# duyhominhnguyen/conan-fgw

Hardware: AMD Instinct MI355X
Metric: molecules/s (K=5 conformers) (higher is better)
Workload: dtype f32

## Files before the change

### conan-fgw_amd/_lib.py

```python
from __future__ import annotations

import ctypes
import os
import subprocess

import torch

_HERE = os.path.dirname(os.path.abspath(__file__))
_SO = os.path.join(_HERE, "libconan_fgw_hip.so")
_LIB = None
ABI_VERSION = 6

c_int, c_float, c_void_p, c_ll = ctypes.c_int, ctypes.c_float, ctypes.c_void_p, ctypes.c_longlong


class FgwParams(ctypes.Structure):
    _fields_ = [("alpha", c_float), ("epsilon", c_float), ("max_iter", c_int), ("tol", c_float), ("inner_tol", c_float),
                ("num_iter_max", c_int), ("stop_thr", c_float), ("fixed_structure", c_int), ("fixed_features", c_int),
                ("warmstart", c_int), ("loss_fun", c_int), ("cs_small_int", c_int)]


class BatchLayout(ctypes.Structure):
    _fields_ = [(n, c_int) for n in ("B", "K", "num_graphs", "num_atoms", "num_bond_edges", "max_nodes", "x_dim", "ea_dim")] + \
               [(n, c_ll) for n in ("off_atom_off", "off_bond_off", "off_z", "off_pos", "off_x", "off_bsrc", "off_bdst", "off_battr", "off_y", "bytes")]


class WgradJob(ctypes.Structure):
    _fields_ = [("ws", c_void_p), ("dW", c_void_p), ("dbias", c_void_p), ("M", c_int), ("K", c_int), ("N", c_int), ("slices", c_int)]


class WgradSlabJob(ctypes.Structure):
    _fields_ = [("g", c_void_p), ("x", c_void_p), ("m_dev", c_void_p), ("ws", c_void_p), ("M", c_int), ("K", c_int), ("N", c_int), ("slices", c_int)]


_P = c_void_p
SIGNATURES = {
    "conan_abi_version": (c_int, []),
    "conan_collate_layout": (c_int, [c_int, c_int, _P, _P, c_int, c_int, ctypes.POINTER(BatchLayout)]),
    "conan_collate_pack": (c_int, [ctypes.POINTER(BatchLayout), _P, _P, _P, _P, _P, _P, _P, _P, _P]),
    "conan_collate_unpack": (c_int, [_P, ctypes.POINTER(BatchLayout), _P, _P, _P, _P, _P, _P, _P, _P, _P, _P, _P]),
    "conan_graph_ptr_from_batch": (c_int, [_P, c_int, c_int, _P, _P]),
    "conan_radius_graph_csr": (c_int, [_P, _P, c_int, c_int, c_float, c_int, c_int, _P, _P, _P, _P, _P, _P]),
    "conan_csr_transpose": (c_int, [_P, c_int, c_int, _P, _P, _P, _P, _P, _P]),
    "conan_edge_pairs": (c_int, [_P, _P, _P, _P, _P, c_int, _P, _P, _P, _P, _P, _P, _P, _P]),
    "conan_radius_graph_build_ws": (c_ll, [c_int, c_int, c_int, c_int]),
    "conan_radius_graph_build": (c_int, [_P, _P, c_int, c_int, c_float, c_int, c_int] + [_P] * 12 + [_P]),
    "conan_edge_index_i64": (c_int, [_P, _P, c_int, _P, _P]),
    "conan_embedding_fwd": (c_int, [_P, _P, c_int, c_int, c_int, _P, _P]),
    "conan_onehot_rows": (c_int, [_P, c_int, c_int, c_int, _P, _P]),
    "conan_embedding_bwd_ws": (c_ll, [c_int, c_int, c_int]),
    "conan_embedding_bwd": (c_int, [_P, _P, c_int, c_int, c_int, c_int, _P, _P, _P]),
    "conan_linear_fwd": (c_int, [_P, _P, _P, _P, c_int, c_int, c_int, c_int, c_int, _P, _P, _P]),
    "conan_linear_multi_fwd": (c_int, [_P, _P, _P, c_int, c_int, c_int, c_int, c_int, _P, _P, _P, _P]),
    "conan_linear_sum_fwd": (c_int, [_P, _P, _P, c_int, c_int, _P, _P, c_int, c_int, _P, _P, _P]),
    "conan_ssp_bwd": (c_int, [_P, _P, c_int, c_int, _P, _P, _P]),
    "conan_linear_wgrad_ws": (c_ll, [c_int, c_int, c_int]),
    "conan_linear_wgrad": (c_int, [_P, _P, c_int, c_int, c_int, _P, _P, _P, _P, _P]),
    "conan_bond_graph_csr": (c_int, [_P, c_int, c_int, _P, _P, _P, _P, _P, _P, _P, _P]),
    "conan_gat_edge_vec": (c_int, [_P, _P, c_int, c_int, _P, _P]),
    "conan_gat_edge_vec_bwd": (c_int, [_P, _P, _P, c_int, c_int, _P, _P, _P]),
    "conan_gat_node_alpha": (c_int, [_P, _P, _P, c_int, c_int, _P, _P, _P]),
    "conan_gat_aggregate_fwd": (c_int, [_P, _P, _P, _P, _P, _P, _P, c_int, _P, _P, c_float, c_int, c_int, _P, _P, _P, _P]),
    "conan_gat_bwd_ws": (c_ll, [c_int, c_int, c_int, c_int]),
    "conan_gat_aggregate_bwd": (c_int, [_P] * 15 + [c_int, _P, c_float, c_int, c_int, c_int, _P, _P, _P, _P]),
    "conan_linear_act_fwd": (c_int, [_P, _P, _P, c_int, c_int, c_int, c_int, _P, _P, _P, _P]),
    "conan_unary_fwd": (c_int, [_P, c_ll, c_int, _P, _P]),
    "conan_unary_bwd": (c_int, [_P, _P, c_ll, c_int, _P, _P]),
    "conan_zero_tail": (c_int, [_P, _P, c_int, c_int, _P]),
    "conan_rbf_wgrad": (c_int, [_P, _P, c_int, _P, c_int, c_float, c_int, _P, _P, _P, _P, _P]),
    "conan_wgrad_batchable": (c_int, [c_int, c_int]),
    "conan_linear_wgrad_scaled": (c_int, [_P, _P, c_int, c_int, c_int, _P, _P, _P, _P, _P, _P]),
    "conan_linear_wgrad_slabs": (c_int, [_P, _P, c_int, c_int, c_int, _P, _P, _P]),
    "conan_rbf_wgrad_slabs": (c_int, [_P, _P, c_int, _P, c_int, c_float, c_int, _P, _P, _P]),
    "conan_wgrad_reduce_batch": (c_int, [ctypes.POINTER(WgradJob), c_int, _P]),
    "conan_linear_wgrad_slabs_batch": (c_int, [ctypes.POINTER(WgradSlabJob), c_int, _P]),
    "conan_filter_bwd_supported": (c_int, [c_int, c_int]),
    "conan_filter_bwd_slices": (c_int, [c_int]),
    "conan_filter_bwd_ws": (c_ll, [c_int, c_int, c_int]),
    "conan_filter_bwd": (c_int, [_P, _P, _P, c_int, _P, c_int, c_float, _P, c_int, _P, _P, _P, _P, _P, _P]),
    "conan_filter_bwd2_supported": (c_int, [c_int, c_int]),
    "conan_filter_bwd2_slices": (c_int, [c_int]),
    "conan_filter_bwd2_ws": (c_ll, [c_int, c_int, c_int]),
    "conan_filter_bwd2": (c_int, [_P, _P, _P, c_int, _P, c_int, c_float, _P, c_int, _P, _P, _P, _P, _P, _P, _P, _P]),
    "conan_rbf_fwd": (c_int, [_P, _P, c_int, _P, c_int, c_float, _P, _P]),
    "conan_cutoff_scale": (c_int, [_P, _P, c_int, c_int, c_float, _P, _P, _P]),
# ... 63 lines not shown
    "conan_fgw_densify": (c_int, [_P, _P, _P, _P, c_int, c_int, c_int, c_float, c_float, c_float, _P, _P, _P, _P]),
    "conan_fgw_densify_bwd": (c_int, [_P, _P, _P, _P, c_int, c_int, c_int, c_float, c_float, c_float, _P, _P]),
    "conan_fgw_workspace_bytes": (c_ll, [c_int] * 7),
    "conan_fgw_barycenter_fwd": (c_int, [_P, _P, _P, _P, _P, _P, _P, c_int, c_int, c_int, c_int, ctypes.POINTER(FgwParams), c_int, c_int,
                                         _P, _P, _P, _P, _P, _P, _P, _P]),
    "conan_fgw_barycenter_fwd_ragged": (c_int, [_P, _P, _P, _P, _P, _P, _P, _P, _P, _P, c_int, c_int, c_int, c_int, ctypes.POINTER(FgwParams),
                                                c_int, c_int, _P, _P, _P, _P, _P, _P, _P, _P]),
    "conan_fgw_pair_workspace_bytes": (c_ll, [c_int, c_int, c_int, c_int]),
    "conan_fgw_pair_fwd": (c_int, [_P, _P, _P, _P, _P, _P, c_int, c_int, ctypes.POINTER(FgwParams), c_int, c_int, _P, _P, _P, _P, _P, _P]),
    "conan_fgw_pair_dist": (c_int, [_P, _P, _P, _P, _P, _P, c_int, c_int, c_float, c_int, _P, _P]),
    "conan_fgw_pair_dist_bwd": (c_int, [_P, _P, _P, _P, _P, _P, c_int, c_int, c_float, c_int, _P, _P, _P, _P, _P, _P]),
    "conan_fgw_acc_lds_resident": (c_int, [c_int]),
    "conan_fgw_acc_pair_workspace_bytes": (c_ll, [c_int, c_int]),
    "conan_fgw_acc_pair_fwd": (c_int, [_P] * 6 + [c_int, c_int, ctypes.c_double, ctypes.c_double, c_int, ctypes.c_double] + [_P] * 5),
    "conan_fgw_mixup_workspace_bytes": (c_ll, [c_int, c_int, c_int, c_int]),
    "conan_fgw_mixup_barycenter_fwd": (c_int, [_P] * 7 + [c_int, c_int, c_int, c_int, ctypes.POINTER(FgwParams), ctypes.c_double, c_int, ctypes.c_double] + [_P] * 8),
    "conan_sinkhorn_workspace_bytes": (c_ll, [c_int, c_int, c_int]),
    "conan_sinkhorn_lds_resident": (c_int, [c_int, c_int]),
    "conan_sinkhorn_fwd": (c_int, [_P] * 7 + [c_int, c_int, c_int, c_ll, c_float, c_int, c_int, c_float] + [_P] * 8),
    "conan_sinkhorn_bwd_workspace_bytes": (c_ll, [c_int, c_int, c_int, c_int]),
    "conan_sinkhorn_bwd_lds_resident": (c_int, [c_int, c_int]),
    "conan_sinkhorn_bwd": (c_int, [_P] * 7 + [c_int, c_int, c_int, c_ll, c_float, c_int, c_int] + [_P] * 9),
    "conan_sinkhorn_ext_workspace_bytes": (c_ll, [c_int, c_int, c_int]),
    "conan_sinkhorn_ext_lds_resident": (c_int, [c_int, c_int]),
    "conan_sinkhorn_ext_nerr": (c_int, [c_int, c_int, c_int]),
    "conan_sinkhorn_ext_fwd": (c_int, [_P] * 7 + [c_int, c_int, c_int, c_ll, ctypes.c_double, c_int, c_int, ctypes.c_double, ctypes.c_double, c_int,
                                       ctypes.c_double, c_int] + [_P] * 11),
    "conan_fgw_barycenter_bwd": (c_int, [_P, _P, _P, _P, c_int, c_int, c_int, c_int, _P, _P]),
    "conan_fgw_barycenter_bwd_full_workspace_bytes": (c_ll, [c_int, c_int, c_int, c_int]),
    "conan_fgw_barycenter_bwd_full": (c_int, [_P, _P, _P, _P, _P, _P, _P, _P, _P, c_int, c_int, c_int, c_int, c_int, c_int, c_int,
                                              _P, _P, _P, _P, _P, _P, _P, _P]),
    "conan_fgw_readout_fwd": (c_int, [_P, c_int, c_int, c_int, c_int, c_int, _P, _P]),
    "conan_fgw_readout_bwd": (c_int, [_P, _P, c_int, c_int, c_int, c_int, c_int, _P, _P]),
}

_D = ctypes.c_double
EXT_SIGNATURES = {
    "conan_fgw_acc_pair_bwd_lds_resident": (c_int, [c_int]),
    "conan_fgw_acc_pair_bwd_workspace_bytes": (c_ll, [c_int, c_int, c_int]),
    "conan_fgw_acc_pair_bwd": (c_int, [_P] * 6 + [c_int, c_int, _D, _D, c_int] + [_P] * 12),
}

EXT_TABLES = {
    "conan_fgw_hip_pair_grad.h": {
        "conan_fgw_pair_bwd_lds_resident": (c_int, [c_int]),
        "conan_fgw_pair_bwd_workspace_bytes": (c_ll, [c_int, c_int, c_int, c_int]),
        "conan_fgw_pair_bwd": (c_int, [_P] * 6 + [c_int, c_int, _D, _D, c_int, c_int, _D, c_int, c_int] + [_P] * 13),
    },
    "conan_fgw_hip_bregman_grad.h": {
        "conan_fgw_bregman_bwd_lds_resident": (c_int, [c_int]),
        "conan_fgw_bregman_bwd_workspace_bytes": (c_ll, [c_int, c_int, c_int]),
        "conan_fgw_bregman_bwd": (c_int, [_P] * 6 + [c_int, c_int, _D, _D, c_int, c_int, c_int] + [_P] * 13),
    },
    "conan_fgw_hip_mixup_grad.h": {
        "conan_fgw_mixup_barycenter_fwd_record": (c_int, [_P] * 7 + [c_int, c_int, c_int, c_int, ctypes.POINTER(FgwParams), _D, c_int, _D] + [_P] * 9),
        "conan_fgw_mixup_barycenter_bwd_lds_resident": (c_int, [c_int]),
        "conan_fgw_mixup_barycenter_bwd_workspace_bytes": (c_ll, [c_int] * 5),
        "conan_fgw_mixup_barycenter_bwd": (c_int, [_P] * 6 + [c_int, c_int, c_int, c_int, ctypes.POINTER(FgwParams), _D, c_int, _D] + [_P] * 15),
    },
}

_ERR = {-1: "bad argument", -2: "HIP launch failure", -3: "unsupported configuration"}


def library_path() -> str:
    return _SO


def build(force: bool = False) -> str:
    args = ["make", "-C", os.path.join(_HERE, "csrc"), "-s", "-j8"]
    if force:
        args.append("-B")
    subprocess.check_call(args)
    return _SO


def lib():
    global _LIB
    if _LIB is None:
        if not os.path.exists(_SO):
            raise RuntimeError(
                f"{_SO} is missing: the HIP extension is not built. Run `python -c 'import __graft_entry__ as g; g.build()'` "
                "(or make -C conan-fgw_amd/csrc). There is no CPU fallback for this path.")
        L = ctypes.CDLL(_SO)
        for table in (SIGNATURES, EXT_SIGNATURES, *EXT_TABLES.values()):
            for name, (res, args) in table.items():
                fn = getattr(L, name)
                fn.restype, fn.argtypes = res, args
        if L.conan_abi_version() != ABI_VERSION:
            raise RuntimeError(f"libconan_fgw_hip.so: ABI version {L.conan_abi_version()} != {ABI_VERSION} expected by _lib.py (stale build: "
                               "make -C conan-fgw_amd/csrc)")
        _LIB = L
    return _LIB


def stream_ptr() -> int:
    return _raw_stream(_cur_device())


try:
    _raw_stream = torch._C._cuda_getCurrentRawStream
    _cur_device = torch._C._cuda_getDevice
except AttributeError:
    def _raw_stream(_dev):
        return torch.cuda.current_stream().cuda_stream

# ... 31 lines not shown
```

### conan-fgw_amd/csrc/fp_planes.h

```cpp
#pragma once
#include "common.h"

namespace {

typedef float f32x16 __attribute__((ext_vector_type(16)));
typedef __bf16 bf16x8 __attribute__((ext_vector_type(8)));
typedef __bf16 bf16x4 __attribute__((ext_vector_type(4)));
typedef _Float16 f16x8 __attribute__((ext_vector_type(8)));
typedef _Float16 f16x4 __attribute__((ext_vector_type(4)));

__device__ __forceinline__ void split3(const float *v, bf16x8 &p1, bf16x8 &p2, bf16x8 &p3) {
#pragma unroll
    for (int j = 0; j < 8; ++j) {
        const __bf16 h1 = (__bf16)v[j];
        const float r1 = v[j] - (float)h1;
        const __bf16 h2 = (__bf16)r1;
        const float r2 = r1 - (float)h2;
        p1[j] = h1; p2[j] = h2; p3[j] = (__bf16)r2;
    }
}
__device__ __forceinline__ void split2h(const float *v, f16x8 &p1, f16x8 &p2) {
#pragma unroll
    for (int j = 0; j < 8; ++j) {
        const _Float16 h1 = (_Float16)v[j];
// ... 70 lines not shown
    float4 v[TRANS ? PERW * 4 : PER];
    static __device__ __forceinline__ bool block(int u, int &n, int &k) {
        const int tid = threadIdx.x, lane = tid & 63, wave = tid >> 6;
        if (!TRANS) {
            const int q = tid + u * NT;
            n = (4 * q) / KD; k = 4 * q - n * KD;
            return q < V4;
        }
        const int n4l = (lane & 3) | ((lane >> 4) << 2), k4l = (lane >> 2) & 3;
        const int pt = wave + u * (NT / 64);
        k = (pt / (NO / 64)) * 16 + 4 * k4l; n = (pt % (NO / 64)) * 64 + 4 * n4l;
        return pt < PATCHES;
    }
    __device__ __forceinline__ void fetch(const float *w, int ldw = TRANS ? NO : KD) {
#pragma unroll
        for (int u = 0; u < (TRANS ? PERW : PER); ++u) {
            int n, k;
            const bool ok = block(u, n, k);
#pragma unroll
            for (int j = 0; j < (TRANS ? 4 : 1); ++j) {
                const float *p = TRANS ? w + (size_t)(k + j) * ldw + n : w + (size_t)(n * KD + k) + (size_t)n * (ldw - KD);
                v[(TRANS ? 4 : 1) * u + j] = ok ? *reinterpret_cast<const float4 *>(p) : make_float4(0.f, 0.f, 0.f, 0.f);
            }
        }
    }
    __device__ __forceinline__ float absmax() const {
        float m = 0.f;
#pragma unroll
        for (int u = 0; u < (TRANS ? PERW * 4 : PER); ++u) m = absmax4(m, v[u]);
        return m;
    }
    template <class St>
    __device__ __forceinline__ void each4(St st) const {
#pragma unroll
        for (int u = 0; u < (TRANS ? PERW : PER); ++u) {
            int n, k;
            if (!block(u, n, k)) continue;
#pragma unroll
            for (int e = 0; e < (TRANS ? 4 : 1); ++e) {
                float v4[4];
                if (TRANS) transpose4_row(&v[4 * u], e, v4);
                else { v4[0] = v[u].x; v4[1] = v[u].y; v4[2] = v[u].z; v4[3] = v[u].w; }
                st(n + e, k, v4);
            }
        }
    }
    template <class P>
    __device__ __forceinline__ void park(void *planes, float sc, P kperm) const {
        each4([&](int n, int k, const float *v4) { store4_planes(planes, NO, KD + 8, n, kperm(k), v4, sc); });
    }
    __device__ __forceinline__ void park(void *planes, float sc) const { park(planes, sc, [](int k) { return k; }); }
};

template <int S>
__device__ __forceinline__ void row_load(const float *__restrict__ src, int row, int pitch, int h, float4 (&xa)[S], float4 (&xb)[S]) {
    const float *r = src + (size_t)row * pitch + 8 * h;
#pragma unroll
    for (int s = 0; s < S; ++s) {
        xa[s] = *reinterpret_cast<const float4 *>(r + 16 * s);
        xb[s] = *reinterpret_cast<const float4 *>(r + 16 * s + 4);
    }
}
template <int S>
__device__ __forceinline__ float row_absmax(const float4 (&xa)[S], const float4 (&xb)[S]) {
    float am = 0.f;
#pragma unroll
    for (int s = 0; s < S; ++s) { am = absmax4(am, xa[s]); am = absmax4(am, xb[s]); }
    return fmaxf(am, __shfl_xor(am, 32));
}
__device__ __forceinline__ void row_split(const float4 &a, const float4 &b, float sc, f16x8 &q1, f16x8 &q2) {
    const float xv[8] = {a.x, a.y, a.z, a.w, b.x, b.y, b.z, b.w};
    split2h(xv, sc, q1, q2);
}
template <int N, int WS, int NB>
__device__ __forceinline__ void planes_kstep(const void *planes, int colp, int l31, const f16x8 &q1, const f16x8 &q2, f32x16 (&acc)[NB]) {
    const _Float16 *WH = reinterpret_cast<const _Float16 *>(planes);
#pragma unroll
    for (int nb = 0; nb < NB; ++nb) {
        const int row = 32 * nb + l31;
        const f16x8 p1 = *reinterpret_cast<const f16x8 *>(&WH[(0 * N + row) * WS + colp]);
        const f16x8 p2 = *reinterpret_cast<const f16x8 *>(&WH[(1 * N + row) * WS + colp]);
        acc[nb] = __builtin_amdgcn_mfma_f32_32x32x16_f16(p2, q1, acc[nb], 0, 0, 0);
        acc[nb] = __builtin_amdgcn_mfma_f32_32x32x16_f16(p1, q2, acc[nb], 0, 0, 0);
        acc[nb] = __builtin_amdgcn_mfma_f32_32x32x16_f16(p1, q1, acc[nb], 0, 0, 0);
    }
}

}
```

### conan-fgw_amd/csrc/gemm.hip

```cpp
#include "fp_planes.h"

namespace {

constexpr int BM = 64;
constexpr int BK = 32;
constexpr int XP = BK + 1;

template <int NB>
__global__ void __launch_bounds__(256) k_linear(const float *__restrict__ x, const float *__restrict__ w,
                                                const float *__restrict__ bias, const float *__restrict__ residual,
                                                int M, int K, int N, int w_kn, int act, float *__restrict__ y,
                                                const int *__restrict__ m_dev) {
    constexpr int BN = 64 * NB;
    if (m_dev) M = min(M, *m_dev);
    if ((int)blockIdx.x * BM >= M) return;
    constexpr int WP = BN + 1;
    __shared__ float xs[BM * XP];
    __shared__ float ws[BK * WP];
    const int tid = threadIdx.x, lane = tid & 63, wave = tid >> 6;
    const int wm = wave >> 1, wn = wave & 1;
    const int row0 = blockIdx.x * BM, col0 = blockIdx.y * BN;
    f32x16 acc[NB];
#pragma unroll
    for (int b = 0; b < NB; ++b)
#pragma unroll
        for (int r = 0; r < 16; ++r) acc[b][r] = 0.f;

    for (int k0 = 0; k0 < K; k0 += BK) {
        for (int t = tid; t < BM * BK; t += 256) {
            int r = t / BK, k = t % BK;
            int gr = row0 + r, gk = k0 + k;
            xs[r * XP + k] = (gr < M && gk < K) ? x[(size_t)gr * K + gk] : 0.f;
        }
        if (w_kn) {
            for (int t = tid; t < BK * BN; t += 256) {
                int k = t / BN, n = t % BN;
                int gk = k0 + k, gn = col0 + n;
                ws[k * WP + n] = (gk < K && gn < N) ? w[(size_t)gk * N + gn] : 0.f;
            }
        } else {
            for (int t = tid; t < BK * BN; t += 256) {
                int n = t / BK, k = t % BK;
                int gk = k0 + k, gn = col0 + n;
                ws[k * WP + n] = (gk < K && gn < N) ? w[(size_t)gn * K + gk] : 0.f;
            }
        }
        __syncthreads();
        const int arow = wm * 32 + (lane & 31), kh = lane >> 5;
#pragma unroll
        for (int kk = 0; kk < BK; kk += 2) {
            float a = xs[arow * XP + kk + kh];
#pragma unroll
            for (int b = 0; b < NB; ++b) {
// ... 641 lines not shown
__global__ void __launch_bounds__(256) k_wgrad_reduce4_batch(WgradJobs J) {
    __shared__ float4 part[8][32];
    const int job = blockIdx.y;
    const int NK4 = J.NK4[job], N4 = J.N4[job], slices = J.slices[job];
    float4 *bout = J.bout[job];
    const int g = threadIdx.x >> 5, c = threadIdx.x & 31;
    const int idx = blockIdx.x * 32 + c;
    if ((int)blockIdx.x * 32 >= NK4 + (bout ? N4 : 0)) return;
    const bool is_w = idx < NK4, is_b = !is_w && bout && idx - NK4 < N4;
    const float4 *src = is_w ? J.slabs[job] + idx : J.bias_slabs[job] + (idx - NK4);
    const int stride = is_w ? NK4 : N4;
    float4 a0 = make_float4(0.f, 0.f, 0.f, 0.f), a1 = a0, a2 = a0, a3 = a0;
    if (is_w || is_b) {
        int s = g;
        for (; s + 56 < slices; s += 64) {
            float4 v[8];
#pragma unroll
            for (int u = 0; u < 8; ++u) v[u] = src[(size_t)(s + 8 * u) * stride];
#pragma unroll
            for (int u = 0; u < 8; u += 4) {
                a0.x += v[u].x; a0.y += v[u].y; a0.z += v[u].z; a0.w += v[u].w;
                a1.x += v[u + 1].x; a1.y += v[u + 1].y; a1.z += v[u + 1].z; a1.w += v[u + 1].w;
                a2.x += v[u + 2].x; a2.y += v[u + 2].y; a2.z += v[u + 2].z; a2.w += v[u + 2].w;
                a3.x += v[u + 3].x; a3.y += v[u + 3].y; a3.z += v[u + 3].z; a3.w += v[u + 3].w;
            }
        }
        for (; s < slices; s += 8) { const float4 v0 = src[(size_t)s * stride]; a0.x += v0.x; a0.y += v0.y; a0.z += v0.z; a0.w += v0.w; }
    }
    a0.x += a2.x; a0.y += a2.y; a0.z += a2.z; a0.w += a2.w;
    a1.x += a3.x; a1.y += a3.y; a1.z += a3.z; a1.w += a3.w;
    part[g][c] = make_float4(a0.x + a1.x, a0.y + a1.y, a0.z + a1.z, a0.w + a1.w);
    __syncthreads();
    if (g == 0 && (is_w || is_b)) {
        float4 r = part[0][c];
#pragma unroll
        for (int q = 1; q < 8; ++q) { const float4 v = part[q][c]; r.x += v.x; r.y += v.y; r.z += v.z; r.w += v.w; }
        if (is_w) J.out[job][idx] = r; else bout[idx - NK4] = r;
    }
}

constexpr int WG_GROUPS = 16;

static int wgrad_slices(int M, int K) {
    int s = (M + 127) / 128;
    if (s < 1) s = 1;
    const int cap = K > 64 ? 512 : WG_SLICES_MAX;
    if (s > cap) s = cap;
    return s;
}

}

int conan_linear_t_try(const float *x, const float *w, const float *bias, const float *residual, int M, int K, int N, int w_kn,
                       int act, float *y, const int *m_dev, hipStream_t s, int *rc, float *pre_out);
int conan_linear_t_multi(const float *x, const float *const *w, const float *const *bias, int M, int K, int N, int njobs, int act, float *const *y,
                         float *const *pre, const int *m_dev, hipStream_t s, int *rc);
int conan_linear_t_sum(const float *const *x, const int *ldx, const float *const *w, int nsrc, int w_kn, int ldw, const float *bias,
                       const float *residual, int M, int N, float *y, const int *m_dev, hipStream_t s, int *rc);

extern "C" {

int conan_linear_fwd(const float *x, const float *w, const float *bias, const float *residual, int M, int K, int N,
                     int w_kn, int act, const int *m_dev, float *y, void *stream) {
    if (!x || !w || !y || M < 0 || K <= 0 || N <= 0 || act < 0 || act > 3 || (act == 2 && !residual)) return CONAN_E_BADARG;
    if (M == 0) return CONAN_OK;
    hipStream_t s = as_stream(stream);
    {
        int rc = CONAN_OK;
        if (conan_linear_t_try(x, w, bias, residual, M, K, N, w_kn, act, y, m_dev, s, &rc, nullptr)) return rc;
    }
    if (K <= 128 && N <= 128 && (K % BK) == 0) {
        const int Kp = (K + BK - 1) / BK * BK;
        const int tiles = (M + RM - 1) / RM;
        const int grid = tiles < 512 ? tiles : 512;
        if (N > 64) {
            const size_t lds = ((size_t)Kp * 129 + 2 * RM * XP) * 4;
            (void)hipFuncSetAttribute(reinterpret_cast<const void *>(&k_linear_res<2>), hipFuncAttributeMaxDynamicSharedMemorySize, (int)lds);
            k_linear_res<2><<<grid, 256, lds, s>>>(x, w, bias, residual, M, K, N, w_kn, act, y, m_dev);
        } else {
            const size_t lds = ((size_t)Kp * 65 + 2 * RM * XP) * 4;
            (void)hipFuncSetAttribute(reinterpret_cast<const void *>(&k_linear_res<1>), hipFuncAttributeMaxDynamicSharedMemorySize, (int)lds);
            k_linear_res<1><<<grid, 256, lds, s>>>(x, w, bias, residual, M, K, N, w_kn, act, y, m_dev);
        }
        CONAN_LAUNCH_CHECK();
        return CONAN_OK;
    }
    if (N > 64) {
        dim3 grid((M + BM - 1) / BM, (N + 127) / 128);
        k_linear<2><<<grid, 256, 0, s>>>(x, w, bias, residual, M, K, N, w_kn, act, y, m_dev);
    } else {
        dim3 grid((M + BM - 1) / BM, (N + 63) / 64);
        k_linear<1><<<grid, 256, 0, s>>>(x, w, bias, residual, M, K, N, w_kn, act, y, m_dev);
    }
    CONAN_LAUNCH_CHECK();
    return CONAN_OK;
}

int conan_linear_act_fwd(const float *x, const float *w, const float *bias, int M, int K, int N, int act, const int *m_dev, float *y,
                         float *pre, void *stream) {
    if (!x || !w || !y || !pre || M < 0 || K <= 0 || N <= 0 || (act != 1 && act != 3)) return CONAN_E_BADARG;
    if (M == 0) return CONAN_OK;
    int rc = CONAN_OK;
    if (conan_linear_t_try(x, w, bias, nullptr, M, K, N, 0, act, y, m_dev, as_stream(stream), &rc, pre)) return rc;
    return CONAN_E_UNSUPPORTED;
}

int conan_linear_multi_fwd(const float *x, const float *const *w, const float *const *bias, int M, int K, int N, int num_layers, int act,
                           const int *m_dev, float *const *y, float *const *pre, void *stream) {
    if (!x || !w || !y || M < 0 || K <= 0 || N <= 0 || num_layers < 1 || (act != 0 && act != 1 && act != 3)) return CONAN_E_BADARG;
    for (int q = 0; q < num_layers; ++q)
        if (!w[q] || !y[q]) return CONAN_E_BADARG;
    if (M == 0) return CONAN_OK;
    int rc = CONAN_OK;
    if (conan_linear_t_multi(x, w, bias, M, K, N, num_layers, act, y, pre, m_dev, as_stream(stream), &rc)) return rc;
    for (int q = 0; q < num_layers; ++q) {
        if (!conan_linear_t_try(x, w[q], bias ? bias[q] : nullptr, nullptr, M, K, N, 0, act, y[q], m_dev, as_stream(stream), &rc, pre ? pre[q] : nullptr))
            return CONAN_E_UNSUPPORTED;
        if (rc != CONAN_OK) return rc;
    }
    return CONAN_OK;
}

int conan_linear_sum_fwd(const float *const *x, const int *ldx, const float *const *w, int num_inputs, int w_kn, const float *bias,
                         const float *residual, int M, int N, const int *m_dev, float *y, void *stream) {
    if (!x || !ldx || !w || !y || M < 0 || N <= 0 || num_inputs < 1) return CONAN_E_BADARG;
    for (int c = 0; c < num_inputs; ++c)
        if (!x[c] || !w[c] || ldx[c] < 128 || (ldx[c] & 3)) return CONAN_E_BADARG;
    if (M == 0) return CONAN_OK;
    int rc = CONAN_OK;
    if (conan_linear_t_sum(x, ldx, w, num_inputs, w_kn, w_kn ? N : 128, bias, residual, M, N, y, m_dev, as_stream(stream), &rc)) return rc;
    return CONAN_E_UNSUPPORTED;
}

int conan_ssp_bwd(const float *dy, const float *y, int rows, int width, const int *m_dev, float *g, void *stream) {
    const long long count = (long long)rows * width;
    if (rows < 0 || width <= 0 || (count && (!dy || !y || !g))) return CONAN_E_BADARG;
    if (!count) return CONAN_OK;
    int blocks = (int)((count + 255) / 256);
    if (blocks > 4096) blocks = 4096;
    k_ssp_bwd<<<blocks, 256, 0, as_stream(stream)>>>(dy, y, count, width, m_dev, g);
    CONAN_LAUNCH_CHECK();
    return CONAN_OK;
}

long long conan_linear_wgrad_ws(int M, int K, int N) {
    return (long long)(wgrad_slices(M, K) + WG_GROUPS) * ((long long)N * K + N);
}

static int wgrad_launch(const float *g, const float *x, int M, int K, int N, const int *m_dev, float *dW, float *dbias, float *ws,
                        hipStream_t s, const float *dist, const float *offset, float coeff, const float *gmax = nullptr) {
    const bool rbf = dist != nullptr;
    const int slices = wgrad_slices(M, K);
    float *slabs = ws, *bias_slabs = ws + (size_t)slices * N * K;
    {
        const int KT = K > 64 ? 128 : 64;
        dim3 grid(slices, (N + 127) / 128, (K + KT - 1) / KT);
        int tn_remap = 0;
// ... 170 lines not shown
```

### conan-fgw_amd/csrc/gemm_t.hip

```cpp
#include "fp_planes.h"

namespace {

constexpr int LT_THREADS = 512;
#ifndef CONAN_LINEAR_MAX_WGS
#define CONAN_LINEAR_MAX_WGS 256
#endif

constexpr int LT_NPL = 2;
constexpr int LT_OP = 68;

struct LtJobs {
    const float *w[4], *bias[4];
    float *y[4], *pre[4];
};

template <int K, int N, int ACT, int NT>
__global__ void __launch_bounds__(NT) k_linear_t16(const float *__restrict__ x, const float *__restrict__ w,
                                                           const float *__restrict__ bias, const float *__restrict__ residual,
                                                           int M, int w_kn, float *y,
                                                           const int *__restrict__ m_dev, int ldx, int ldw, int ldy,
                                                           const float *accum, float *pre_out, int nc, const LtJobs J) {
    constexpr int act = ACT;
    constexpr int NB = N / 32;
    constexpr int S = K / 16;
    constexpr int WS = K + 8;
    extern __shared__ __attribute__((aligned(16))) float lds[];
    __bf16 *WB = reinterpret_cast<__bf16 *>(lds);
    float *BL = lds + (LT_NPL * N * WS) / 2;
    float *OT = BL + N + (threadIdx.x >> 6) * (32 * LT_OP);
    __shared__ float wred[NT / 64];
    float wun = 1.0f;
    if (m_dev) M = min(M, *m_dev);
    const int tiles = (M + 31) >> 5;
    const int tid = threadIdx.x, lane = tid & 63, wave = tid >> 6;
    const int chunk = nc > 1 ? (int)blockIdx.x % nc : 0, slot = nc > 1 ? (int)blockIdx.x / nc : (int)blockIdx.x;
    const int nslots = nc > 1 ? (int)gridDim.x / nc : (int)gridDim.x;
    if (nc > 1 && J.w[0]) {
        w = J.w[chunk]; bias = J.bias[chunk]; y = J.y[chunk]; pre_out = J.pre[chunk];
    } else if (nc > 1) {
        const int n0 = chunk * N;
        w += w_kn ? (size_t)n0 : (size_t)n0 * ldw;
        if (bias) bias += n0;
        if (residual) residual += n0;
        if (accum) accum += n0;
        if (pre_out) pre_out += n0;
        y += n0;
    }
    if (slot * (NT / 64) >= tiles) return;
    const int l31 = lane & 31, h = lane >> 5;
    const int wave_stride = nslots * (NT / 64);
    float4 xa[S], xb[S];
    auto load_x = [&](int t) { row_load<S>(x, min((t << 5) + l31, M - 1), ldx, h, xa, xb); };
    if (slot * (NT / 64) + wave < tiles) load_x(slot * (NT / 64) + wave);
    auto stage = [&](auto &st) {
        st.fetch(w, ldw);
        float wsc;
        pow2_scale(block_absmax<NT>(st.absmax(), wred), wsc, wun);
        st.park(WB, wsc);
    };
    if (!w_kn) { WeightPlanes<N, K, NT, false> st; stage(st); } else { WeightPlanes<N, K, NT, true> st; stage(st); }
    for (int t = tid; t < N; t += NT) BL[t] = bias ? bias[t] : 0.f;
    __syncthreads();

    for (int tile = slot * (NT / 64) + wave; tile < tiles; tile += wave_stride) {
        const int m = (tile << 5) + l31;
        const bool valid = m < M;
        f32x16 acc[NB];
#pragma unroll
        for (int nb = 0; nb < NB; ++nb)
#pragma unroll
            for (int r = 0; r < 16; ++r) acc[nb][r] = 0.f;
        float xsc, xu;
        pow2_scale(row_absmax<S>(xa, xb), xsc, xu);
        const float xun = xu * wun;
        f16x8 q1[S], q2[S];
#pragma unroll
        for (int s = 0; s < S; ++s) row_split(xa[s], xb[s], xsc, q1[s], q2[s]);
        if (tile + wave_stride < tiles) load_x(tile + wave_stride);
#pragma unroll
        for (int s = 0; s < S; ++s) {
            planes_kstep<N, WS>(WB, 16 * s + 8 * h, l31, q1[s], q2[s], acc);
            __builtin_amdgcn_sched_barrier(0);
        }
        const int mc = valid ? m : M - 1;
        const float *rr = residual ? residual + (size_t)mc * ldy + 4 * h : nullptr;
        const float *ar = accum ? accum + (size_t)mc * ldy + 4 * h : nullptr;
        float4 rv[NB][4];
        if (rr) {
#pragma unroll
            for (int nb = 0; nb < NB; ++nb)
#pragma unroll
                for (int q = 0; q < 4; ++q) rv[nb][q] = *reinterpret_cast<const float4 *>(rr + 32 * nb + 8 * q);
        }
#pragma unroll
        for (int nb = 0; nb < NB; ++nb) {
#pragma unroll
            for (int q = 0; q < 4; ++q) {
                const float4 bb = *reinterpret_cast<const float4 *>(&BL[32 * nb + 8 * q + 4 * h]);
                float v[4] = {fmaf(acc[nb][4 * q], xun, bb.x), fmaf(acc[nb][4 * q + 1], xun, bb.y), fmaf(acc[nb][4 * q + 2], xun, bb.z),
                              fmaf(acc[nb][4 * q + 3], xun, bb.w)};
                if (ar) {
                    const float4 av = *reinterpret_cast<const float4 *>(ar + 32 * nb + 8 * q);
                    v[0] += av.x; v[1] += av.y; v[2] += av.z; v[3] += av.w;
                }
                if (pre_out && valid) *reinterpret_cast<float4 *>(pre_out + (size_t)m * ldy + 4 * h + 32 * nb + 8 * q) = make_float4(v[0], v[1], v[2], v[3]);
                const float r4[4] = {rr ? rv[nb][q].x : 0.f, rr ? rv[nb][q].y : 0.f, rr ? rv[nb][q].z : 0.f, rr ? rv[nb][q].w : 0.f};
#pragma unroll
                for (int u = 0; u < 4; ++u) {
                    if (act == 1) v[u] = ssp_f(v[u]);
                    else if (act == 3) v[u] = v[u] * __builtin_amdgcn_rcpf(1.0f + __expf(-v[u]));
                    if (act == 2) v[u] *= 1.0f - 0.5f * __expf(-r4[u]);
                    else if (rr) v[u] += r4[u];
                }
                *reinterpret_cast<float4 *>(&OT[l31 * LT_OP + 32 * (nb & 1) + 8 * q + 4 * h]) = make_float4(v[0], v[1], v[2], v[3]);
            }
            if (nb & 1) {
                const int rbase = tile << 5;
                wave_lds_fence();
#pragma unroll
                for (int i = 0; i < 8; ++i) {
                    const int r = 4 * i + (lane >> 4), c = 4 * (lane & 15);
                    const float4 o = *reinterpret_cast<const float4 *>(&OT[r * LT_OP + c]);
                    if (rbase + r < M) *reinterpret_cast<float4 *>(y + (size_t)(rbase + r) * ldy + 32 * (nb - 1) + c) = o;
                }
                wave_lds_fence();
            }
        }
    }
}

template <int K, int N>
int launch_t(const float *x, const float *w, const float *bias, const float *residual, int M, int w_kn, int act, float *y,
             const int *m_dev, hipStream_t s, int ldx = K, int ldw = 0, int ldy = N, const float *accum = nullptr, float *pre_out = nullptr,
             int nc = 1, const LtJobs *jobs = nullptr) {
    if (ldw == 0) ldw = w_kn ? N : K;
    LtJobs J{};
    if (jobs) J = *jobs;
    const size_t lds_w = ((size_t)(LT_NPL * N * (K + 8)) / 2 + N) * 4;
    const int tiles16 = (M + 31) / 32;
    const bool narrow = tiles16 < 8 * 256;
    const size_t lds16 = lds_w + (size_t)(narrow ? 4 : 8) * 32 * LT_OP * 4;
    const int per = narrow ? 4 : 8;
    int grid16 = (tiles16 + per - 1) / per;
    if (grid16 > CONAN_LINEAR_MAX_WGS / nc) grid16 = CONAN_LINEAR_MAX_WGS / nc;
    grid16 *= nc;
#define LAUNCH16(A)                                                                                                              \
    do {                                                                                                                         \
        if (narrow) {                                                                                                            \
            (void)hipFuncSetAttribute(reinterpret_cast<const void *>(&k_linear_t16<K, N, A, 256>),                               \
                                      hipFuncAttributeMaxDynamicSharedMemorySize, (int)lds16);                                   \
            k_linear_t16<K, N, A, 256><<<grid16, 256, lds16, s>>>(x, w, bias, residual, M, w_kn, y, m_dev, ldx, ldw, ldy, accum, pre_out, nc, J); \
        } else {                                                                                                                 \
            (void)hipFuncSetAttribute(reinterpret_cast<const void *>(&k_linear_t16<K, N, A, LT_THREADS>),                        \
                                      hipFuncAttributeMaxDynamicSharedMemorySize, (int)lds16);                                   \
            k_linear_t16<K, N, A, LT_THREADS><<<grid16, LT_THREADS, lds16, s>>>(x, w, bias, residual, M, w_kn, y, m_dev, ldx, ldw, ldy, accum, \
                                                                                pre_out, nc, J);                                 \
        }                                                                                                                        \
    } while (0)
    switch (act) {
        case 0: LAUNCH16(0); break;
        case 1: LAUNCH16(1); break;
        case 2: LAUNCH16(2); break;
        default: LAUNCH16(3); break;
    }
#undef LAUNCH16
    return hipGetLastError() == hipSuccess ? CONAN_OK : CONAN_E_LAUNCH;
}


struct LtSrcs {
    const float *x[3], *w[3];
    int ldx[3];
};
__device__ __forceinline__ float pow2i(int e) { return e < -126 ? 0.f : __uint_as_float((unsigned)(min(e, 127) + 127) << 23); }
constexpr int LT_NOEXP = -100000;
__device__ __forceinline__ int pow2_exp(float amax) {
    const int e = (int)((__float_as_uint(amax) >> 23) & 0xffu);
    return (e >= 9 && e <= 254) ? e - 135 : LT_NOEXP;
}
template <int K, int N, int NT>
__device__ __forceinline__ int lt_stage_planes(const float *__restrict__ w, int w_kn, int ldw, _Float16 *WB, float *wred) {
    int ew;
    auto stage = [&](auto &st) {
        st.fetch(w, ldw);
        ew = pow2_exp(block_absmax<NT>(st.absmax(), wred));
        st.park(WB, ew == LT_NOEXP ? 1.0f : pow2i(-ew));
    };
    if (!w_kn) { WeightPlanes<N, K, NT, false> st; stage(st); } else { WeightPlanes<N, K, NT, true> st; stage(st); }
    __syncthreads();
    return ew == LT_NOEXP ? 0 : ew;
}

constexpr int LS_OP = 36;
__device__ __forceinline__ void ls_store64(float *OT, const float4 (&vv)[2][4], float *yb, int ldy, int rbase, int M, int lane) {
    const int l31 = lane & 31, h = lane >> 5;
#pragma unroll
    for (int half = 0; half < 2; ++half) {
        if ((l31 >> 4) == half) {
#pragma unroll
            for (int nb = 0; nb < 2; ++nb)
#pragma unroll
                for (int q = 0; q < 4; ++q) *reinterpret_cast<float4 *>(&OT[(l31 & 15) * LT_OP + 32 * nb + 8 * q + 4 * h]) = vv[nb][q];
        }
        wave_lds_fence();
#pragma unroll
        for (int i = 0; i < 4; ++i) {
            const int rw = 4 * i + (lane >> 4), cc = 4 * (lane & 15);
            const float4 o = *reinterpret_cast<const float4 *>(&OT[rw * LT_OP + cc]);
            const int r = rbase + 16 * half + rw;
// ... 190 lines not shown
}

template <int KC, int NC>
static int chunk_launch(const float *x, const float *w, const float *bias, const float *residual, int M, int K, int N, int w_kn, int act,
                        float *y, const int *m_dev, hipStream_t s, float *pre_out) {
    if (K == KC && N / NC > 1 && N / NC <= 4)
        return launch_t<KC, NC>(x, w, bias, residual, M, w_kn, act, y, m_dev, s, K, w_kn ? N : K, N, nullptr, pre_out, N / NC);
    for (int n0 = 0; n0 < N; n0 += NC)
        for (int k0 = 0; k0 < K; k0 += KC) {
            const bool first = k0 == 0, last = k0 + KC >= K;
            const float *wc = w_kn ? w + (size_t)k0 * N + n0 : w + (size_t)n0 * K + k0;
            const int rc = launch_t<KC, NC>(x + k0, wc, (first && bias) ? bias + n0 : nullptr, (last && residual) ? residual + n0 : nullptr, M, w_kn,
                                            last ? act : 0, y + n0, m_dev, s, K, w_kn ? N : K, N, first ? nullptr : y + n0,
                                            (last && pre_out) ? pre_out + n0 : nullptr);
            if (rc != CONAN_OK) return rc;
        }
    return CONAN_OK;
}

#ifndef CONAN_LINEAR_FAN
#define CONAN_LINEAR_FAN 1
#endif
#ifndef CONAN_LINEAR_FAN_MIN_ROWS
#define CONAN_LINEAR_FAN_MIN_ROWS 65536
#endif
int conan_linear_t_multi(const float *x, const float *const *w, const float *const *bias, int M, int K, int N, int njobs, int act, float *const *y,
                         float *const *pre, const int *m_dev, hipStream_t s, int *rc) {
    if (K != 128 || N != 128 || njobs < 2 || njobs > 4 || M < 1) return 0;
    LtJobs J{};
    for (int q = 0; q < njobs; ++q) { J.w[q] = w[q]; J.bias[q] = bias ? bias[q] : nullptr; J.y[q] = y[q]; J.pre[q] = pre ? pre[q] : nullptr; }
    if (CONAN_LINEAR_FAN && act == 0 && !pre && njobs <= 3 && M >= CONAN_LINEAR_FAN_MIN_ROWS) {
        *rc = njobs == 2 ? launch_fan<2>(x, J, M, m_dev, s) : launch_fan<3>(x, J, M, m_dev, s);
        return 1;
    }
    *rc = launch_t<128, 128>(x, w[0], nullptr, nullptr, M, 0, act, y[0], m_dev, s, 128, 0, 128, nullptr, nullptr, njobs, &J);
    return 1;
}

int conan_linear_t_sum(const float *const *x, const int *ldx, const float *const *w, int nsrc, int w_kn, int ldw, const float *bias,
                       const float *residual, int M, int N, float *y, const int *m_dev, hipStream_t s, int *rc) {
    if (N != 128 || nsrc < 2 || nsrc > 3 || M < 1) return 0;
    LtSrcs Sx{};
    for (int c = 0; c < nsrc; ++c) { Sx.x[c] = x[c]; Sx.w[c] = w[c]; Sx.ldx[c] = ldx[c]; }
    *rc = nsrc == 2 ? launch_sum<2>(Sx, bias, residual, M, w_kn, y, m_dev, ldw, N, s) : launch_sum<3>(Sx, bias, residual, M, w_kn, y, m_dev, ldw, N, s);
    return 1;
}

#ifndef CONAN_LINEAR_NO_KSUM
#define CONAN_LINEAR_KSUM 1
#else
#define CONAN_LINEAR_KSUM 0
#endif
int conan_linear_t_try(const float *x, const float *w, const float *bias, const float *residual, int M, int K, int N, int w_kn,
                       int act, float *y, const int *m_dev, hipStream_t s, int *rc, float *pre_out) {
    if (M < 1) return 0;
    if (CONAN_LINEAR_KSUM && N == 128 && (K == 256 || K == 384) && act == 0 && !pre_out) {
        const float *xs[3], *wc[3];
        int ldx[3];
        for (int c = 0; c < K / 128; ++c) { xs[c] = x + 128 * c; ldx[c] = K; wc[c] = w_kn ? w + (size_t)128 * c * N : w + 128 * c; }
        if (conan_linear_t_sum(xs, ldx, wc, K / 128, w_kn, w_kn ? N : K, bias, residual, M, N, y, m_dev, s, rc)) return 1;
    }
    if (K == 128 && N == 128) { *rc = launch_t<128, 128>(x, w, bias, residual, M, w_kn, act, y, m_dev, s, 128, 0, 128, nullptr, pre_out); return 1; }
    if (K == 128 && N == 64) { *rc = launch_t<128, 64>(x, w, bias, residual, M, w_kn, act, y, m_dev, s, 128, 0, 64, nullptr, pre_out); return 1; }
    if (K == 64 && N == 64) { *rc = launch_t<64, 64>(x, w, bias, residual, M, w_kn, act, y, m_dev, s, 64, 0, 64, nullptr, pre_out); return 1; }
    if (K == 64 && N == 128) { *rc = launch_t<64, 128>(x, w, bias, residual, M, w_kn, act, y, m_dev, s, 64, 0, 128, nullptr, pre_out); return 1; }
    if (K == 32 && N == 128 && !w_kn) { *rc = launch_t<32, 128>(x, w, bias, residual, M, w_kn, act, y, m_dev, s, 32, 0, 128, nullptr, pre_out); return 1; }
    if ((K % 64) || (N % 64) || K > 1024 || N > 1024) return 0;
    const bool k128 = (K % 128) == 0, n128 = (N % 128) == 0;
    if (k128 && n128) *rc = chunk_launch<128, 128>(x, w, bias, residual, M, K, N, w_kn, act, y, m_dev, s, pre_out);
    else if (k128) *rc = chunk_launch<128, 64>(x, w, bias, residual, M, K, N, w_kn, act, y, m_dev, s, pre_out);
    else if (n128) *rc = chunk_launch<64, 128>(x, w, bias, residual, M, K, N, w_kn, act, y, m_dev, s, pre_out);
    else *rc = chunk_launch<64, 64>(x, w, bias, residual, M, K, N, w_kn, act, y, m_dev, s, pre_out);
    return 1;
}
```

### conan-fgw_amd/csrc/mlp2.hip

```cpp
#include "fp_planes.h"

namespace {

constexpr int M2_THREADS = 256, M2_WAVES = 4;
constexpr int M2_NPL = 2;

__device__ __forceinline__ int m2_perm4(int k) {
    const int a = (k & 15) >> 2;
    return (k & ~15) + 8 * (a & 1) + 4 * (a >> 1);
}
template <int NO, int KD, bool TRANS> using M2Planes = WeightPlanes<NO, KD, M2_THREADS, TRANS>;

template <int KA, int NA, int NB, int MODE, int SUM = 0>
__device__ __forceinline__ void m2_rows(const float4 (&xa)[KA / 16], const float4 (&xb)[KA / 16], const float4 (&av)[MODE == 1 ? NA / 32 : 1][4],
                                        const float *__restrict__ residual, const __bf16 *WB, const __bf16 *WB2, const float *BL, float unA, float unB,
                                        int m, int mr, bool valid, int h, int l31, float *__restrict__ mid_out, float *__restrict__ y,
                                        float4 (&keep)[SUM ? NB / 32 : 1][4]) {
    constexpr int SA = KA / 16, SB = NA / 16, MBA = NA / 32, MBB = NB / 32;
    constexpr int WSA = KA + 8, WSB = NA + 8;
    f32x16 acc1[MBA];
#pragma unroll
    for (int nb = 0; nb < MBA; ++nb)
#pragma unroll
        for (int r = 0; r < 16; ++r) acc1[nb][r] = 0.f;
    float xsc, xu;
    pow2_scale(row_absmax<SA>(xa, xb), xsc, xu);
    const float un1 = xu * unA;
#pragma unroll
    for (int s = 0; s < SA; ++s) {
        f16x8 q1, q2;
        row_split(xa[s], xb[s], xsc, q1, q2);
        planes_kstep<NA, WSA>(WB, 16 * s + 8 * h, l31, q1, q2, acc1);
        __builtin_amdgcn_sched_barrier(0);
    }
#pragma unroll
    for (int nb = 0; nb < MBA; ++nb)
#pragma unroll
        for (int r = 0; r < 16; ++r) acc1[nb][r] *= un1;
#pragma unroll
    for (int nb = 0; nb < MBA; ++nb)
#pragma unroll
        for (int q = 0; q < 4; ++q) {
            float v[4];
            if (MODE == 1) {
                const float a4[4] = {av[nb][q].x, av[nb][q].y, av[nb][q].z, av[nb][q].w};
#pragma unroll
                for (int u = 0; u < 4; ++u) v[u] = acc1[nb][4 * q + u] * (1.0f - 0.5f * __expf(-a4[u]));
            } else if (MODE == 3) {
#pragma unroll
                for (int u = 0; u < 4; ++u) v[u] = acc1[nb][4 * q + u];
            } else {
                const float4 bb = *reinterpret_cast<const float4 *>(&BL[32 * nb + 8 * q + 4 * h]);
                const float p4[4] = {acc1[nb][4 * q + 0] + bb.x, acc1[nb][4 * q + 1] + bb.y, acc1[nb][4 * q + 2] + bb.z, acc1[nb][4 * q + 3] + bb.w};
#pragma unroll
                for (int u = 0; u < 4; ++u) v[u] = MODE == 0 ? ssp_f(p4[u]) : p4[u];
            }
#pragma unroll
            for (int u = 0; u < 4; ++u) acc1[nb][4 * q + u] = v[u];
            if (mid_out && valid)
                *reinterpret_cast<float4 *>(mid_out + (size_t)m * NA + 32 * nb + 8 * q + 4 * h) = make_float4(v[0], v[1], v[2], v[3]);
        }
    float4 rv[MODE == 0 ? MBB : 1][4];
    if (MODE == 0 && residual) {
        const float *rr = residual + (size_t)mr * NB + 4 * h;
// ... 15 lines not shown
        for (int r = 0; r < 16; ++r) am = fmaxf(am, fabsf(acc1[nb][r]));
    am = fmaxf(am, __shfl_xor(am, 32));
    float msc, mu;
    pow2_scale(am, msc, mu);
    const float un2 = mu * unB;
#pragma unroll
    for (int ms = 0; ms < SB; ++ms) {
        const int mb = ms >> 1, sgrp = ms & 1;
        float hv[8];
#pragma unroll
        for (int j = 0; j < 8; ++j) hv[j] = acc1[mb][8 * sgrp + j];
        f16x8 q1, q2;
        split2h(hv, msc, q1, q2);
        planes_kstep<NB, WSB>(WB2, 32 * mb + 16 * sgrp + 8 * h, l31, q1, q2, acc2);
        __builtin_amdgcn_sched_barrier(0);
    }
    if (!valid) return;
#pragma unroll
    for (int nb = 0; nb < MBB; ++nb)
#pragma unroll
        for (int q = 0; q < 4; ++q) {
            const float4 bb = *reinterpret_cast<const float4 *>(&BL[NA + 32 * nb + 8 * q + 4 * h]);
            float4 o = make_float4(fmaf(acc2[nb][4 * q], un2, bb.x), fmaf(acc2[nb][4 * q + 1], un2, bb.y), fmaf(acc2[nb][4 * q + 2], un2, bb.z),
                                   fmaf(acc2[nb][4 * q + 3], un2, bb.w));
            if (MODE == 0 && residual) { o.x += rv[nb][q].x; o.y += rv[nb][q].y; o.z += rv[nb][q].z; o.w += rv[nb][q].w; }
            if (MODE == 2) { o.x = ssp_f(o.x); o.y = ssp_f(o.y); o.z = ssp_f(o.z); o.w = ssp_f(o.w); }
            if (SUM == 1) { keep[nb][q] = o; continue; }
            if (SUM == 2) { o.x += keep[nb][q].x; o.y += keep[nb][q].y; o.z += keep[nb][q].z; o.w += keep[nb][q].w; }
            *reinterpret_cast<float4 *>(y + (size_t)m * NB + 32 * nb + 8 * q + 4 * h) = o;
        }
}

template <int KA>
__device__ __forceinline__ void m2_ssp_bwd_row(float4 (&xa)[KA / 16], float4 (&xb)[KA / 16], const float4 (&ya)[KA / 16], const float4 (&yb)[KA / 16],
                                               float *__restrict__ in_out, int m, int h, bool valid) {
#pragma unroll
    for (int s = 0; s < KA / 16; ++s) {
        xa[s].x *= 1.0f - 0.5f * __expf(-ya[s].x); xa[s].y *= 1.0f - 0.5f * __expf(-ya[s].y);
        xa[s].z *= 1.0f - 0.5f * __expf(-ya[s].z); xa[s].w *= 1.0f - 0.5f * __expf(-ya[s].w);
        xb[s].x *= 1.0f - 0.5f * __expf(-yb[s].x); xb[s].y *= 1.0f - 0.5f * __expf(-yb[s].y);
        xb[s].z *= 1.0f - 0.5f * __expf(-yb[s].z); xb[s].w *= 1.0f - 0.5f * __expf(-yb[s].w);
        if (in_out && valid) {
            float *gr = in_out + (size_t)m * KA + 8 * h + 16 * s;
            *reinterpret_cast<float4 *>(gr) = xa[s];
            *reinterpret_cast<float4 *>(gr + 4) = xb[s];
        }
    }
}

template <int KA, int NA, int NB, int MODE>
__global__ void __launch_bounds__(M2_THREADS) k_mlp2(const float *__restrict__ x, const float *__restrict__ wA, const float *__restrict__ bA,
                                                     const float *__restrict__ wB, const float *__restrict__ bB, const float *__restrict__ aux,
                                                     const float *__restrict__ residual, int M, float *__restrict__ mid_out, float *__restrict__ y,
                                                     float *__restrict__ in_out) {
    constexpr bool BWD = (MODE & 1) != 0;
    constexpr int SA = KA / 16, MBA = NA / 32;
    constexpr int WORDS_A = (M2_NPL * NA * (KA + 8)) / 2, WORDS_B = (M2_NPL * NB * (NA + 8)) / 2;
    constexpr int WORDS = WORDS_A + WORDS_B;
    extern __shared__ __attribute__((aligned(16))) float lds[];
    __bf16 *WB = reinterpret_cast<__bf16 *>(lds);
    __bf16 *WB2 = reinterpret_cast<__bf16 *>(lds + WORDS_A);
    float *BL = lds + WORDS;
    __shared__ float wred[2 * M2_WAVES];
    float unA = 1.0f, unB = 1.0f;
    const int tid = threadIdx.x, lane = tid & 63, wave = tid >> 6;
    const int l31 = lane & 31, h = lane >> 5;
    const int tile = blockIdx.x * M2_WAVES + wave;
    const int m = (tile << 5) + l31;
    const bool valid = m < M;
    const int mr = valid ? m : M - 1;

    float4 xa[SA], xb[SA];
    row_load<SA>(x, mr, KA, h, xa, xb);
    float4 av[MODE == 1 ? MBA : 1][4];
    if (MODE == 1) {
        const float *ar = aux + (size_t)mr * NA + 4 * h;
#pragma unroll
        for (int nb = 0; nb < MBA; ++nb)
#pragma unroll
            for (int q = 0; q < 4; ++q) av[nb][q] = *reinterpret_cast<const float4 *>(ar + 32 * nb + 8 * q);
    }
    float4 ya[SA], yb[SA];
    if (MODE == 3) row_load<SA>(aux, mr, KA, h, ya, yb);
    M2Planes<NA, KA, BWD> stA;
    M2Planes<NB, NA, BWD> stB;
    stA.fetch(wA);
    stB.fetch(wB);
    const float ma = wave_max(stA.absmax()), mb = wave_max(stB.absmax());
    if (lane == 0) { wred[wave] = ma; wred[M2_WAVES + wave] = mb; }
    __syncthreads();
    float a = wred[0], b = wred[M2_WAVES];
#pragma unroll
    for (int w = 1; w < M2_WAVES; ++w) { a = fmaxf(a, wred[w]); b = fmaxf(b, wred[M2_WAVES + w]); }
    float scA, scB;
    pow2_scale(a, scA, unA);
    pow2_scale(b, scB, unB);
    stA.park(WB, scA);
    stB.park(WB2, scB, [](int k) { return m2_perm4(k); });
    for (int t = tid; t < NA + NB; t += M2_THREADS) BL[t] = BWD ? 0.f : (t < NA ? bA[t] : bB[t - NA]);
    if (MODE == 3) m2_ssp_bwd_row<KA>(xa, xb, ya, yb, in_out, m, h, valid);
    __syncthreads();

    float4 none[1][4];
    m2_rows<KA, NA, NB, MODE>(xa, xb, av, residual, WB, WB2, BL, unA, unB, m, mr, valid, h, l31, mid_out, y, none);
}

struct M2Head {
    const float *x, *wA, *bA, *wB, *bB, *aux;
    float *mid_out, *y, *in_out;
};
template <int KA, int NA, int NB, int MODE, bool SPLIT>
__global__ void __launch_bounds__(M2_THREADS) k_mlp2_dual(const M2Head ha, const M2Head hb, const int *__restrict__ m_dev, int M) {
    static_assert(MODE == 2 || (MODE == 3 && !SPLIT), "heads: lin1 -> lin2 -> act and its backward");
    constexpr bool BWD = MODE == 3;
    constexpr int NH = SPLIT ? 1 : 2, NX = BWD ? NH : 1;
    constexpr int SA = KA / 16;
    constexpr int WORDS_A = (M2_NPL * NA * (KA + 8)) / 2, WORDS_B = (M2_NPL * NB * (NA + 8)) / 2;
    constexpr int WORDS = WORDS_A + WORDS_B;
    extern __shared__ __attribute__((aligned(16))) float lds[];
    __shared__ float wred[NH * 2 * M2_WAVES];
    if (m_dev) M = min(M, *m_dev);
    if ((int)blockIdx.x * (32 * M2_WAVES) >= M) return;
    const M2Head hd[2] = {SPLIT && blockIdx.y ? hb : ha, hb};
    const int tid = threadIdx.x, lane = tid & 63, wave = tid >> 6;
    const int l31 = lane & 31, h = lane >> 5;
    const int m = ((blockIdx.x * M2_WAVES + wave) << 5) + l31;
    const bool valid = m < M;
    const int mr = valid ? m : M - 1;

    float4 xa[NX][SA], xb[NX][SA], ya[NX][SA], yb[NX][SA];
#pragma unroll
    for (int i = 0; i < NX; ++i) {
        row_load<SA>(hd[i].x, mr, KA, h, xa[i], xb[i]);
        if (BWD) row_load<SA>(hd[i].aux, mr, KA, h, ya[i], yb[i]);
    }
    M2Planes<NA, KA, BWD> stA[NH];
    M2Planes<NB, NA, BWD> stB[NH];
#pragma unroll
    for (int i = 0; i < NH; ++i) {
        stA[i].fetch(hd[i].wA);
        stB[i].fetch(hd[i].wB);
    }
#pragma unroll
    for (int i = 0; i < NH; ++i) {
        const float ma = wave_max(stA[i].absmax()), mb = wave_max(stB[i].absmax());
        if (lane == 0) { wred[(2 * i) * M2_WAVES + wave] = ma; wred[(2 * i + 1) * M2_WAVES + wave] = mb; }
    }
    __syncthreads();
    float unA[NH], unB[NH];
#pragma unroll
    for (int i = 0; i < NH; ++i) {
        float a = wred[(2 * i) * M2_WAVES], b = wred[(2 * i + 1) * M2_WAVES];
#pragma unroll
        for (int w = 1; w < M2_WAVES; ++w) { a = fmaxf(a, wred[(2 * i) * M2_WAVES + w]); b = fmaxf(b, wred[(2 * i + 1) * M2_WAVES + w]); }
        float scA, scB;
        pow2_scale(a, scA, unA[i]);
        pow2_scale(b, scB, unB[i]);
        stA[i].park(lds + i * WORDS, scA);
        stB[i].park(lds + i * WORDS + WORDS_A, scB, [](int k) { return m2_perm4(k); });
        float *BL = lds + NH * WORDS + i * (NA + NB);
        for (int t = tid; t < NA + NB; t += M2_THREADS) BL[t] = BWD ? 0.f : (t < NA ? hd[i].bA[t] : hd[i].bB[t - NA]);
        if (BWD) m2_ssp_bwd_row<KA>(xa[i], xb[i], ya[i], yb[i], hd[i].in_out, m, h, valid);
    }
    __syncthreads();

    float4 av[1][4];
    float4 keep[BWD ? NB / 32 : 1][4];
#pragma unroll
    for (int i = 0; i < NH; ++i) {
        const __bf16 *WB = reinterpret_cast<const __bf16 *>(lds + i * WORDS), *WB2 = reinterpret_cast<const __bf16 *>(lds + i * WORDS + WORDS_A);
        const float *BL = lds + NH * WORDS + i * (NA + NB);
        if constexpr (!BWD) {
            float4 none[1][4];
            m2_rows<KA, NA, NB, MODE>(xa[0], xb[0], av, nullptr, WB, WB2, BL, unA[i], unB[i], m, mr, valid, h, l31, hd[i].mid_out, hd[i].y, none);
        } else if (i == 0) {
            m2_rows<KA, NA, NB, MODE, 1>(xa[i], xb[i], av, nullptr, WB, WB2, BL, unA[i], unB[i], m, mr, valid, h, l31, hd[i].mid_out, nullptr, keep);
        } else {
            m2_rows<KA, NA, NB, MODE, 2>(xa[i], xb[i], av, nullptr, WB, WB2, BL, unA[i], unB[i], m, mr, valid, h, l31, hd[i].mid_out, hd[i].y, keep);
        }
    }
}

template <int KA, int NA, int NB, int MODE>
int m2_launch(const float *x, const float *wA, const float *bA, const float *wB, const float *bB, const float *aux, const float *residual, int M,
              float *mid_out, float *y, float *in_out, hipStream_t s) {
    constexpr int WA = (M2_NPL * NA * (KA + 8)) / 2, WBw = (M2_NPL * NB * (NA + 8)) / 2;
    const size_t lds = ((size_t)(WA + WBw) + NA + NB) * 4;
    (void)hipFuncSetAttribute(reinterpret_cast<const void *>(&k_mlp2<KA, NA, NB, MODE>), hipFuncAttributeMaxDynamicSharedMemorySize, (int)lds);
    const int tiles = (M + 31) / 32;
    k_mlp2<KA, NA, NB, MODE><<<(tiles + M2_WAVES - 1) / M2_WAVES, M2_THREADS, lds, s>>>(x, wA, bA, wB, bB, aux, residual, M, mid_out, y, in_out);
    return hipGetLastError() == hipSuccess ? CONAN_OK : CONAN_E_LAUNCH;
}

template <int KA, int NA, int NB, int MODE, bool SPLIT>
int m2_launch_dual(const M2Head &ha, const M2Head &hb, const int *m_dev, int M, hipStream_t s) {
    constexpr int WA = (M2_NPL * NA * (KA + 8)) / 2, WBw = (M2_NPL * NB * (NA + 8)) / 2;
    const size_t lds = (SPLIT ? 1 : 2) * ((size_t)(WA + WBw) + NA + NB) * 4;
    (void)hipFuncSetAttribute(reinterpret_cast<const void *>(&k_mlp2_dual<KA, NA, NB, MODE, SPLIT>), hipFuncAttributeMaxDynamicSharedMemorySize, (int)lds);
    const int tiles = (M + 31) / 32;
    k_mlp2_dual<KA, NA, NB, MODE, SPLIT><<<dim3((tiles + M2_WAVES - 1) / M2_WAVES, SPLIT ? 2 : 1), M2_THREADS, lds, s>>>(ha, hb, m_dev, M);
    return hipGetLastError() == hipSuccess ? CONAN_OK : CONAN_E_LAUNCH;
}

}

extern "C" {

int conan_mlp2_supported(int M, int K, int N1, int N2) { return (K == 128 && N1 == 128 && N2 == 128 && M >= 1 && M <= 65536) ? 1 : 0; }

int conan_mlp2_fwd(const float *x, const float *w1, const float *b1, const float *w2, const float *b2, const float *residual, int M, int K, int N1,
                   int N2, float *mid_out, float *y, void *stream) {
    if (!x || !w1 || !b1 || !w2 || !b2 || !y || M < 0) return CONAN_E_BADARG;
    if (M == 0) return CONAN_OK;
    if (!conan_mlp2_supported(M, K, N1, N2)) return CONAN_E_UNSUPPORTED;
    return m2_launch<128, 128, 128, 0>(x, w1, b1, w2, b2, nullptr, residual, M, mid_out, y, nullptr, as_stream(stream));
}

int conan_mlp2_bwd(const float *dy, const float *w2, const float *w1, const float *mid, int M, int K, int N1, int N2, float *dmid_out, float *dx,
                   void *stream) {
    if (!dy || !w1 || !w2 || !mid || !dx || M < 0) return CONAN_E_BADARG;
    if (M == 0) return CONAN_OK;
    if (!conan_mlp2_supported(M, K, N1, N2)) return CONAN_E_UNSUPPORTED;
    return m2_launch<128, 128, 128, 1>(dy, w2, nullptr, w1, nullptr, mid, nullptr, M, dmid_out, dx, nullptr, as_stream(stream));
}

int conan_mlp2_outact_supported(int M, int K, int N1, int N2) { return (K == 128 && N1 == 64 && N2 == 64 && M >= 1 && M <= 65536) ? 1 : 0; }

int conan_mlp2_outact_fwd(const float *x, const float *w1, const float *b1, const float *w2, const float *b2, int M, int K, int N1, int N2,
                          float *mid_out, float *y, void *stream) {
    if (!x || !w1 || !b1 || !w2 || !b2 || !y || M < 0) return CONAN_E_BADARG;
    if (M == 0) return CONAN_OK;
    if (!conan_mlp2_outact_supported(M, K, N1, N2)) return CONAN_E_UNSUPPORTED;
    return m2_launch<128, 64, 64, 2>(x, w1, b1, w2, b2, nullptr, nullptr, M, mid_out, y, nullptr, as_stream(stream));
}

int conan_mlp2_outact_bwd(const float *dy, const float *y, const float *w2, const float *w1, int M, int K, int N1, int N2, float *g_out,
                          float *dmid_out, float *dx, void *stream) {
    if (!dy || !y || !w1 || !w2 || !dx || M < 0) return CONAN_E_BADARG;
    if (M == 0) return CONAN_OK;
    if (!conan_mlp2_outact_supported(M, K, N1, N2)) return CONAN_E_UNSUPPORTED;
    return m2_launch<64, 64, 128, 3>(dy, w2, nullptr, w1, nullptr, y, nullptr, M, dmid_out, dx, g_out, as_stream(stream));
}

int conan_mlp2_outact_dual_fwd(const float *x, const float *w1a, const float *b1a, const float *w2a, const float *b2a, const float *w1b, const float *b1b,
                               const float *w2b, const float *b2b, int M, int K, int N1, int N2, const int *m_dev, int form, float *mid_a, float *y_a,
                               float *mid_b, float *y_b, void *stream) {
    if (!x || !w1a || !b1a || !w2a || !b2a || !w1b || !b1b || !w2b || !b2b || !y_a || !y_b || M < 0 || (form != 0 && form != 1)) return CONAN_E_BADARG;
    if (M == 0) return CONAN_OK;
    if (!conan_mlp2_outact_supported(M, K, N1, N2)) return CONAN_E_UNSUPPORTED;
    const M2Head ha = {x, w1a, b1a, w2a, b2a, nullptr, mid_a, y_a, nullptr}, hb = {x, w1b, b1b, w2b, b2b, nullptr, mid_b, y_b, nullptr};
    return form == 0 ? m2_launch_dual<128, 64, 64, 2, true>(ha, hb, m_dev, M, as_stream(stream))
                     : m2_launch_dual<128, 64, 64, 2, false>(ha, hb, m_dev, M, as_stream(stream));
}

int conan_mlp2_outact_dual_bwd(const float *dy_a, const float *y_a, const float *w2a, const float *w1a, const float *dy_b, const float *y_b,
                               const float *w2b, const float *w1b, int M, int K, int N1, int N2, const int *m_dev, float *g_a, float *dmid_a, float *g_b,
                               float *dmid_b, float *dx, void *stream) {
    if (!dy_a || !y_a || !w1a || !w2a || !dy_b || !y_b || !w1b || !w2b || !dx || M < 0) return CONAN_E_BADARG;
    if (M == 0) return CONAN_OK;
    if (!conan_mlp2_outact_supported(M, K, N1, N2)) return CONAN_E_UNSUPPORTED;
    const M2Head ha = {dy_a, w2a, nullptr, w1a, nullptr, y_a, dmid_a, nullptr, g_a}, hb = {dy_b, w2b, nullptr, w1b, nullptr, y_b, dmid_b, dx, g_b};
    return m2_launch_dual<64, 64, 128, 3, false>(ha, hb, m_dev, M, as_stream(stream));
}

}
```

### conan-fgw_amd/gat.py

```python
from __future__ import annotations

import math
from typing import Optional

import torch
from torch import Tensor, nn

from . import ops
from ._lib import call, lib, ptr, stream_ptr

f32 = torch.float32
i32 = torch.int32


class BondGraph:

    def __init__(self, edge_index: Tensor, num_nodes: int):
        if not edge_index.is_cuda:
            raise RuntimeError("conan_fgw_amd has no CPU path: edge_index must live on the GPU")
        dev = edge_index.device
        ei = edge_index.to(torch.int64).contiguous()
        self.num_nodes, self.num_edges = int(num_nodes), int(ei.shape[1])
        n, E = self.num_nodes, max(self.num_edges, 1)
        ws = torch.empty(2 * (n + 1), dtype=i32, device=dev)
# ... 33 lines not shown
        g = ctx.graph
        dout = dout.contiguous()
        n, C = h.shape
        D = w_e.shape[1]
        dev = h.device
        ws = torch.empty(int(lib().conan_gat_bwd_ws(n, g.num_edges, C, D)), dtype=f32, device=dev)
        dh = torch.empty_like(h)
        dpar = torch.empty(3 * C + D, dtype=f32, device=dev)
        call("conan_gat_aggregate_bwd", ptr(h), ptr(dout), ptr(alpha), ptr(alpha_self), ptr(al_s), ptr(al_d), ptr(a_s), ptr(a_d), ptr(g.rowptr),
             ptr(g.col), ptr(g.eid), ptr(g.t_rowptr), ptr(g.t_pos), ptr(g.t_tgt), ptr(ea), D, ptr(v), ctx.slope, n, g.num_edges, C, ptr(ws), ptr(dh),
             ptr(dpar), stream_ptr())
        dw_e, datt_e = torch.empty_like(w_e), torch.empty(C, dtype=f32, device=dev)
        call("conan_gat_edge_vec_bwd", ptr(w_e), ptr(a_e), ptr(dpar[3 * C:]), C, D, ptr(dw_e), ptr(datt_e), stream_ptr())
        s_src, s_dst, s_edge = ctx.shapes
        return (dh, dpar[:C].view(s_src), dpar[C:2 * C].view(s_dst), dw_e, datt_e.view(s_edge),
                dpar[2 * C:3 * C] if ctx.needs_input_grad[5] else None, None, None, None)


def _glorot(t: Tensor):
    a = math.sqrt(6.0 / (t.size(-2) + t.size(-1)))
    with torch.no_grad():
        t.uniform_(-a, a)


class GATConv(nn.Module):

    def __init__(self, in_channels: int, out_channels: int, edge_dim: int = 3, negative_slope: float = 0.2):
        super().__init__()
        self.in_channels, self.out_channels, self.edge_dim, self.negative_slope = in_channels, out_channels, edge_dim, negative_slope
        self.heads = 1
        self.lin_src = nn.Linear(in_channels, out_channels, bias=False)
        self.lin_dst = self.lin_src
        self.att_src = nn.Parameter(torch.empty(1, 1, out_channels))
        self.att_dst = nn.Parameter(torch.empty(1, 1, out_channels))
        self.lin_edge = nn.Linear(edge_dim, out_channels, bias=False)
        self.att_edge = nn.Parameter(torch.empty(1, 1, out_channels))
        self.bias = nn.Parameter(torch.zeros(out_channels))
        for t in (self.lin_src.weight, self.lin_edge.weight, self.att_src, self.att_dst, self.att_edge):
            _glorot(t)

    def forward(self, x: Tensor, graph: BondGraph, edge_attr: Tensor) -> Tensor:
        h = ops.linear(x, self.lin_src.weight, None)
        return _GATAggregateFn.apply(h, self.att_src, self.att_dst, self.lin_edge.weight, self.att_edge, self.bias, graph, edge_attr,
                                     self.negative_slope)


class GATBased(nn.Module):

    def __init__(self, out_channels: int = 64, edge_dim: int = 3, in_channels: int = 9):
        super().__init__()
        self.gat_conv1 = GATConv(in_channels, out_channels, edge_dim)
        self.gat_conv2 = GATConv(out_channels, out_channels, edge_dim)

    def forward(self, x: Tensor, edge_index: Tensor, edge_attr: Tensor, batch: Tensor, num_graphs: Optional[int] = None) -> Tensor:
        if not x.is_cuda:
            raise RuntimeError("conan_fgw_amd has no CPU path: inputs must live on the GPU")
        x = x.float().contiguous()
        edge_attr = edge_attr.float()
        graph = BondGraph(edge_index, x.shape[0])
        h = self.gat_conv1(x, graph, edge_attr)
        h = self.gat_conv2(h, graph, edge_attr)
        if num_graphs is None:
            num_graphs = ops.batch_hints(batch)[0]
        if num_graphs is None:
            num_graphs = int(batch.max().item()) + 1
        gp = ops.graph_ptr_from_batch(batch, num_graphs)
        return ops.segment_sum(h, gp, num_graphs)
```

### conan-fgw_amd/head.py

```python
from __future__ import annotations

import torch
from torch import Tensor
from torch.nn import Linear

from . import ops


class EquivModelsHolder:

    @staticmethod
    def get_model(name: str, device, **kwargs):
        if name == "schnet":
            from .schnet import SchNetNoSum
            if "cutoff" in kwargs:
                return SchNetNoSum(device, hidden_channels=kwargs.get("feat_dim"), use_covalent=False, cutoff=kwargs.get("cutoff"),
                                   num_gaussians=10, num_filters=256, num_interactions=3)
            return SchNetNoSum(device, hidden_channels=kwargs.get("feat_dim"), use_covalent=False, num_interactions=3)
        if name == "gat":
            from .gat import GATBased
            return GATBased(out_channels=kwargs.get("feat_dim") // 2)
        if name == "visnet":
            from .visnet import ViSNet
            return ViSNet(device, hidden_channels=kwargs.get("feat_dim"))
        raise ValueError(f"get_model({name!r}): not a backbone of the MI355X hot path (schnet, visnet, gat); DimeNet / ESAN / "
                         "schnet_covalent variants are not reachable from train_val.py and are not built here")


def get_model(name: str, device, **kwargs):
    return EquivModelsHolder.get_model(name, device, **kwargs)


GAT_ON_SIDE_STREAM = True


class EmbeddingsWithGATAggregationBaryCenter(torch.nn.Module):

    def __init__(self, num_conformers: int, device=None, model_name: str = "schnet", agg_weight: float = 0.2,
                 max_iter: int = 100, epsilon: float = 0.1, gat_in_channels: int = 9):
        super().__init__()
        from .gat import GATBased
        self.num_conformers = num_conformers
        device = torch.device("cuda", torch.cuda.current_device()) if device is None else torch.device(device)
        self.node_embeddings_model = EquivModelsHolder.get_model(model_name, device, feat_dim=128)
        out_channels = self.node_embeddings_model.hidden_channels // 2
        self.gat_embeddings_model = (EquivModelsHolder.get_model("gat", device, feat_dim=128) if gat_in_channels == 9
                                     else GATBased(out_channels=128 // 2, in_channels=gat_in_channels))
        self.transformation_matrix_3d = Linear(out_channels, out_channels)
        self.transformation_matrix_bary = Linear(out_channels, out_channels)
        self.transformation_matrix_cov = Linear(out_channels, out_channels)
        self.molecular_regression_lin = Linear(out_channels, 1)
        self.numItermax, self.epsilon, self.agg_weight = max_iter, epsilon, agg_weight

    def _side_stream(self, device) -> "torch.cuda.Stream":
        s = getattr(self, "_gat_stream", None)
        if s is None or s.device != device:
            s = torch.cuda.Stream(device=device)
            object.__setattr__(self, "_gat_stream", s)
        return s

    def forward_dummy(self, batch, conformers_index, node_index):
        return None

    def create_aggregation_index(self, num_graphs, device=None) -> Tensor:
        if not isinstance(num_graphs, int):
            batch = num_graphs
            num_graphs = len(batch.smiles) if hasattr(batch, "smiles") else int(batch.num_graphs)
            if device is None:
                device = batch.z.device
        return self._aggregation_index(num_graphs, device)

    def _aggregation_index(self, num_graphs: int, device) -> Tensor:
        return torch.arange(num_graphs // self.num_conformers, device=device).repeat_interleave(self.num_conformers)

    def forward(self, batch, conformers_index: Tensor, node_index: Tensor, num_graphs: int = None, max_nodes: int = None) -> Tensor:
        K = self.num_conformers
        main = torch.cuda.current_stream()
        side = self._side_stream(main.device) if GAT_ON_SIDE_STREAM else main
        side.wait_stream(main)
        with torch.cuda.stream(side):
            x_cov = self.gat_embeddings_model(batch.x, batch.edge_index, batch.edge_attr, batch.batch,
                                              **({"num_graphs": num_graphs} if num_graphs is not None else {}))
            x_cov = ops.linear(x_cov, self.transformation_matrix_cov.weight, self.transformation_matrix_cov.bias)
        nm = self.node_embeddings_model
        if (ops.HEAD_SUMS_FUSED and isinstance(self.molecular_regression_lin, Linear) and hasattr(nm, "forward_w_barycenter_parts")
                and ops.stage2_head_sums_supported(nm.hidden_channels // 2, K, nm.READOUT_MODE)):
            h_3d, gptr, Y = nm.forward_w_barycenter_parts(batch.z, batch.pos, K, node_index,
                                                          **({"num_graphs": num_graphs, "max_nodes": max_nodes} if num_graphs is not None else {}))
            if conformers_index is not None and conformers_index.numel() != gptr.numel() - 1:
                raise ValueError("conformers_index must have one entry per conformer graph")
            main.wait_stream(side)
            x_cov.record_stream(main)
            return ops.stage2_head_sums(Y, h_3d, gptr, x_cov, self.transformation_matrix_3d, self.transformation_matrix_bary,
                                        self.molecular_regression_lin, self.agg_weight, K)
        x_3d, x_bary = self.node_embeddings_model.forward_w_barycenter(
            z=batch.z, pos=batch.pos, num_conformers=K, batch=node_index, max_iter=self.numItermax, epsilon=self.epsilon,
            **({"num_graphs": num_graphs, "max_nodes": max_nodes} if num_graphs is not None else {}))
        G, d = x_3d.shape
        if conformers_index is not None and conformers_index.numel() != G:
            raise ValueError("conformers_index must have one entry per conformer graph")
        main.wait_stream(side)
        x_cov.record_stream(main)
        if isinstance(self.molecular_regression_lin, Linear) and ops.stage2_head_supported(d):
            return ops.stage2_head(x_3d, x_cov, x_bary, self.transformation_matrix_3d, self.transformation_matrix_bary,
                                   self.molecular_regression_lin, self.agg_weight, K)
        x_bary = ops.linear(x_bary, self.transformation_matrix_bary.weight, self.transformation_matrix_bary.bias)
        x_3d = ops.linear(x_3d, self.transformation_matrix_3d.weight, self.transformation_matrix_3d.bias)
        x = x_3d + x_cov + self.agg_weight * x_bary
        x = x.view(G // K, K, d).mean(dim=1)
        return ops.linear(x.contiguous(), self.molecular_regression_lin.weight, self.molecular_regression_lin.bias)


class EmbeddingsWithGATAggregation(EmbeddingsWithGATAggregationBaryCenter):

    def forward(self, batch, conformers_index: Tensor, node_index: Tensor, num_graphs: int = None, max_nodes: int = None) -> Tensor:
        K = self.num_conformers
        x_3d = self.node_embeddings_model(batch.z, batch.pos, node_index)
        x_3d = ops.linear(x_3d, self.transformation_matrix_3d.weight, self.transformation_matrix_3d.bias)
        x_cov = self.gat_embeddings_model(batch.x, batch.edge_index, batch.edge_attr, batch.batch,
                                          **({"num_graphs": num_graphs} if num_graphs is not None else {}))
        x_cov = ops.linear(x_cov, self.transformation_matrix_cov.weight, self.transformation_matrix_cov.bias)
        x = x_3d + x_cov
        G, d = x.shape
        if conformers_index is not None and conformers_index.numel() != G:
            raise ValueError("conformers_index must have one entry per conformer graph")
        x = x.view(G // K, K, d).mean(dim=1)
        return ops.linear(x.contiguous(), self.molecular_regression_lin.weight, self.molecular_regression_lin.bias)


class _SelfAttentionParams(torch.nn.Module):

    def __init__(self, dim: int):
        super().__init__()
        self.query, self.key, self.value = Linear(dim, dim), Linear(dim, dim), Linear(dim, dim)


class EmbeddingsWithGATAggregationClassificationBaryCenter(EmbeddingsWithGATAggregationBaryCenter):

    def __init__(self, num_conformers: int, device=None, agg_weight: float = 0.2, gat_in_channels: int = 9, model_name: str = "schnet",
                 feat_dim: int = 512):
        torch.nn.Module.__init__(self)
        from .gat import GATBased
        self.num_conformers = num_conformers
        device = torch.device("cuda", torch.cuda.current_device()) if device is None else torch.device(device)
        self.node_embeddings_model = EquivModelsHolder.get_model(model_name, device, feat_dim=feat_dim, cutoff=10.0)
        out_channels = self.node_embeddings_model.hidden_channels // 2
        self.gat_embeddings_model = (EquivModelsHolder.get_model("gat", device, feat_dim=feat_dim) if gat_in_channels == 9
                                     else GATBased(out_channels=feat_dim // 2, in_channels=gat_in_channels))
        self.transformation_matrix_3d = Linear(out_channels, out_channels)
        self.transformation_matrix_cov = Linear(out_channels, out_channels)
        self.transformation_matrix_bary = Linear(out_channels, out_channels)
        self.molecular_regression_lin = torch.nn.Sequential(
            Linear(out_channels, out_channels), torch.nn.ReLU(), Linear(out_channels, out_channels // 2), torch.nn.ReLU(),
            Linear(out_channels // 2, 1))
        self.self_attention = _SelfAttentionParams(out_channels)
        self.numItermax, self.epsilon, self.agg_weight = 100, 0.1, agg_weight

    def forward(self, batch, conformers_index: Tensor, node_index: Tensor, num_graphs: int = None, max_nodes: int = None) -> Tensor:
        K = self.num_conformers
        main = torch.cuda.current_stream()
        side = self._side_stream(main.device)
        side.wait_stream(main)
        with torch.cuda.stream(side):
            x_cov = self.gat_embeddings_model(batch.x, batch.edge_index, batch.edge_attr, batch.batch,
                                              **({"num_graphs": num_graphs} if num_graphs is not None else {}))
            x_cov = ops.linear(x_cov, self.transformation_matrix_cov.weight, self.transformation_matrix_cov.bias)
        x_3d, x_bary = self.node_embeddings_model.forward_w_barycenter(
            z=batch.z, pos=batch.pos, num_conformers=K, batch=node_index,
            **({"num_graphs": num_graphs, "max_nodes": max_nodes} if num_graphs is not None else {}))
        x_3d = ops.linear(x_3d, self.transformation_matrix_3d.weight, self.transformation_matrix_3d.bias)
        x_bary = ops.linear(x_bary, self.transformation_matrix_bary.weight, self.transformation_matrix_bary.bias)
        main.wait_stream(side)
        x_cov.record_stream(main)
        x = x_3d + x_cov + self.agg_weight * x_bary
        G, d = x.shape
        if conformers_index is not None and conformers_index.numel() != G:
            raise ValueError("conformers_index must have one entry per conformer graph")
        x = x.view(G // K, K, d).mean(dim=1).contiguous()
        mlp = self.molecular_regression_lin
        x = ops.relu(ops.linear(x, mlp[0].weight, mlp[0].bias))
        x = ops.relu(ops.linear(x, mlp[2].weight, mlp[2].bias))
        x = ops.linear(x, mlp[4].weight, mlp[4].bias)
        return ops.sigmoid(x)


class EmbeddingsWithGATAggregationClassification(EmbeddingsWithGATAggregationClassificationBaryCenter):

    def forward(self, batch, conformers_index: Tensor, node_index: Tensor, num_graphs: int = None, max_nodes: int = None) -> Tensor:
        K = self.num_conformers
        hint = {"num_graphs": num_graphs} if num_graphs is not None else {}
        x_3d = self.node_embeddings_model(batch.z, batch.pos, node_index, **hint)
        x_3d = ops.linear(x_3d, self.transformation_matrix_3d.weight, self.transformation_matrix_3d.bias)
        x_cov = self.gat_embeddings_model(batch.x, batch.edge_index, batch.edge_attr, batch.batch, **hint)
        x_cov = ops.linear(x_cov, self.transformation_matrix_cov.weight, self.transformation_matrix_cov.bias)
        x = x_3d + x_cov
        G, d = x.shape
        if conformers_index is not None and conformers_index.numel() != G:
            raise ValueError("conformers_index must have one entry per conformer graph")
        x = x.view(G // K, K, d).mean(dim=1).contiguous()
        value = self.self_attention.value
        x = ops.linear(x, value.weight, value.bias)
        mlp = self.molecular_regression_lin
        x = ops.relu(ops.linear(x, mlp[0].weight, mlp[0].bias))
        x = ops.relu(ops.linear(x, mlp[2].weight, mlp[2].bias))
        x = ops.linear(x, mlp[4].weight, mlp[4].bias)
        return ops.sigmoid(x)


class EmbeddingsWithGAT(torch.nn.Module):

    def __init__(self, num_conformers: int, device=None, model_name: str = "schnet", gat_in_channels: int = 9):
        super().__init__()
        from .gat import GATBased
        self.num_conformers = num_conformers
        device = torch.device("cuda", torch.cuda.current_device()) if device is None else torch.device(device)
        self.node_embeddings_model = EquivModelsHolder.get_model(model_name, device, feat_dim=128)
        out_channels = self.node_embeddings_model.hidden_channels // 2
        self.gat_embeddings_model = (EquivModelsHolder.get_model("gat", device, feat_dim=128) if gat_in_channels == 9
                                     else GATBased(out_channels=128 // 2, in_channels=gat_in_channels))
        self.molecular_regression_lin = Linear(out_channels, 1)

    def forward_dummy(self, batch, conformers_index, node_index):
        return None

    create_aggregation_index = EmbeddingsWithGATAggregationBaryCenter.create_aggregation_index
    _aggregation_index = EmbeddingsWithGATAggregationBaryCenter._aggregation_index

    def forward(self, batch, conformers_index: Tensor = None, node_index: Tensor = None, num_graphs: int = None, max_nodes: int = None) -> Tensor:
        x_cov = self.gat_embeddings_model(batch.x, batch.edge_index, batch.edge_attr, batch.batch,
                                          **({"num_graphs": num_graphs} if num_graphs is not None else {}))
        return ops.linear(x_cov, self.molecular_regression_lin.weight, self.molecular_regression_lin.bias)


def classification_loss(predicted: Tensor, expected: Tensor, class_weights: Tensor = None) -> Tensor:
    return ops.bce_loss(predicted, expected, weight=class_weights)
```

### conan-fgw_amd/ops.py

```python
from __future__ import annotations

import ctypes
import math
from typing import Optional

import torch
from torch import Tensor

from . import wgrad
from ._lib import FgwParams, call, lib, ptr, stream_ptr

f32, i32, i64 = torch.float32, torch.int32, torch.int64


def _c(t: Tensor) -> Tensor:
    return t if t.is_contiguous() else t.contiguous()


FUSED_GRAPH_BUILD = True


class RadiusGraph:

    def __init__(self, pos: Tensor, graph_ptr: Tensor, num_graphs: int, cutoff: float, max_num_neighbors: int, loop: bool = False,
                 pairs: bool = False, transpose: bool = False):
        pos = _c(pos)
        if pos.dtype != f32:
            raise RuntimeError("pos must be float32")
        n = pos.shape[0]
        dev = pos.device
        self.num_atoms, self.num_graphs, self.graph_ptr = n, num_graphs, graph_ptr
        self.cutoff, self.cap, self.loop = float(cutoff), int(max_num_neighbors), bool(loop)
        self.max_edges = ME = max(1, n * (self.cap if self.loop else self.cap + 1))
        self.rowptr = torch.empty(n + 1, dtype=i32, device=dev)
        self.col = torch.empty(ME, dtype=i32, device=dev)
        self.tgt = torch.empty(ME, dtype=i32, device=dev)
        self.dist = torch.empty(ME, dtype=f32, device=dev)
        self._deg = torch.empty(n + 1, dtype=i32, device=dev)
        self._t_rowptr = self._t_eid = None
        self.pid = None
        if FUSED_GRAPH_BUILD:
            ws = torch.empty(max(1, lib().conan_radius_graph_build_ws(n, num_graphs, self.cap, int(self.loop))), dtype=i32, device=dev)
            if pairs:
                self.pid = torch.empty(ME, dtype=i32, device=dev)
                self.pair_e0 = torch.empty(ME, dtype=i32, device=dev)
                self.pair_e1 = torch.empty(ME, dtype=i32, device=dev)
                self.pair_dist = torch.empty(ME, dtype=f32, device=dev)
                self.num_pairs_dev = torch.empty(1, dtype=i32, device=dev)
            if transpose:
                self._t_rowptr = torch.empty(n + 1, dtype=i32, device=dev)
                self._t_eid = torch.empty(ME, dtype=i32, device=dev)
            call("conan_radius_graph_build", ptr(pos) if n else None, ptr(graph_ptr, i32), n, num_graphs, self.cutoff, self.cap, int(self.loop), ptr(ws),
                 ptr(self.rowptr), ptr(self.col), ptr(self.tgt), ptr(self.dist),
                 ptr(self.pid), ptr(self.pair_e0 if pairs else None), ptr(self.pair_e1 if pairs else None), ptr(self.pair_dist if pairs else None),
                 ptr(self.num_pairs_dev if pairs else None), ptr(self._t_rowptr), ptr(self._t_eid), stream_ptr())
# ... 41 lines not shown

    def edge_weight(self) -> Tensor:
        return self.dist[: self.num_edges]


def empty_rows(rows: int, width: int, device, m_dev: Optional[Tensor]) -> Tensor:
    t = torch.empty(rows, width, dtype=f32, device=device)
    if m_dev is not None:
        call("conan_zero_tail", ptr(t), ptr(m_dev), rows, width, stream_ptr())
    return t


POISON_UNREAD_TAILS = False


def unread_rows(rows: int, width: int, device) -> Tensor:
    t = torch.empty(rows, width, dtype=f32, device=device)
    if POISON_UNREAD_TAILS:
        t.fill_(float("nan"))
    return t


def batch_hints(batch: Optional[Tensor]):
    h = getattr(batch, "_conan_hints", None) if batch is not None else None
    return h if h is not None else (None, None)


def graph_ptr_from_batch(batch: Tensor, num_graphs: int) -> Tensor:
    batch = _c(batch)
    out = torch.empty(num_graphs + 1, dtype=i32, device=batch.device)
    call("conan_graph_ptr_from_batch", ptr(batch, i64), batch.shape[0], num_graphs, ptr(out), stream_ptr())
    return out


deferred_weight_gradients, flush_weight_gradients = wgrad.deferred, wgrad.flush


gmax_stats = {"tracked": 0, "used": 0}


def _tag_gmax(t: Tensor, gmax: Tensor):
    t._conan_gmax = (gmax, t._version)
    gmax_stats["tracked"] += 1


def _take_gmax(t: Tensor, g: Tensor):
    tag = getattr(t, "_conan_gmax", None)
    if tag is None or tag[1] != t._version or g.data_ptr() != t.data_ptr():
        return None
    gmax_stats["used"] += 1
    return tag[0]


class _LinearFn(torch.autograd.Function):
    @staticmethod
    def forward(ctx, x, w, b, residual, act, m_dev, grad_tail_unread=False):
        x, w = _c(x), _c(w)
        M, K = x.shape
        N = w.shape[0]
        y = torch.empty(M, N, dtype=f32, device=x.device)
        call("conan_linear_fwd", ptr(x, f32), ptr(w, f32), ptr(b), ptr(_c(residual)) if residual is not None else None,
             M, K, N, 0, act, ptr(m_dev), ptr(y), stream_ptr())
        ctx.act, ctx.m_dev, ctx.has_b, ctx.has_res, ctx.grad_tail_unread = act, m_dev, b is not None, residual is not None, grad_tail_unread
        ctx.save_for_backward(x, w, y if act else None)
        return y

    @staticmethod
    def backward(ctx, dy):
        x, w, y = ctx.saved_tensors
        dy = _c(dy)
        M, K = x.shape
        N = w.shape[0]
        md = ctx.m_dev
        if ctx.act:
            if ctx.has_res:
                raise RuntimeError("act + residual backward is not defined for this op")
            g = torch.empty_like(dy)
            call("conan_ssp_bwd", ptr(dy), ptr(y), M, N, ptr(md), ptr(g), stream_ptr())
        else:
            g = dy
        dx = dw = db = None
        if ctx.needs_input_grad[0]:
            if ctx.grad_tail_unread:
                dx = unread_rows(x.shape[0], x.shape[1], x.device)
            else:
                dx = empty_rows(x.shape[0], x.shape[1], x.device, md)
            call("conan_linear_fwd", ptr(g), ptr(w), None, None, M, N, K, 1, 0, ptr(md), ptr(dx), stream_ptr())
        if ctx.needs_input_grad[1] or (ctx.has_b and ctx.needs_input_grad[2]):
            dw, db = wgrad.plain(g, x, M, K, N, md, w, ctx.has_b)
        return dx, dw, db, (dy if ctx.has_res else None), None, None, None


class _LinearTapFn(torch.autograd.Function):

    @staticmethod
    def forward(ctx, x, w):
        x, w = _c(x), _c(w)
        M, K = x.shape
        N = w.shape[0]
        y = torch.empty(M, N, dtype=f32, device=x.device)
        call("conan_linear_fwd", ptr(x, f32), ptr(w, f32), None, None, M, K, N, 0, 0, None, ptr(y), stream_ptr())
        ctx.save_for_backward(x, w)
        return y, x.view_as(x)

    @staticmethod
    def backward(ctx, dy, dtap):
        x, w = ctx.saved_tensors
        M, K = x.shape
        N = w.shape[0]
        dx = dw = None
        if dy is None:
            return dtap, None
        dy = _c(dy)
        if ctx.needs_input_grad[0]:
            dx = torch.empty(M, K, dtype=f32, device=x.device)
            call("conan_linear_fwd", ptr(dy), ptr(w), None, ptr(_c(dtap)) if dtap is not None else None, M, N, K, 1, 0, None, ptr(dx), stream_ptr())
        elif dtap is not None:
            dx = dtap
        if ctx.needs_input_grad[1]:
            dw, _ = wgrad.plain(dy, x, M, K, N, None, w, False)
        return dx, dw


def linear_tap(x: Tensor, weight: Tensor):
    return _LinearTapFn.apply(x, weight)


def linear(x: Tensor, weight: Tensor, bias: Optional[Tensor] = None, act: bool = False, residual: Optional[Tensor] = None,
           m_dev: Optional[Tensor] = None, grad_tail_unread: bool = False) -> Tensor:
    return _LinearFn.apply(x, weight, bias, residual, 1 if act else 0, m_dev, grad_tail_unread)


class _Mlp2Fn(torch.autograd.Function):

    @staticmethod
    def forward(ctx, x, w1, b1, w2, b2, residual):
        x, w1, w2 = _c(x), _c(w1), _c(w2)
        M, K = x.shape
        N1, N2 = w1.shape[0], w2.shape[0]
        need = any(ctx.needs_input_grad[:5])
        mid = torch.empty(M, N1, dtype=f32, device=x.device) if need else None
        y = torch.empty(M, N2, dtype=f32, device=x.device)
        call("conan_mlp2_fwd", ptr(x, f32), ptr(w1, f32), ptr(_c(b1), f32), ptr(w2, f32), ptr(_c(b2), f32),
             ptr(_c(residual)) if residual is not None else None, M, K, N1, N2, ptr(mid), ptr(y), stream_ptr())
        ctx.has_res = residual is not None
        ctx.save_for_backward(x, w1, w2, mid)
        return y

    @staticmethod
    def backward(ctx, dy):
        x, w1, w2, mid = ctx.saved_tensors
        dy = _c(dy)
        M, K = x.shape
        N1, N2 = w1.shape[0], w2.shape[0]
        dmid = torch.empty(M, N1, dtype=f32, device=x.device)
        dx = torch.empty(M, K, dtype=f32, device=x.device)
        call("conan_mlp2_bwd", ptr(dy), ptr(w2), ptr(w1), ptr(mid), M, K, N1, N2, ptr(dmid), ptr(dx), stream_ptr())
        dw2, db2 = wgrad.plain(dy, mid, M, N1, N2, None, w2, True)
        dw1, db1 = wgrad.plain(dmid, x, M, K, N1, None, w1, True)
        return dx, dw1, db1, dw2, db2, (dy if ctx.has_res else None)


def mlp2(x: Tensor, w1: Tensor, b1: Tensor, w2: Tensor, b2: Tensor, residual: Optional[Tensor] = None) -> Tensor:
    if x.is_cuda and b1 is not None and b2 is not None and lib().conan_mlp2_supported(x.shape[0], x.shape[1], w1.shape[0], w2.shape[0]):
        return _Mlp2Fn.apply(x, w1, b1, w2, b2, residual)
    return linear(linear(x, w1, b1, act=True), w2, b2, residual=residual)


class _Mlp2OutActFn(torch.autograd.Function):

    @staticmethod
    def forward(ctx, x, w1, b1, w2, b2):
        x, w1, w2 = _c(x), _c(w1), _c(w2)
        M, K = x.shape
        N1, N2 = w1.shape[0], w2.shape[0]
        need = any(ctx.needs_input_grad)
        mid = torch.empty(M, N1, dtype=f32, device=x.device) if need else None
        y = torch.empty(M, N2, dtype=f32, device=x.device)
        call("conan_mlp2_outact_fwd", ptr(x, f32), ptr(w1, f32), ptr(_c(b1), f32), ptr(w2, f32), ptr(_c(b2), f32), M, K, N1, N2, ptr(mid), ptr(y),
             stream_ptr())
        ctx.save_for_backward(x, w1, w2, mid, y)
        return y

    @staticmethod
    def backward(ctx, dy):
        x, w1, w2, mid, y = ctx.saved_tensors
        dy = _c(dy)
        M, K = x.shape
        N1, N2 = w1.shape[0], w2.shape[0]
        dev = x.device
        g = torch.empty(M, N2, dtype=f32, device=dev)
        dmid = torch.empty(M, N1, dtype=f32, device=dev)
        dx = torch.empty(M, K, dtype=f32, device=dev)
        call("conan_mlp2_outact_bwd", ptr(dy), ptr(y), ptr(w2), ptr(w1), M, K, N1, N2, ptr(g), ptr(dmid), ptr(dx), stream_ptr())
        dw2, db2 = wgrad.plain(g, mid, M, N1, N2, None, w2, True)
        dw1, db1 = wgrad.plain(dmid, x, M, K, N1, None, w1, True)
        return dx, dw1, db1, dw2, db2


def mlp2_outact(x: Tensor, w1: Tensor, b1: Tensor, w2: Tensor, b2: Tensor) -> Tensor:
    if x.is_cuda and b1 is not None and b2 is not None and lib().conan_mlp2_outact_supported(x.shape[0], x.shape[1], w1.shape[0], w2.shape[0]):
        return _Mlp2OutActFn.apply(x, w1, b1, w2, b2)
    return linear(linear(x, w1, b1), w2, b2, act=True)


DUAL_HEAD = True
DUAL_HEAD_FORWARD_FORM = 0


class _Mlp2OutActDualFn(torch.autograd.Function):

    @staticmethod
    def forward(ctx, x, w1a, b1a, w2a, b2a, w1b, b1b, w2b, b2b, m_dev):
        x, w1a, w2a, w1b, w2b = _c(x), _c(w1a), _c(w2a), _c(w1b), _c(w2b)
        M, K = x.shape
        N1, N2 = w1a.shape[0], w2a.shape[0]
        dev = x.device
        need = any(ctx.needs_input_grad)
        mid_a, mid_b = (torch.empty(M, N1, dtype=f32, device=dev) if need else None for _ in range(2))
        y_a, y_b = (torch.empty(M, N2, dtype=f32, device=dev) for _ in range(2))
        call("conan_mlp2_outact_dual_fwd", ptr(x, f32), ptr(w1a, f32), ptr(_c(b1a), f32), ptr(w2a, f32), ptr(_c(b2a), f32), ptr(w1b, f32),
             ptr(_c(b1b), f32), ptr(w2b, f32), ptr(_c(b2b), f32), M, K, N1, N2, ptr(m_dev), DUAL_HEAD_FORWARD_FORM, ptr(mid_a), ptr(y_a), ptr(mid_b),
             ptr(y_b), stream_ptr())
        ctx.m_dev = m_dev
        ctx.save_for_backward(x, w1a, w2a, mid_a, y_a, w1b, w2b, mid_b, y_b)
        return y_a, y_b

    @staticmethod
    def backward(ctx, dy_a, dy_b):
        x, w1a, w2a, mid_a, y_a, w1b, w2b, mid_b, y_b = ctx.saved_tensors
        M, K = x.shape
        N1, N2 = w1a.shape[0], w2a.shape[0]
        dev, md = x.device, ctx.m_dev
        dy_a, dy_b = _c(dy_a), _c(dy_b)
        g_a, g_b = (torch.empty(M, N2, dtype=f32, device=dev) for _ in range(2))
        dmid_a, dmid_b = (torch.empty(M, N1, dtype=f32, device=dev) for _ in range(2))
        dx = empty_rows(M, K, dev, md)
        call("conan_mlp2_outact_dual_bwd", ptr(dy_a), ptr(y_a), ptr(w2a), ptr(w1a), ptr(dy_b), ptr(y_b), ptr(w2b), ptr(w1b), M, K, N1, N2, ptr(md),
             ptr(g_a), ptr(dmid_a), ptr(g_b), ptr(dmid_b), ptr(dx), stream_ptr())
        dw2b, db2b = wgrad.plain(g_b, mid_b, M, N1, N2, md, w2b, True)
        dw1b, db1b = wgrad.plain(dmid_b, x, M, K, N1, md, w1b, True)
        dw2a, db2a = wgrad.plain(g_a, mid_a, M, N1, N2, md, w2a, True)
        dw1a, db1a = wgrad.plain(dmid_a, x, M, K, N1, md, w1a, True)
        return dx, dw1a, db1a, dw2a, db2a, dw1b, db1b, dw2b, db2b, None


def mlp2_outact_dual_supported(M: int, K: int, N1: int, N2: int) -> bool:
    return bool(lib().conan_mlp2_outact_supported(int(M), int(K), int(N1), int(N2)))


def mlp2_outact_dual(x: Tensor, head_a, head_b, m_dev: Optional[Tensor] = None):
    (w1a, b1a, w2a, b2a), (w1b, b1b, w2b, b2b) = head_a, head_b
    if (DUAL_HEAD and x.is_cuda and all(b is not None for b in (b1a, b2a, b1b, b2b)) and w1a.shape == w1b.shape and w2a.shape == w2b.shape
            and mlp2_outact_dual_supported(x.shape[0], x.shape[1], w1a.shape[0], w2a.shape[0])):
        return _Mlp2OutActDualFn.apply(x, w1a, b1a, w2a, b2a, w1b, b1b, w2b, b2b, m_dev)
    if m_dev is not None:
        raise ValueError("mlp2_outact_dual: a device-side row count needs the one-launch form")
    return mlp2_outact(x, w1a, b1a, w2a, b2a), mlp2_outact(x, w1b, b1b, w2b, b2b)


class _Stage2HeadFn(torch.autograd.Function):

    @staticmethod
    def forward(ctx, x3, xc, xb, W3, b3, Wb, bb, wreg, breg, aw, K):
        x3, xc, xb = _c(x3), _c(xc), _c(xb)
        G, D = x3.shape
        if G % K != 0:
            raise ValueError(f"stage2_head: {G} conformer graphs are not a multiple of num_conformers={K}")
        B = G // K
        dev = x3.device
        out = torch.empty(B, 1, dtype=f32, device=dev)
        m3, mb, t = (torch.empty(B, D, dtype=f32, device=dev) for _ in range(3))
        call("conan_stage2_head_fwd", ptr(x3, f32), ptr(xc, f32), ptr(xb, f32), ptr(_c(W3), f32), ptr(_c(b3), f32), ptr(_c(Wb), f32), ptr(_c(bb), f32),
             ptr(_c(wreg), f32), ptr(_c(breg), f32), float(aw), B, K, D, ptr(out), ptr(m3), ptr(mb), ptr(t), stream_ptr())
        ctx.save_for_backward(W3, Wb, wreg, m3, mb, t)
        ctx.dims, ctx.aw = (B, K, D), float(aw)
        return out

    @staticmethod
    def backward(ctx, dout):
        W3, Wb, wreg, m3, mb, t = ctx.saved_tensors
        B, K, D = ctx.dims
        dev = dout.device
        dx3, dxc, dxb = (torch.empty(B * K, D, dtype=f32, device=dev) for _ in range(3))
        dW3, dWb = torch.empty(D, D, dtype=f32, device=dev), torch.empty(D, D, dtype=f32, device=dev)
        db3, dbb = torch.empty(D, dtype=f32, device=dev), torch.empty(D, dtype=f32, device=dev)
        dwreg, dbreg = torch.empty(1, D, dtype=f32, device=dev), torch.empty(1, dtype=f32, device=dev)
        call("conan_stage2_head_bwd", ptr(_c(dout)), ptr(_c(W3)), ptr(_c(Wb)), ptr(_c(wreg)), ptr(m3), ptr(mb), ptr(t), ctx.aw, B, K, D,
             ptr(dx3), ptr(dxc), ptr(dxb), ptr(dW3), ptr(db3), ptr(dWb), ptr(dbb), ptr(dwreg), ptr(dbreg), stream_ptr())
        return dx3, dxc, dxb, dW3, db3, dWb, dbb, dwreg, dbreg, None, None


# ... 1325 lines not shown
```

### conan-fgw_amd/schnet.py

```python
from __future__ import annotations

import math
from typing import Callable, Optional

import torch
from torch import Tensor
from torch.nn import Embedding, Linear, ModuleList, Sequential

from . import ops

OptTensor = Optional[Tensor]


class ShiftedSoftplus(torch.nn.Module):

    def __init__(self):
        super().__init__()
        self.shift = math.log(2.0)

    def forward(self, x: Tensor) -> Tensor:
        return ops.shifted_softplus(x)


class GaussianSmearing(torch.nn.Module):
# ... 112 lines not shown
        if readout not in ("add", "sum"):
            raise NotImplementedError("only the sum readout is used by ConAN")
        self.device = device
        self.hidden_channels = hidden_channels
        self.num_filters = num_filters
        self.num_interactions = num_interactions
        self.num_gaussians = num_gaussians
        self.cutoff = cutoff
        self.use_readout = use_readout
        self.use_covalent = use_covalent
        self.fused_filter = True
        self.mean, self.std, self.scale = mean, std, None
        self.embedding = Embedding(100, hidden_channels, padding_idx=0)
        self.interaction_graph = RadiusInteractionGraph(cutoff, max_num_neighbors)
        self.distance_expansion = GaussianSmearing(0.0, cutoff, num_gaussians)
        self.interactions = ModuleList([InteractionBlock(hidden_channels, num_gaussians, num_filters, cutoff)
                                        for _ in range(num_interactions)])
        self.lin1 = Linear(hidden_channels, hidden_channels // 2)
        self.act = ShiftedSoftplus()
        self.register_buffer("initial_atomref", None)
        self.atomref = None
        torch.nn.init.xavier_uniform_(self.lin1.weight)
        self.lin1.bias.data.fill_(0)
        self.lin1_bary = Linear(hidden_channels, hidden_channels // 2)
        self.lin2_bary = Linear(hidden_channels // 2, hidden_channels // 2)
        self.lin2 = Linear(hidden_channels // 2, hidden_channels // 2)

    def _graphs(self, z: Tensor, pos: Tensor, batch: OptTensor, num_graphs: Optional[int]):
        if not z.is_cuda:
            raise RuntimeError("SchNetNoSum (MI355X) runs on the GPU only: move the inputs to the device; there is no CPU fallback")
        batch = torch.zeros_like(z) if batch is None else batch
        hint_g, hint_n = ops.batch_hints(batch)
        if num_graphs is None:
            num_graphs = hint_g if hint_g is not None else int(batch[-1].item()) + 1
        gptr = ops.graph_ptr_from_batch(batch, num_graphs)
        pairs = self.fused_filter and ops.filter_fused_supported(self.num_gaussians, self.num_filters)
        graph = self.interaction_graph.csr(pos, gptr, num_graphs, pairs=pairs, transpose=torch.is_grad_enabled())
        graph.max_nodes_hint = hint_n if hint_g == num_graphs else None
        return batch, gptr, graph, num_graphs

    def _trunk(self, z: Tensor, graph: ops.RadiusGraph) -> Tensor:
        h = ops.embedding(z, self.embedding.weight, self.embedding.padding_idx)
        if self.fused_filter and ops.filter_fused_supported(self.num_gaussians, self.num_filters):
            rbf = (self.distance_expansion.offset, self.distance_expansion.coeff)
        else:
            rbf = self.distance_expansion(graph)
        for interaction in self.interactions:
            h = interaction(h, graph, rbf)
        return h

    def _head(self, h: Tensor, lin1: Linear, lin2: Linear) -> Tensor:
        return ops.mlp2_outact(h, lin1.weight, lin1.bias, lin2.weight, lin2.bias)

    def forward(self, z: Tensor, pos: Tensor, batch: OptTensor = None, data_batch=None, num_graphs: Optional[int] = None) -> Tensor:
        batch, gptr, graph, G = self._graphs(z, pos, batch, num_graphs)
        h = self._head(self._trunk(z, graph), self.lin1, self.lin2)
        return ops.segment_sum(h, gptr, G) if self.use_readout else h

    def forward_3d_bary(self, z: Tensor, pos: Tensor, batch: OptTensor = None, data_batch=None, num_graphs: Optional[int] = None,
                        _graph=None):
        if _graph is None:
            _, _, graph, _ = self._graphs(z, pos, batch, num_graphs)
        else:
            graph = _graph
        h_shared = self._trunk(z, graph)
        return ops.mlp2_outact_dual(h_shared, *((l1.weight, l1.bias, l2.weight, l2.bias)
                                                for l1, l2 in ((self.lin1, self.lin2), (self.lin1_bary, self.lin2_bary))))

    def _solve_barycenter(self, node_feature: Tensor, edge_index, batch: Tensor, batch_size: int, num_conformers: int,
                          max_nodes: Optional[int] = None):
        K = num_conformers
        G = batch_size * K
        if isinstance(edge_index, ops.RadiusGraph):
            graph = edge_index
        else:
            graph = _graph_from_edge_index(edge_index, batch, G)
        if max_nodes is None:
            max_nodes = getattr(graph, "max_nodes_hint", None)
        if max_nodes is None:
            gp = graph.graph_ptr
            max_nodes = int((gp[1:] - gp[:-1]).max().item())
        Ys, _ = ops.fgw_densify(node_feature, graph, max_nodes, self.FEATURE_SHIFT, adjacency=False)
        N, d = max_nodes, node_feature.shape[1]
        Y, C, T, info, errs = ops.fgw_barycenter_batched(Ys.view(batch_size, K, N, d), None, adjacency=graph)
        self.last_fgw = dict(Y=Y, C=C, T=T, info=info, errs=errs, Ys=Ys)
        return Y, graph

    def _compute_barycenter(self, node_feature: Tensor, edge_index, batch: Tensor, batch_size: int, num_conformers: int,
                            max_nodes: Optional[int] = None, _want_node_out: bool = True):
        Y, graph = self._solve_barycenter(node_feature, edge_index, batch, batch_size, num_conformers, max_nodes)
        F_bary_batch = ops.fgw_readout(Y, num_conformers, self.READOUT_MODE)
        node_out = ops.segment_sum(node_feature, graph.graph_ptr, batch_size * num_conformers) if _want_node_out else None
        return node_out, F_bary_batch

    def forward_w_barycenter_parts(self, z: Tensor, pos: Tensor, num_conformers: int, batch: OptTensor = None, num_graphs: Optional[int] = None,
                                   max_nodes: Optional[int] = None):
        batch, gptr, graph, G = self._graphs(z, pos, batch, num_graphs)
        h_3d, h_bary = self.forward_3d_bary(z, pos, batch, _graph=graph)
        Y, _ = self._solve_barycenter(h_bary, graph, batch, G // num_conformers, num_conformers, max_nodes=max_nodes)
        return h_3d, gptr, Y

    def forward_w_barycenter(self, z: Tensor, pos: Tensor, num_conformers: int, batch: OptTensor = None, data_batch=None,
                             max_iter: int = 100, epsilon: float = 0.1, num_graphs: Optional[int] = None,
                             max_nodes: Optional[int] = None):
        h_3d, gptr, Y = self.forward_w_barycenter_parts(z, pos, num_conformers, batch, num_graphs=num_graphs, max_nodes=max_nodes)
        h_bary = ops.fgw_readout(Y, num_conformers, self.READOUT_MODE)
        h_3d = ops.segment_sum(h_3d, gptr, gptr.numel() - 1)
        return h_3d, h_bary


def _graph_from_edge_index(edge_index: Tensor, batch: Tensor, num_graphs: int) -> ops.RadiusGraph:
    g = object.__new__(ops.RadiusGraph)
    n = batch.shape[0]
    src, tgt = edge_index[0], edge_index[1]
    order = torch.argsort(tgt * n + src)
    src, tgt = src[order], tgt[order]
    deg = torch.bincount(tgt, minlength=n)
    rowptr = torch.zeros(n + 1, dtype=torch.int32, device=batch.device)
    rowptr[1:] = deg.cumsum(0).to(torch.int32)
    g.num_atoms, g.num_graphs = n, num_graphs
    g.graph_ptr = ops.graph_ptr_from_batch(batch, num_graphs)
    g.rowptr, g.col, g.tgt = rowptr, src.to(torch.int32).contiguous(), tgt.to(torch.int32).contiguous()
    g.dist = None
    g.max_edges = max(1, int(src.shape[0]))
    g.num_edges_dev = rowptr[n:]
    g._num_edges = int(src.shape[0])
    g._t_rowptr = g._t_eid = None
    g.pid = None
    g._deg = torch.empty(n + 1, dtype=torch.int32, device=batch.device)
    g.cutoff = g.cap = g.loop = None
    return g
```

### conan-fgw_amd/visnet.py

```python
from __future__ import annotations

import math
from typing import Optional

import torch
from torch import Tensor
from torch.nn import Embedding, LayerNorm, Linear

from . import ops
from . import visnet_ops as vo
from ._lib import call, ptr, stream_ptr

f32 = torch.float32


class ExpNormalSmearing(torch.nn.Module):
    def __init__(self, cutoff: float = 5.0, num_rbf: int = 32):
        super().__init__()
        self.cutoff, self.num_rbf, self.alpha = cutoff, num_rbf, 5.0 / cutoff
        start = torch.exp(torch.tensor(-cutoff))
        self.register_buffer("means", torch.linspace(start, 1, num_rbf))
        self.register_buffer("betas", torch.tensor([(2 / num_rbf * (1 - start)) ** -2] * num_rbf))


# ... 188 lines not shown

class EquivariantScalar(torch.nn.Module):
    def __init__(self, hidden: int, out: int):
        super().__init__()
        self.output_network = torch.nn.ModuleList([GatedEquivariantBlock(hidden, hidden // 2, True), GatedEquivariantBlock(hidden // 2, out, False)])

    def pre_reduce(self, x: Tensor, v: Tensor) -> Tensor:
        for layer in self.output_network:
            x, v = layer(x, v)
        return x


class Atomref(torch.nn.Module):
    def __init__(self, max_z: int = 100):
        super().__init__()
        self.register_buffer("initial_atomref", torch.zeros(max_z, 1))
        self.atomref = Embedding(max_z, 1)
        self.atomref.weight.data.copy_(self.initial_atomref)


class ViSNet(torch.nn.Module):
    FEATURE_SHIFT = 1.0
    READOUT_MODE = 1

    def __init__(self, device, hidden_channels: int, cutoff: float = 5.0):
        super().__init__()
        self.device = device
        self.hidden_channels = hidden_channels
        self.cutoff = cutoff
        self.derivative = False
        self.reduce_op = "sum"
        self.representation_model = ViSNetBlock(hidden_channels=hidden_channels)
        self.output_model = EquivariantScalar(hidden_channels, hidden_channels // 2)
        self.prior_model = Atomref()
        self.output_model_bary = EquivariantScalar(hidden_channels, hidden_channels // 2)
        self.prior_model_bary = Atomref()
        self.register_buffer("mean", torch.tensor(0.0))
        self.register_buffer("std", torch.tensor(1.0))
        from .schnet import RadiusInteractionGraph
        self.interaction_graph = RadiusInteractionGraph(cutoff, max_num_neighbors=32)

    def _prep(self, z: Tensor, batch: Optional[Tensor], num_graphs: Optional[int]):
        if not z.is_cuda:
            raise RuntimeError("ViSNet (MI355X) runs on the GPU only: move the inputs to the device; there is no CPU fallback")
        batch = torch.zeros_like(z) if batch is None else batch
        if num_graphs is None:
            hint_g, _ = ops.batch_hints(batch)
            num_graphs = hint_g if hint_g is not None else int(batch[-1].item()) + 1
        return batch, ops.graph_ptr_from_batch(batch, num_graphs), num_graphs

    def _head(self, xs, vs, z, output_model, prior):
        return vo.prior(output_model.pre_reduce(xs, vs), z, prior.atomref.weight, self.std)

    def forward(self, z: Tensor, pos: Tensor, batch: Tensor, num_graphs: Optional[int] = None) -> Tensor:
        batch, gp, G = self._prep(z, batch, num_graphs)
        xs, vs = self.representation_model(z, pos, gp, G)
        return ops.segment_sum(self._head(xs, vs, z, self.output_model, self.prior_model), gp, G)

    def forward_3d_bary(self, z: Tensor, pos: Tensor, batch: Tensor, num_graphs: Optional[int] = None):
        batch, gp, G = self._prep(z, batch, num_graphs)
        xs, vs = self.representation_model(z, pos, gp, G)
        if NODE_LEVEL_ON_SIDE_STREAM >= 3:
            main = torch.cuda.current_stream()
            side = getattr(self.representation_model, "_node_stream", None) or torch.cuda.Stream(device=main.device)
            object.__setattr__(self.representation_model, "_node_stream", side)
            side.wait_stream(main)
            with torch.cuda.stream(side):
                h = self._head(xs, vs, z, self.output_model, self.prior_model)
            hb = self._head(xs, vs, z, self.output_model_bary, self.prior_model_bary)
            main.wait_stream(side)
            h.record_stream(main)
            return h, hb
        return self._head(xs, vs, z, self.output_model, self.prior_model), self._head(xs, vs, z, self.output_model_bary, self.prior_model_bary)

    def _compute_barycenter(self, node_feature: Tensor, edge_index, batch: Tensor, batch_size: int, num_conformers: int,
                            max_nodes: Optional[int] = None):
        from .schnet import _graph_from_edge_index
        K, G = num_conformers, batch_size * num_conformers
        graph = edge_index if isinstance(edge_index, ops.RadiusGraph) else _graph_from_edge_index(edge_index, batch, G)
        if max_nodes is None:
            hint_g, hint_n = ops.batch_hints(batch)
            max_nodes = hint_n if hint_g == G else None
        if max_nodes is None:
            gp = graph.graph_ptr
            max_nodes = int((gp[1:] - gp[:-1]).max().item())
        Ys, _ = ops.fgw_densify(node_feature, graph, max_nodes, self.FEATURE_SHIFT, adjacency=False)
        N, d = max_nodes, node_feature.shape[1]
        Y, C, T, info, errs = ops.fgw_barycenter_batched(Ys.view(batch_size, K, N, d), None, adjacency=graph)
        self.last_fgw = dict(Y=Y, C=C, T=T, info=info, errs=errs)
        return ops.segment_sum(node_feature, graph.graph_ptr, G), ops.fgw_readout(Y, K, self.READOUT_MODE)

    def forward_w_barycenter(self, z: Tensor, pos: Tensor, num_conformers: int, batch: Optional[Tensor] = None, data_batch=None,
                             max_iter: int = 100, epsilon: float = 0.1, num_graphs: Optional[int] = None, max_nodes: Optional[int] = None):
        batch, gp, G = self._prep(z, batch, num_graphs)
        h_3d, h_bary = self.forward_3d_bary(z, pos, batch, num_graphs=G)
        graph = self.interaction_graph.csr(pos, gp, G)
        _, h_bary = self._compute_barycenter(h_bary, graph, batch, G // num_conformers, num_conformers, max_nodes=max_nodes)
        return ops.segment_sum(h_3d, gp, G), h_bary
```

### conan-fgw_amd/visnet_ops.py

```python
from __future__ import annotations

import torch
from torch import Tensor

from . import ops, wgrad
from ._lib import call, lib, ptr, stream_ptr

f32 = torch.float32
_c = ops._c


SUM_INPUT_GRADIENTS = True


def _new(like: Tensor, *shape):
    return torch.empty(*shape, dtype=f32, device=like.device)


def _tail0_shape(rows: int, width: int, device, m_dev):
    return ops.unread_rows(rows, width, device)


def _tail0(like: Tensor, m_dev):
    return _tail0_shape(like.shape[0], like[0].numel(), like.device, m_dev).view(like.shape)


class _Silu(torch.autograd.Function):
    @staticmethod
    def forward(ctx, x, m_dev):
        x = _c(x)
        y = _tail0(x, m_dev)
        call("conan_silu_fwd", ptr(x, f32), x.shape[0], x.shape[1], ptr(m_dev), ptr(y), stream_ptr())
        ctx.save_for_backward(x)
        ctx.m_dev = m_dev
        return y

    @staticmethod
    def backward(ctx, dy):
        (x,) = ctx.saved_tensors
        dx = _tail0(x, ctx.m_dev)
        call("conan_silu_bwd", ptr(x), ptr(_c(dy)), x.shape[0], x.shape[1], ptr(ctx.m_dev), ptr(dx), stream_ptr())
        return dx, None


def silu(x, m_dev=None):
    return _Silu.apply(x, m_dev)


class _LinearSilu(torch.autograd.Function):

    @staticmethod
    def forward(ctx, x, w, b, m_dev):
        x, w = _c(x), _c(w)
        M, K = x.shape
        N = w.shape[0]
        need = any(ctx.needs_input_grad[:3])
        y = _tail0_shape(M, N, x.device, m_dev)
        if need:
            pre = torch.empty(M, N, dtype=f32, device=x.device)
            call("conan_linear_act_fwd", ptr(x, f32), ptr(w, f32), ptr(b), M, K, N, 3, ptr(m_dev), ptr(y), ptr(pre), stream_ptr())
            ctx.save_for_backward(x, w, pre)
        else:
            call("conan_linear_fwd", ptr(x, f32), ptr(w, f32), ptr(b), None, M, K, N, 0, 3, ptr(m_dev), ptr(y), stream_ptr())
        ctx.m_dev, ctx.has_b = m_dev, b is not None
        return y

    @staticmethod
    def backward(ctx, dy):
        x, w, pre = ctx.saved_tensors
        md = ctx.m_dev
        M, K = x.shape
        N = w.shape[0]
        g = _tail0(pre, md)
        call("conan_silu_bwd", ptr(pre), ptr(_c(dy)), M, N, ptr(md), ptr(g), stream_ptr())
        dx = dw = db = None
        if ctx.needs_input_grad[0]:
            dx = _tail0_shape(M, K, x.device, md)
            call("conan_linear_fwd", ptr(g), ptr(w), None, None, M, N, K, 1, 0, ptr(md), ptr(dx), stream_ptr())
        if ctx.needs_input_grad[1] or (ctx.has_b and ctx.needs_input_grad[2]):
            dw, db = wgrad.plain(g, x, M, K, N, md, w, ctx.has_b)
        return dx, dw, db, None


class _MultiLinear(torch.autograd.Function):

    @staticmethod
    def forward(ctx, x, m_dev, act, tap, *wb):
        x = _c(x)
        M, K = x.shape
        n = len(wb) // 2
        ws, bs = [_c(w) for w in wb[:n]], list(wb[n:])
        need = x.requires_grad or any(w.requires_grad for w in ws)
        ys, pres = [], []
        widths = {w.shape[0] for w in ws}
        if 2 <= n <= 4 and K == 128 and widths == {128} and (all(b is not None for b in bs) or all(b is None for b in bs)):
            import ctypes
            ys = [_tail0_shape(M, 128, x.device, m_dev) for _ in range(n)]
            if act and need:
                pres = [torch.empty(M, 128, dtype=f32, device=x.device) for _ in range(n)]
            arr = lambda ts: (ctypes.c_void_p * n)(*[t.data_ptr() for t in ts])
            call("conan_linear_multi_fwd", ptr(x, f32), arr(ws), arr(bs) if bs[0] is not None else None, M, K, 128, n, 3 if act else 0, ptr(m_dev),
                 arr(ys), arr(pres) if pres else None, stream_ptr())
        else:
            for w, b in zip(ws, bs):
                N = w.shape[0]
                y = _tail0_shape(M, N, x.device, m_dev)
                if act and need:
                    pre = torch.empty(M, N, dtype=f32, device=x.device)
                    call("conan_linear_act_fwd", ptr(x, f32), ptr(w, f32), ptr(b), M, K, N, 3, ptr(m_dev), ptr(y), ptr(pre), stream_ptr())
                    pres.append(pre)
                else:
                    call("conan_linear_fwd", ptr(x, f32), ptr(w, f32), ptr(b), None, M, K, N, 0, 3 if act else 0, ptr(m_dev), ptr(y), stream_ptr())
                ys.append(y)
        ctx.save_for_backward(x, *ws, *pres)
        ctx.n, ctx.act, ctx.m_dev, ctx.has_b, ctx.tap = n, act, m_dev, [b is not None for b in bs], bool(tap)
        return tuple(ys) + ((x.view_as(x),) if tap else ())

    @staticmethod
    def backward(ctx, *dys):
        n, md = ctx.n, ctx.m_dev
        saved = ctx.saved_tensors
        x, ws, pres = saved[0], saved[1:1 + n], saved[1 + n:]
        M, K = x.shape
        seed = _c(dys[n]) if (ctx.tap and dys[n] is not None) else None
        dx = None
        dws, dbs, gs = [None] * n, [None] * n, [None] * n
        for i in range(n):
            if dys[i] is None:
                continue
            N = ws[i].shape[0]
            if ctx.act:
                gs[i] = _tail0(pres[i], md)
                call("conan_silu_bwd", ptr(pres[i]), ptr(_c(dys[i])), M, N, ptr(md), ptr(gs[i]), stream_ptr())
            else:
                gs[i] = _c(dys[i])
        live = [i for i in range(n) if gs[i] is not None]
        one_launch = (SUM_INPUT_GRADIENTS and ctx.needs_input_grad[0] and K == 128 and 2 <= len(live) <= 3
                      and all(ws[i].shape[0] == 128 for i in live))
        if one_launch:
            import ctypes
            m = len(live)
            dx = _tail0_shape(M, K, x.device, md)
            call("conan_linear_sum_fwd", (ctypes.c_void_p * m)(*[gs[i].data_ptr() for i in live]), (ctypes.c_int * m)(*([128] * m)),
                 (ctypes.c_void_p * m)(*[ws[i].data_ptr() for i in live]), m, 1, None, ptr(seed), M, K, ptr(md), ptr(dx), stream_ptr())
            seed = None
        for i in ([] if one_launch else live):
            w, N, g = ws[i], ws[i].shape[0], gs[i]
            if ctx.needs_input_grad[0]:
                if dx is None:
                    dx, res = _tail0_shape(M, K, x.device, md), seed
                    seed = None
                else:
                    res = dx
                if res is None or N <= 128 or (K == 128 and N in (256, 384)):
                    call("conan_linear_fwd", ptr(g), ptr(w), None, ptr(res), M, N, K, 1, 0, ptr(md), ptr(dx), stream_ptr())
                else:
                    tmp = _tail0_shape(M, K, x.device, md)
                    call("conan_linear_fwd", ptr(g), ptr(w), None, None, M, N, K, 1, 0, ptr(md), ptr(tmp), stream_ptr())
                    dx = res + tmp
        if len(live) > 1 and len({ws[i].shape[0] for i in live}) == 1:
            for i, (dw, db) in zip(live, wgrad.shared_x([gs[i] for i in live], x, M, K, ws[live[0]].shape[0], md, [ws[i] for i in live],
                                                               [ctx.has_b[i] for i in live])):
                dws[i], dbs[i] = dw, db
        else:
            for i in live:
                dws[i], dbs[i] = wgrad.plain(gs[i], x, M, K, ws[i].shape[0], md, ws[i], ctx.has_b[i])
        if dx is None and seed is not None:
            dx = seed
        return (dx, None, None, None) + tuple(dws) + tuple(dbs)


def multi_lin(x: Tensor, mods, act_silu: bool = False, m_dev=None, tap: bool = False):
    if all(x.shape[1] % 64 == 0 and m.weight.shape[0] % 64 == 0 for m in mods):
        return _MultiLinear.apply(x, m_dev, act_silu, tap, *[m.weight for m in mods], *[m.bias for m in mods])
    return tuple(lin(x, m, act_silu, m_dev) for m in mods) + ((x,) if tap else ())


def lin(x: Tensor, m: torch.nn.Linear, act_silu: bool = False, m_dev=None, grad_tail_unread: bool = False) -> Tensor:
    if act_silu and x.shape[1] % 64 == 0 and m.weight.shape[0] % 64 == 0:
        return _LinearSilu.apply(x, m.weight, m.bias, m_dev)
    y = ops.linear(x, m.weight, m.bias, m_dev=m_dev, grad_tail_unread=grad_tail_unread and m_dev is not None)
    return silu(y, m_dev) if act_silu else y


class _NeighborScale(torch.autograd.Function):
    @staticmethod
    def forward(ctx, W, graph, cutoff):
        W = _c(W)
        out = torch.empty_like(W)
        call("conan_visnet_neighbor_scale_to", ptr(W), ptr(graph.dist), ptr(graph.col), ptr(graph.tgt), ptr(graph.num_edges_dev),
             graph.max_edges, W.shape[1], float(cutoff), ptr(out), stream_ptr())
        ctx.graph, ctx.cutoff = graph, float(cutoff)
        return out

    @staticmethod
    def backward(ctx, dout):
        g = ctx.graph
        dout = _c(dout)
        d = torch.empty_like(dout)
        call("conan_visnet_neighbor_scale_to", ptr(dout), ptr(g.dist), ptr(g.col), ptr(g.tgt), ptr(g.num_edges_dev), g.max_edges, dout.shape[1],
             ctx.cutoff, ptr(d), stream_ptr())
        return d, None, None


def neighbor_scale(W, graph, cutoff):
    return _NeighborScale.apply(W, graph, cutoff)


class _Concat2(torch.autograd.Function):
    @staticmethod
    def forward(ctx, a, b):
# ... 323 lines not shown
```

Baseline: 116,300.

## Prebuild split-precision weight images once per forward and reuse them across GEMM kernels

Adds a weight-image cache. Each weight matrix is split into f16 planes, pow2-scaled, padded and permuted once per forward pass (scoped by a with_weight_images decorator). The linear and mlp2 kernels then copy that image straight into LDS instead of every block re-reading fp32 weights, running an absmax reduction and splitting them. This removes redundant per-block weight staging and a block-wide sync, at the cost of extra build launches, image memory, and many new API entry points.

```diff
diff --git a/conan-fgw_amd/_lib.py b/conan-fgw_amd/_lib.py
--- a/conan-fgw_amd/_lib.py
+++ b/conan-fgw_amd/_lib.py
@@ -31,6 +31,10 @@
 
 class WgradSlabJob(ctypes.Structure):
     _fields_ = [("g", c_void_p), ("x", c_void_p), ("m_dev", c_void_p), ("ws", c_void_p), ("M", c_int), ("K", c_int), ("N", c_int), ("slices", c_int)]
+
+
+class WeightImageJob(ctypes.Structure):
+    _fields_ = [("w", c_void_p), ("image", c_void_p), ("K", c_int), ("N", c_int), ("form", c_int), ("reserved", c_int)]
 
 
 _P = c_void_p
@@ -200,6 +204,18 @@
         "conan_fgw_bregman_bwd_workspace_bytes": (c_ll, [c_int, c_int, c_int]),
         "conan_fgw_bregman_bwd": (c_int, [_P] * 6 + [c_int, c_int, _D, _D, c_int, c_int, c_int] + [_P] * 13),
     },
+    "conan_fgw_hip_weight_images.h": {
+        "conan_weight_image_bytes": (c_ll, [c_int, c_int]),
+        "conan_weight_images_build": (c_int, [ctypes.POINTER(WeightImageJob), c_int, _P]),
+        "conan_linear_fwd_img": (c_int, [_P, _P, _P, _P, c_int, c_int, c_int, c_int, c_int, _P, _P, _P, _P]),
+        "conan_linear_act_fwd_img": (c_int, [_P, _P, _P, c_int, c_int, c_int, c_int, _P, _P, _P, _P, _P]),
+        "conan_mlp2_fwd_img": (c_int, [_P, _P, _P, _P, _P, _P, c_int, c_int, c_int, c_int, _P, _P, _P, _P, _P]),
+        "conan_mlp2_bwd_img": (c_int, [_P, _P, _P, _P, c_int, c_int, c_int, c_int, _P, _P, _P, _P, _P]),
+        "conan_mlp2_outact_fwd_img": (c_int, [_P, _P, _P, _P, _P, c_int, c_int, c_int, c_int, _P, _P, _P, _P, _P]),
+        "conan_mlp2_outact_bwd_img": (c_int, [_P, _P, _P, _P, c_int, c_int, c_int, c_int, _P, _P, _P, _P, _P, _P]),
+        "conan_mlp2_outact_dual_fwd_img": (c_int, [_P] * 9 + [c_int] * 4 + [_P, c_int, _P, _P, _P, _P, _P, _P]),
+        "conan_mlp2_outact_dual_bwd_img": (c_int, [_P] * 8 + [c_int] * 4 + [_P, _P, _P, _P, _P, _P, _P, _P]),
+    },
     "conan_fgw_hip_mixup_grad.h": {
         "conan_fgw_mixup_barycenter_fwd_record": (c_int, [_P] * 7 + [c_int, c_int, c_int, c_int, ctypes.POINTER(FgwParams), _D, c_int, _D] + [_P] * 9),
         "conan_fgw_mixup_barycenter_bwd_lds_resident": (c_int, [c_int]),
diff --git a/conan-fgw_amd/csrc/fp_planes.h b/conan-fgw_amd/csrc/fp_planes.h
--- a/conan-fgw_amd/csrc/fp_planes.h
+++ b/conan-fgw_amd/csrc/fp_planes.h
@@ -146,6 +146,36 @@
     __device__ __forceinline__ void park(void *planes, float sc) const { park(planes, sc, [](int k) { return k; }); }
 };
 
+__device__ __forceinline__ int m2_perm4(int k) {
+    const int a = (k & 15) >> 2;
+    return (k & ~15) + 8 * (a & 1) + 4 * (a >> 1);
+}
+
+constexpr long long weight_image_plane_bytes(int K, int N) { return 4LL * N * (K + 8); }
+constexpr long long weight_image_bytes(int K, int N) { return (weight_image_plane_bytes(K, N) + 4 + 255) & ~255LL; }
+template <int NO, int KD, int NT>
+struct ImageCopy {
+    static constexpr int V16 = NO * (KD + 8) / 4, PER = (V16 + NT - 1) / NT;
+    uint4 v[PER];
+    __device__ __forceinline__ void fetch(const void *img) {
+        const uint4 *src = reinterpret_cast<const uint4 *>(img);
+#pragma unroll
+        for (int u = 0; u < PER; ++u) {
+            const int q = (int)threadIdx.x + u * NT;
+            v[u] = q < V16 ? src[q] : make_uint4(0u, 0u, 0u, 0u);
+        }
+    }
+    static __device__ __forceinline__ float un(const void *img) { return *reinterpret_cast<const float *>(reinterpret_cast<const uint4 *>(img) + V16); }
+    __device__ __forceinline__ void park(void *planes) const {
+        uint4 *dst = reinterpret_cast<uint4 *>(planes);
+#pragma unroll
+        for (int u = 0; u < PER; ++u) {
+            const int q = (int)threadIdx.x + u * NT;
+            if (q < V16) dst[q] = v[u];
+        }
+    }
+};
+
 template <int S>
 __device__ __forceinline__ void row_load(const float *__restrict__ src, int row, int pitch, int h, float4 (&xa)[S], float4 (&xb)[S]) {
     const float *r = src + (size_t)row * pitch + 8 * h;
diff --git a/conan-fgw_amd/csrc/gemm.hip b/conan-fgw_amd/csrc/gemm.hip
--- a/conan-fgw_amd/csrc/gemm.hip
+++ b/conan-fgw_amd/csrc/gemm.hip
@@ -1,4 +1,5 @@
 #include "fp_planes.h"
+#include "../../include/conan_fgw_hip_weight_images.h"
 
 namespace {
 
@@ -746,7 +747,7 @@
 }
 
 int conan_linear_t_try(const float *x, const float *w, const float *bias, const float *residual, int M, int K, int N, int w_kn,
-                       int act, float *y, const int *m_dev, hipStream_t s, int *rc, float *pre_out);
+                       int act, float *y, const int *m_dev, hipStream_t s, int *rc, float *pre_out, const void *img = nullptr);
 int conan_linear_t_multi(const float *x, const float *const *w, const float *const *bias, int M, int K, int N, int njobs, int act, float *const *y,
                          float *const *pre, const int *m_dev, hipStream_t s, int *rc);
 int conan_linear_t_sum(const float *const *x, const int *ldx, const float *const *w, int nsrc, int w_kn, int ldw, const float *bias,
@@ -754,14 +755,15 @@
 
 extern "C" {
 
-int conan_linear_fwd(const float *x, const float *w, const float *bias, const float *residual, int M, int K, int N,
-                     int w_kn, int act, const int *m_dev, float *y, void *stream) {
+int conan_linear_fwd_img(const float *x, const float *w, const float *bias, const float *residual, int M, int K, int N,
+                         int w_kn, int act, const int *m_dev, float *y, const void *image, void *stream) {
     if (!x || !w || !y || M < 0 || K <= 0 || N <= 0 || act < 0 || act > 3 || (act == 2 && !residual)) return CONAN_E_BADARG;
+    if (image && ((K != 64 && K != 128) || (N != 64 && N != 128))) return CONAN_E_BADARG;
     if (M == 0) return CONAN_OK;
     hipStream_t s = as_stream(stream);
     {
         int rc = CONAN_OK;
-        if (conan_linear_t_try(x, w, bias, residual, M, K, N, w_kn, act, y, m_dev, s, &rc, nullptr)) return rc;
+        if (conan_linear_t_try(x, w, bias, residual, M, K, N, w_kn, act, y, m_dev, s, &rc, nullptr, image)) return rc;
     }
     if (K <= 128 && N <= 128 && (K % BK) == 0) {
         const int Kp = (K + BK - 1) / BK * BK;
@@ -789,14 +791,23 @@
     CONAN_LAUNCH_CHECK();
     return CONAN_OK;
 }
-
+int conan_linear_fwd(const float *x, const float *w, const float *bias, const float *residual, int M, int K, int N,
+                     int w_kn, int act, const int *m_dev, float *y, void *stream) {
+    return conan_linear_fwd_img(x, w, bias, residual, M, K, N, w_kn, act, m_dev, y, nullptr, stream);
+}
+
+int conan_linear_act_fwd_img(const float *x, const float *w, const float *bias, int M, int K, int N, int act, const int *m_dev, float *y,
+                             float *pre, const void *image, void *stream) {
+    if (!x || !w || !y || !pre || M < 0 || K <= 0 || N <= 0 || (act != 1 && act != 3)) return CONAN_E_BADARG;
+    if (image && ((K != 64 && K != 128) || (N != 64 && N != 128))) return CONAN_E_BADARG;
+    if (M == 0) return CONAN_OK;
+    int rc = CONAN_OK;
+    if (conan_linear_t_try(x, w, bias, nullptr, M, K, N, 0, act, y, m_dev, as_stream(stream), &rc, pre, image)) return rc;
+    return CONAN_E_UNSUPPORTED;
+}
 int conan_linear_act_fwd(const float *x, const float *w, const float *bias, int M, int K, int N, int act, const int *m_dev, float *y,
                          float *pre, void *stream) {
-    if (!x || !w || !y || !pre || M < 0 || K <= 0 || N <= 0 || (act != 1 && act != 3)) return CONAN_E_BADARG;
-    if (M == 0) return CONAN_OK;
-    int rc = CONAN_OK;
-    if (conan_linear_t_try(x, w, bias, nullptr, M, K, N, 0, act, y, m_dev, as_stream(stream), &rc, pre)) return rc;
-    return CONAN_E_UNSUPPORTED;
+    return conan_linear_act_fwd_img(x, w, bias, M, K, N, act, m_dev, y, pre, nullptr, stream);
 }
 
 int conan_linear_multi_fwd(const float *x, const float *const *w, const float *const *bias, int M, int K, int N, int num_layers, int act,
diff --git a/conan-fgw_amd/csrc/gemm_t.hip b/conan-fgw_amd/csrc/gemm_t.hip
--- a/conan-fgw_amd/csrc/gemm_t.hip
+++ b/conan-fgw_amd/csrc/gemm_t.hip
@@ -20,7 +20,8 @@
                                                            const float *__restrict__ bias, const float *__restrict__ residual,
                                                            int M, int w_kn, float *y,
                                                            const int *__restrict__ m_dev, int ldx, int ldw, int ldy,
-                                                           const float *accum, float *pre_out, int nc, const LtJobs J) {
+                                                           const float *accum, float *pre_out, int nc, const LtJobs J,
+                                                           const void *__restrict__ img) {
     constexpr int act = ACT;
     constexpr int NB = N / 32;
     constexpr int S = K / 16;
@@ -59,7 +60,12 @@
         pow2_scale(block_absmax<NT>(st.absmax(), wred), wsc, wun);
         st.park(WB, wsc);
     };
-    if (!w_kn) { WeightPlanes<N, K, NT, false> st; stage(st); } else { WeightPlanes<N, K, NT, true> st; stage(st); }
+    if (img) {
+        ImageCopy<N, K, NT> ic;
+        ic.fetch(img);
+        wun = ic.un(img);
+        ic.park(WB);
+    } else if (!w_kn) { WeightPlanes<N, K, NT, false> st; stage(st); } else { WeightPlanes<N, K, NT, true> st; stage(st); }
     for (int t = tid; t < N; t += NT) BL[t] = bias ? bias[t] : 0.f;
     __syncthreads();
 
@@ -133,8 +139,9 @@
 template <int K, int N>
 int launch_t(const float *x, const float *w, const float *bias, const float *residual, int M, int w_kn, int act, float *y,
              const int *m_dev, hipStream_t s, int ldx = K, int ldw = 0, int ldy = N, const float *accum = nullptr, float *pre_out = nullptr,
-             int nc = 1, const LtJobs *jobs = nullptr) {
+             int nc = 1, const LtJobs *jobs = nullptr, const void *img = nullptr) {
     if (ldw == 0) ldw = w_kn ? N : K;
+    if (nc != 1 || ldw != (w_kn ? N : K)) img = nullptr;
     LtJobs J{};
     if (jobs) J = *jobs;
     const size_t lds_w = ((size_t)(LT_NPL * N * (K + 8)) / 2 + N) * 4;
@@ -150,12 +157,12 @@
         if (narrow) {                                                                                                            \
             (void)hipFuncSetAttribute(reinterpret_cast<const void *>(&k_linear_t16<K, N, A, 256>),                               \
                                       hipFuncAttributeMaxDynamicSharedMemorySize, (int)lds16);                                   \
-            k_linear_t16<K, N, A, 256><<<grid16, 256, lds16, s>>>(x, w, bias, residual, M, w_kn, y, m_dev, ldx, ldw, ldy, accum, pre_out, nc, J); \
+            k_linear_t16<K, N, A, 256><<<grid16, 256, lds16, s>>>(x, w, bias, residual, M, w_kn, y, m_dev, ldx, ldw, ldy, accum, pre_out, nc, J, img); \
         } else {                                                                                                                 \
             (void)hipFuncSetAttribute(reinterpret_cast<const void *>(&k_linear_t16<K, N, A, LT_THREADS>),                        \
                                       hipFuncAttributeMaxDynamicSharedMemorySize, (int)lds16);                                   \
             k_linear_t16<K, N, A, LT_THREADS><<<grid16, LT_THREADS, lds16, s>>>(x, w, bias, residual, M, w_kn, y, m_dev, ldx, ldw, ldy, accum, \
-                                                                                pre_out, nc, J);                                 \
+                                                                                pre_out, nc, J, img);                            \
         }                                                                                                                        \
     } while (0)
     switch (act) {
@@ -452,7 +459,7 @@
 #define CONAN_LINEAR_KSUM 0
 #endif
 int conan_linear_t_try(const float *x, const float *w, const float *bias, const float *residual, int M, int K, int N, int w_kn,
-                       int act, float *y, const int *m_dev, hipStream_t s, int *rc, float *pre_out) {
+                       int act, float *y, const int *m_dev, hipStream_t s, int *rc, float *pre_out, const void *img) {
     if (M < 1) return 0;
     if (CONAN_LINEAR_KSUM && N == 128 && (K == 256 || K == 384) && act == 0 && !pre_out) {
         const float *xs[3], *wc[3];
@@ -460,10 +467,10 @@
         for (int c = 0; c < K / 128; ++c) { xs[c] = x + 128 * c; ldx[c] = K; wc[c] = w_kn ? w + (size_t)128 * c * N : w + 128 * c; }
         if (conan_linear_t_sum(xs, ldx, wc, K / 128, w_kn, w_kn ? N : K, bias, residual, M, N, y, m_dev, s, rc)) return 1;
     }
-    if (K == 128 && N == 128) { *rc = launch_t<128, 128>(x, w, bias, residual, M, w_kn, act, y, m_dev, s, 128, 0, 128, nullptr, pre_out); return 1; }
-    if (K == 128 && N == 64) { *rc = launch_t<128, 64>(x, w, bias, residual, M, w_kn, act, y, m_dev, s, 128, 0, 64, nullptr, pre_out); return 1; }
-    if (K == 64 && N == 64) { *rc = launch_t<64, 64>(x, w, bias, residual, M, w_kn, act, y, m_dev, s, 64, 0, 64, nullptr, pre_out); return 1; }
-    if (K == 64 && N == 128) { *rc = launch_t<64, 128>(x, w, bias, residual, M, w_kn, act, y, m_dev, s, 64, 0, 128, nullptr, pre_out); return 1; }
+    if (K == 128 && N == 128) { *rc = launch_t<128, 128>(x, w, bias, residual, M, w_kn, act, y, m_dev, s, 128, 0, 128, nullptr, pre_out, 1, nullptr, img); return 1; }
+    if (K == 128 && N == 64) { *rc = launch_t<128, 64>(x, w, bias, residual, M, w_kn, act, y, m_dev, s, 128, 0, 64, nullptr, pre_out, 1, nullptr, img); return 1; }
+    if (K == 64 && N == 64) { *rc = launch_t<64, 64>(x, w, bias, residual, M, w_kn, act, y, m_dev, s, 64, 0, 64, nullptr, pre_out, 1, nullptr, img); return 1; }
+    if (K == 64 && N == 128) { *rc = launch_t<64, 128>(x, w, bias, residual, M, w_kn, act, y, m_dev, s, 64, 0, 128, nullptr, pre_out, 1, nullptr, img); return 1; }
     if (K == 32 && N == 128 && !w_kn) { *rc = launch_t<32, 128>(x, w, bias, residual, M, w_kn, act, y, m_dev, s, 32, 0, 128, nullptr, pre_out); return 1; }
     if ((K % 64) || (N % 64) || K > 1024 || N > 1024) return 0;
     const bool k128 = (K % 128) == 0, n128 = (N % 128) == 0;
diff --git a/conan-fgw_amd/csrc/mlp2.hip b/conan-fgw_amd/csrc/mlp2.hip
--- a/conan-fgw_amd/csrc/mlp2.hip
+++ b/conan-fgw_amd/csrc/mlp2.hip
@@ -1,15 +1,13 @@
 #include "fp_planes.h"
+#include "../../include/conan_fgw_hip_weight_images.h"
 
 namespace {
 
 constexpr int M2_THREADS = 256, M2_WAVES = 4;
 constexpr int M2_NPL = 2;
 
-__device__ __forceinline__ int m2_perm4(int k) {
-    const int a = (k & 15) >> 2;
-    return (k & ~15) + 8 * (a & 1) + 4 * (a >> 1);
-}
 template <int NO, int KD, bool TRANS> using M2Planes = WeightPlanes<NO, KD, M2_THREADS, TRANS>;
+template <int NO, int KD> using M2Image = ImageCopy<NO, KD, M2_THREADS>;
 
 template <int KA, int NA, int NB, int MODE, int SUM = 0>
 __device__ __forceinline__ void m2_rows(const float4 (&xa)[KA / 16], const float4 (&xb)[KA / 16], const float4 (&av)[MODE == 1 ? NA / 32 : 1][4],
@@ -131,7 +129,7 @@
 __global__ void __launch_bounds__(M2_THREADS) k_mlp2(const float *__restrict__ x, const float *__restrict__ wA, const float *__restrict__ bA,
                                                      const float *__restrict__ wB, const float *__restrict__ bB, const float *__restrict__ aux,
                                                      const float *__restrict__ residual, int M, float *__restrict__ mid_out, float *__restrict__ y,
-                                                     float *__restrict__ in_out) {
+                                                     float *__restrict__ in_out, const void *__restrict__ imgA, const void *__restrict__ imgB) {
     constexpr bool BWD = (MODE & 1) != 0;
     constexpr int SA = KA / 16, MBA = NA / 32;
     constexpr int WORDS_A = (M2_NPL * NA * (KA + 8)) / 2, WORDS_B = (M2_NPL * NB * (NA + 8)) / 2;
@@ -161,21 +159,32 @@
     }
     float4 ya[SA], yb[SA];
     if (MODE == 3) row_load<SA>(aux, mr, KA, h, ya, yb);
-    M2Planes<NA, KA, BWD> stA;
-    M2Planes<NB, NA, BWD> stB;
-    stA.fetch(wA);
-    stB.fetch(wB);
-    const float ma = wave_max(stA.absmax()), mb = wave_max(stB.absmax());
-    if (lane == 0) { wred[wave] = ma; wred[M2_WAVES + wave] = mb; }
-    __syncthreads();
-    float a = wred[0], b = wred[M2_WAVES];
-#pragma unroll
-    for (int w = 1; w < M2_WAVES; ++w) { a = fmaxf(a, wred[w]); b = fmaxf(b, wred[M2_WAVES + w]); }
-    float scA, scB;
-    pow2_scale(a, scA, unA);
-    pow2_scale(b, scB, unB);
-    stA.park(WB, scA);
-    stB.park(WB2, scB, [](int k) { return m2_perm4(k); });
+    if (imgA) {
+        M2Image<NA, KA> icA;
+        M2Image<NB, NA> icB;
+        icA.fetch(imgA);
+        icB.fetch(imgB);
+        unA = icA.un(imgA);
+        unB = icB.un(imgB);
+        icA.park(WB);
+        icB.park(WB2);
+    } else {
+        M2Planes<NA, KA, BWD> stA;
+        M2Planes<NB, NA, BWD> stB;
+        stA.fetch(wA);
+        stB.fetch(wB);
+        const float ma = wave_max(stA.absmax()), mb = wave_max(stB.absmax());
+        if (lane == 0) { wred[wave] = ma; wred[M2_WAVES + wave] = mb; }
+        __syncthreads();
+        float a = wred[0], b = wred[M2_WAVES];
+#pragma unroll
+        for (int w = 1; w < M2_WAVES; ++w) { a = fmaxf(a, wred[w]); b = fmaxf(b, wred[M2_WAVES + w]); }
+        float scA, scB;
+        pow2_scale(a, scA, unA);
+        pow2_scale(b, scB, unB);
+        stA.park(WB, scA);
+        stB.park(WB2, scB, [](int k) { return m2_perm4(k); });
+    }
     for (int t = tid; t < NA + NB; t += M2_THREADS) BL[t] = BWD ? 0.f : (t < NA ? bA[t] : bB[t - NA]);
     if (MODE == 3) m2_ssp_bwd_row<KA>(xa, xb, ya, yb, in_out, m, h, valid);
     __syncthreads();
@@ -187,6 +196,7 @@
 struct M2Head {
     const float *x, *wA, *bA, *wB, *bB, *aux;
     float *mid_out, *y, *in_out;
+    const void *imgA, *imgB;
 };
 template <int KA, int NA, int NB, int MODE, bool SPLIT>
 __global__ void __launch_bounds__(M2_THREADS) k_mlp2_dual(const M2Head ha, const M2Head hb, const int *__restrict__ m_dev, int M) {
@@ -213,30 +223,50 @@
         row_load<SA>(hd[i].x, mr, KA, h, xa[i], xb[i]);
         if (BWD) row_load<SA>(hd[i].aux, mr, KA, h, ya[i], yb[i]);
     }
-    M2Planes<NA, KA, BWD> stA[NH];
-    M2Planes<NB, NA, BWD> stB[NH];
+    float unA[NH], unB[NH];
+    if (ha.imgA) {
+        M2Image<NA, KA> icA[NH];
+        M2Image<NB, NA> icB[NH];
+#pragma unroll
+        for (int i = 0; i < NH; ++i) {
+            icA[i].fetch(hd[i].imgA);
+            icB[i].fetch(hd[i].imgB);
+        }
+#pragma unroll
+        for (int i = 0; i < NH; ++i) {
+            unA[i] = icA[i].un(hd[i].imgA);
+            unB[i] = icB[i].un(hd[i].imgB);
+            icA[i].park(lds + i * WORDS);
+            icB[i].park(lds + i * WORDS + WORDS_A);
+        }
+    } else {
+        M2Planes<NA, KA, BWD> stA[NH];
+        M2Planes<NB, NA, BWD> stB[NH];
+#pragma unroll
+        for (int i = 0; i < NH; ++i) {
+            stA[i].fetch(hd[i].wA);
+            stB[i].fetch(hd[i].wB);
+        }
+#pragma unroll
+        for (int i = 0; i < NH; ++i) {
+            const float ma = wave_max(stA[i].absmax()), mb = wave_max(stB[i].absmax());
+            if (lane == 0) { wred[(2 * i) * M2_WAVES + wave] = ma; wred[(2 * i + 1) * M2_WAVES + wave] = mb; }
+        }
+        __syncthreads();
+#pragma unroll
+        for (int i = 0; i < NH; ++i) {
+            float a = wred[(2 * i) * M2_WAVES], b = wred[(2 * i + 1) * M2_WAVES];
+#pragma unroll
+            for (int w = 1; w < M2_WAVES; ++w) { a = fmaxf(a, wred[(2 * i) * M2_WAVES + w]); b = fmaxf(b, wred[(2 * i + 1) * M2_WAVES + w]); }
+            float scA, scB;
+            pow2_scale(a, scA, unA[i]);
+            pow2_scale(b, scB, unB[i]);
+            stA[i].park(lds + i * WORDS, scA);
+            stB[i].park(lds + i * WORDS + WORDS_A, scB, [](int k) { return m2_perm4(k); });
+        }
+    }
 #pragma unroll
     for (int i = 0; i < NH; ++i) {
-        stA[i].fetch(hd[i].wA);
-        stB[i].fetch(hd[i].wB);
-    }
-#pragma unroll
-    for (int i = 0; i < NH; ++i) {
-        const float ma = wave_max(stA[i].absmax()), mb = wave_max(stB[i].absmax());
-        if (lane == 0) { wred[(2 * i) * M2_WAVES + wave] = ma; wred[(2 * i + 1) * M2_WAVES + wave] = mb; }
-    }
-    __syncthreads();
-    float unA[NH], unB[NH];
-#pragma unroll
-    for (int i = 0; i < NH; ++i) {
-        float a = wred[(2 * i) * M2_WAVES], b = wred[(2 * i + 1) * M2_WAVES];
-#pragma unroll
-        for (int w = 1; w < M2_WAVES; ++w) { a = fmaxf(a, wred[(2 * i) * M2_WAVES + w]); b = fmaxf(b, wred[(2 * i + 1) * M2_WAVES + w]); }
-        float scA, scB;
-        pow2_scale(a, scA, unA[i]);
-        pow2_scale(b, scB, unB[i]);
-        stA[i].park(lds + i * WORDS, scA);
-        stB[i].park(lds + i * WORDS + WORDS_A, scB, [](int k) { return m2_perm4(k); });
         float *BL = lds + NH * WORDS + i * (NA + NB);
         for (int t = tid; t < NA + NB; t += M2_THREADS) BL[t] = BWD ? 0.f : (t < NA ? hd[i].bA[t] : hd[i].bB[t - NA]);
         if (BWD) m2_ssp_bwd_row<KA>(xa[i], xb[i], ya[i], yb[i], hd[i].in_out, m, h, valid);
@@ -262,12 +292,14 @@
 
 template <int KA, int NA, int NB, int MODE>
 int m2_launch(const float *x, const float *wA, const float *bA, const float *wB, const float *bB, const float *aux, const float *residual, int M,
-              float *mid_out, float *y, float *in_out, hipStream_t s) {
+              float *mid_out, float *y, float *in_out, const void *imgA, const void *imgB, hipStream_t s) {
+    if (!imgA || !imgB) imgA = imgB = nullptr;
     constexpr int WA = (M2_NPL * NA * (KA + 8)) / 2, WBw = (M2_NPL * NB * (NA + 8)) / 2;
     const size_t lds = ((size_t)(WA + WBw) + NA + NB) * 4;
     (void)hipFuncSetAttribute(reinterpret_cast<const void *>(&k_mlp2<KA, NA, NB, MODE>), hipFuncAttributeMaxDynamicSharedMemorySize, (int)lds);
     const int tiles = (M + 31) / 32;
-    k_mlp2<KA, NA, NB, MODE><<<(tiles + M2_WAVES - 1) / M2_WAVES, M2_THREADS, lds, s>>>(x, wA, bA, wB, bB, aux, residual, M, mid_out, y, in_out);
+    k_mlp2<KA, NA, NB, MODE><<<(tiles + M2_WAVES - 1) / M2_WAVES, M2_THREADS, lds, s>>>(x, wA, bA, wB, bB, aux, residual, M, mid_out, y, in_out, imgA,
+                                                                                        imgB);
     return hipGetLastError() == hipSuccess ? CONAN_OK : CONAN_E_LAUNCH;
 }
 
@@ -287,59 +319,89 @@
 
 int conan_mlp2_supported(int M, int K, int N1, int N2) { return (K == 128 && N1 == 128 && N2 == 128 && M >= 1 && M <= 65536) ? 1 : 0; }
 
+int conan_mlp2_fwd_img(const float *x, const float *w1, const float *b1, const float *w2, const float *b2, const float *residual, int M, int K, int N1,
+                       int N2, float *mid_out, float *y, const void *img_w1, const void *img_w2, void *stream) {
+    if (!x || !w1 || !b1 || !w2 || !b2 || !y || M < 0) return CONAN_E_BADARG;
+    if (M == 0) return CONAN_OK;
+    if (!conan_mlp2_supported(M, K, N1, N2)) return CONAN_E_UNSUPPORTED;
+    return m2_launch<128, 128, 128, 0>(x, w1, b1, w2, b2, nullptr, residual, M, mid_out, y, nullptr, img_w1, img_w2, as_stream(stream));
+}
 int conan_mlp2_fwd(const float *x, const float *w1, const float *b1, const float *w2, const float *b2, const float *residual, int M, int K, int N1,
                    int N2, float *mid_out, float *y, void *stream) {
-    if (!x || !w1 || !b1 || !w2 || !b2 || !y || M < 0) return CONAN_E_BADARG;
+    return conan_mlp2_fwd_img(x, w1, b1, w2, b2, residual, M, K, N1, N2, mid_out, y, nullptr, nullptr, stream);
+}
+
+int conan_mlp2_bwd_img(const float *dy, const float *w2, const float *w1, const float *mid, int M, int K, int N1, int N2, float *dmid_out, float *dx,
+                       const void *img_w2, const void *img_w1, void *stream) {
+    if (!dy || !w1 || !w2 || !mid || !dx || M < 0) return CONAN_E_BADARG;
     if (M == 0) return CONAN_OK;
     if (!conan_mlp2_supported(M, K, N1, N2)) return CONAN_E_UNSUPPORTED;
-    return m2_launch<128, 128, 128, 0>(x, w1, b1, w2, b2, nullptr, residual, M, mid_out, y, nullptr, as_stream(stream));
-}
-
+    return m2_launch<128, 128, 128, 1>(dy, w2, nullptr, w1, nullptr, mid, nullptr, M, dmid_out, dx, nullptr, img_w2, img_w1, as_stream(stream));
+}
 int conan_mlp2_bwd(const float *dy, const float *w2, const float *w1, const float *mid, int M, int K, int N1, int N2, float *dmid_out, float *dx,
                    void *stream) {
-    if (!dy || !w1 || !w2 || !mid || !dx || M < 0) return CONAN_E_BADARG;
-    if (M == 0) return CONAN_OK;
-    if (!conan_mlp2_supported(M, K, N1, N2)) return CONAN_E_UNSUPPORTED;
-    return m2_launch<128, 128, 128, 1>(dy, w2, nullptr, w1, nullptr, mid, nullptr, M, dmid_out, dx, nullptr, as_stream(stream));
+    return conan_mlp2_bwd_img(dy, w2, w1, mid, M, K, N1, N2, dmid_out, dx, nullptr, nullptr, stream);
 }
 
 int conan_mlp2_outact_supported(int M, int K, int N1, int N2) { return (K == 128 && N1 == 64 && N2 == 64 && M >= 1 && M <= 65536) ? 1 : 0; }
 
+int conan_mlp2_outact_fwd_img(const float *x, const float *w1, const float *b1, const float *w2, const float *b2, int M, int K, int N1, int N2,
+                              float *mid_out, float *y, const void *img_w1, const void *img_w2, void *stream) {
+    if (!x || !w1 || !b1 || !w2 || !b2 || !y || M < 0) return CONAN_E_BADARG;
+    if (M == 0) return CONAN_OK;
+    if (!conan_mlp2_outact_supported(M, K, N1, N2)) return CONAN_E_UNSUPPORTED;
+    return m2_launch<128, 64, 64, 2>(x, w1, b1, w2, b2, nullptr, nullptr, M, mid_out, y, nullptr, img_w1, img_w2, as_stream(stream));
+}
 int conan_mlp2_outact_fwd(const float *x, const float *w1, const float *b1, const float *w2, const float *b2, int M, int K, int N1, int N2,
                           float *mid_out, float *y, void *stream) {
-    if (!x || !w1 || !b1 || !w2 || !b2 || !y || M < 0) return CONAN_E_BADARG;
+    return conan_mlp2_outact_fwd_img(x, w1, b1, w2, b2, M, K, N1, N2, mid_out, y, nullptr, nullptr, stream);
+}
+
+int conan_mlp2_outact_bwd_img(const float *dy, const float *y, const float *w2, const float *w1, int M, int K, int N1, int N2, float *g_out,
+                              float *dmid_out, float *dx, const void *img_w2, const void *img_w1, void *stream) {
+    if (!dy || !y || !w1 || !w2 || !dx || M < 0) return CONAN_E_BADARG;
     if (M == 0) return CONAN_OK;
     if (!conan_mlp2_outact_supported(M, K, N1, N2)) return CONAN_E_UNSUPPORTED;
-    return m2_launch<128, 64, 64, 2>(x, w1, b1, w2, b2, nullptr, nullptr, M, mid_out, y, nullptr, as_stream(stream));
-}
-
+    return m2_launch<64, 64, 128, 3>(dy, w2, nullptr, w1, nullptr, y, nullptr, M, dmid_out, dx, g_out, img_w2, img_w1, as_stream(stream));
+}
 int conan_mlp2_outact_bwd(const float *dy, const float *y, const float *w2, const float *w1, int M, int K, int N1, int N2, float *g_out,
                           float *dmid_out, float *dx, void *stream) {
-    if (!dy || !y || !w1 || !w2 || !dx || M < 0) return CONAN_E_BADARG;
+    return conan_mlp2_outact_bwd_img(dy, y, w2, w1, M, K, N1, N2, g_out, dmid_out, dx, nullptr, nullptr, stream);
+}
+
+int conan_mlp2_outact_dual_fwd_img(const float *x, const float *w1a, const float *b1a, const float *w2a, const float *b2a, const float *w1b,
+                                   const float *b1b, const float *w2b, const float *b2b, int M, int K, int N1, int N2, const int *m_dev, int form,
+                                   float *mid_a, float *y_a, float *mid_b, float *y_b, const void *const *images, void *stream) {
+    if (!x || !w1a || !b1a || !w2a || !b2a || !w1b || !b1b || !w2b || !b2b || !y_a || !y_b || M < 0 || (form != 0 && form != 1)) return CONAN_E_BADARG;
     if (M == 0) return CONAN_OK;
     if (!conan_mlp2_outact_supported(M, K, N1, N2)) return CONAN_E_UNSUPPORTED;
-    return m2_launch<64, 64, 128, 3>(dy, w2, nullptr, w1, nullptr, y, nullptr, M, dmid_out, dx, g_out, as_stream(stream));
-}
-
+    const bool im = images && images[0] && images[1] && images[2] && images[3];
+    const M2Head ha = {x, w1a, b1a, w2a, b2a, nullptr, mid_a, y_a, nullptr, im ? images[0] : nullptr, im ? images[1] : nullptr},
+                 hb = {x, w1b, b1b, w2b, b2b, nullptr, mid_b, y_b, nullptr, im ? images[2] : nullptr, im ? images[3] : nullptr};
+    return form == 0 ? m2_launch_dual<128, 64, 64, 2, true>(ha, hb, m_dev, M, as_stream(stream))
+                     : m2_launch_dual<128, 64, 64, 2, false>(ha, hb, m_dev, M, as_stream(stream));
+}
 int conan_mlp2_outact_dual_fwd(const float *x, const float *w1a, const float *b1a, const float *w2a, const float *b2a, const float *w1b, const float *b1b,
                                const float *w2b, const float *b2b, int M, int K, int N1, int N2, const int *m_dev, int form, float *mid_a, float *y_a,
                                float *mid_b, float *y_b, void *stream) {
-    if (!x || !w1a || !b1a || !w2a || !b2a || !w1b || !b1b || !w2b || !b2b || !y_a || !y_b || M < 0 || (form != 0 && form != 1)) return CONAN_E_BADARG;
+    return conan_mlp2_outact_dual_fwd_img(x, w1a, b1a, w2a, b2a, w1b, b1b, w2b, b2b, M, K, N1, N2, m_dev, form, mid_a, y_a, mid_b, y_b, nullptr, stream);
+}
+
+int conan_mlp2_outact_dual_bwd_img(const float *dy_a, const float *y_a, const float *w2a, const float *w1a, const float *dy_b, const float *y_b,
+                                   const float *w2b, const float *w1b, int M, int K, int N1, int N2, const int *m_dev, float *g_a, float *dmid_a,
+                                   float *g_b, float *dmid_b, float *dx, const void *const *images, void *stream) {
+    if (!dy_a || !y_a || !w1a || !w2a || !dy_b || !y_b || !w1b || !w2b || !dx || M < 0) return CONAN_E_BADARG;
     if (M == 0) return CONAN_OK;
     if (!conan_mlp2_outact_supported(M, K, N1, N2)) return CONAN_E_UNSUPPORTED;
-    const M2Head ha = {x, w1a, b1a, w2a, b2a, nullptr, mid_a, y_a, nullptr}, hb = {x, w1b, b1b, w2b, b2b, nullptr, mid_b, y_b, nullptr};
-    return form == 0 ? m2_launch_dual<128, 64, 64, 2, true>(ha, hb, m_dev, M, as_stream(stream))
-                     : m2_launch_dual<128, 64, 64, 2, false>(ha, hb, m_dev, M, as_stream(stream));
-}
-
+    const bool im = images && images[0] && images[1] && images[2] && images[3];
+    const M2Head ha = {dy_a, w2a, nullptr, w1a, nullptr, y_a, dmid_a, nullptr, g_a, im ? images[0] : nullptr, im ? images[1] : nullptr},
+                 hb = {dy_b, w2b, nullptr, w1b, nullptr, y_b, dmid_b, dx, g_b, im ? images[2] : nullptr, im ? images[3] : nullptr};
+    return m2_launch_dual<64, 64, 128, 3, false>(ha, hb, m_dev, M, as_stream(stream));
+}
 int conan_mlp2_outact_dual_bwd(const float *dy_a, const float *y_a, const float *w2a, const float *w1a, const float *dy_b, const float *y_b,
                                const float *w2b, const float *w1b, int M, int K, int N1, int N2, const int *m_dev, float *g_a, float *dmid_a, float *g_b,
                                float *dmid_b, float *dx, void *stream) {
-    if (!dy_a || !y_a || !w1a || !w2a || !dy_b || !y_b || !w1b || !w2b || !dx || M < 0) return CONAN_E_BADARG;
-    if (M == 0) return CONAN_OK;
-    if (!conan_mlp2_outact_supported(M, K, N1, N2)) return CONAN_E_UNSUPPORTED;
-    const M2Head ha = {dy_a, w2a, nullptr, w1a, nullptr, y_a, dmid_a, nullptr, g_a}, hb = {dy_b, w2b, nullptr, w1b, nullptr, y_b, dmid_b, dx, g_b};
-    return m2_launch_dual<64, 64, 128, 3, false>(ha, hb, m_dev, M, as_stream(stream));
-}
-
-}
+    return conan_mlp2_outact_dual_bwd_img(dy_a, y_a, w2a, w1a, dy_b, y_b, w2b, w1b, M, K, N1, N2, m_dev, g_a, dmid_a, g_b, dmid_b, dx, nullptr, stream);
+}
+
+}
diff --git a/conan-fgw_amd/csrc/weight_images.hip b/conan-fgw_amd/csrc/weight_images.hip
--- /dev/null
+++ b/conan-fgw_amd/csrc/weight_images.hip
@@ -0,0 +1,74 @@
+#include "fp_planes.h"
+#include "../../include/conan_fgw_hip_weight_images.h"
+
+namespace {
+
+constexpr int WI_THREADS = 256, WI_BATCH = 64;
+struct WiJobs {
+    const float *w[WI_BATCH];
+    void *image[WI_BATCH];
+    int code[WI_BATCH];
+};
+
+template <int N, int K, bool TRANS>
+__device__ __forceinline__ void wi_build(const float *__restrict__ w, void *image, bool perm, float *red) {
+    WeightPlanes<N, K, WI_THREADS, TRANS> st;
+    st.fetch(w);
+    float sc, un;
+    pow2_scale(block_absmax<WI_THREADS>(st.absmax(), red), sc, un);
+    if (perm) st.park(image, sc, [](int k) { return m2_perm4(k); });
+    else st.park(image, sc);
+    if (threadIdx.x == 0) *reinterpret_cast<float *>(reinterpret_cast<char *>(image) + weight_image_plane_bytes(K, N)) = un;
+}
+
+__global__ void __launch_bounds__(WI_THREADS) k_weight_images(const WiJobs J) {
+    __shared__ float red[WI_THREADS / 64];
+    const int j = (int)blockIdx.x;
+    const float *w = J.w[j];
+    void *image = J.image[j];
+    const int code = J.code[j];
+    const bool perm = (code & 8) != 0;
+    switch (code & 7) {
+        case 0: wi_build<64, 64, false>(w, image, perm, red); break;
+        case 1: wi_build<64, 128, false>(w, image, perm, red); break;
+        case 2: wi_build<128, 64, false>(w, image, perm, red); break;
+        case 3: wi_build<128, 128, false>(w, image, perm, red); break;
+        case 4: wi_build<64, 64, true>(w, image, perm, red); break;
+        case 5: wi_build<64, 128, true>(w, image, perm, red); break;
+        case 6: wi_build<128, 64, true>(w, image, perm, red); break;
+        default: wi_build<128, 128, true>(w, image, perm, red); break;
+    }
+}
+
+bool wi_dim(int d) { return d == 64 || d == 128; }
+
+}
+
+extern "C" {
+
+long long conan_weight_image_bytes(int K, int N) { return wi_dim(K) && wi_dim(N) ? weight_image_bytes(K, N) : 0; }
+
+int conan_weight_images_build(const conan_weight_image_job *jobs, int num_jobs, void *stream) {
+    if (num_jobs < 0 || (num_jobs && !jobs)) return CONAN_E_BADARG;
+    for (int q = 0; q < num_jobs; ++q) {
+        const conan_weight_image_job &b = jobs[q];
+        if (!b.w || !b.image || !wi_dim(b.K) || !wi_dim(b.N) || b.form < 0 || b.form > 3 || (reinterpret_cast<size_t>(b.w) & 15) ||
+            (reinterpret_cast<size_t>(b.image) & 15))
+            return CONAN_E_BADARG;
+    }
+    hipStream_t s = as_stream(stream);
+    for (int j0 = 0; j0 < num_jobs; j0 += WI_BATCH) {
+        WiJobs J{};
+        const int nb = num_jobs - j0 < WI_BATCH ? num_jobs - j0 : WI_BATCH;
+        for (int q = 0; q < nb; ++q) {
+            const conan_weight_image_job &b = jobs[j0 + q];
+            J.w[q] = b.w; J.image[q] = b.image;
+            J.code[q] = (b.K == 128 ? 1 : 0) | (b.N == 128 ? 2 : 0) | ((b.form & 1) << 2) | ((b.form & 2) << 2);
+        }
+        k_weight_images<<<nb, WI_THREADS, 0, s>>>(J);
+        CONAN_LAUNCH_CHECK();
+    }
+    return CONAN_OK;
+}
+
+}
diff --git a/conan-fgw_amd/gat.py b/conan-fgw_amd/gat.py
--- a/conan-fgw_amd/gat.py
+++ b/conan-fgw_amd/gat.py
@@ -109,6 +109,7 @@
         self.gat_conv1 = GATConv(in_channels, out_channels, edge_dim)
         self.gat_conv2 = GATConv(out_channels, out_channels, edge_dim)
 
+    @ops.with_weight_images
     def forward(self, x: Tensor, edge_index: Tensor, edge_attr: Tensor, batch: Tensor, num_graphs: Optional[int] = None) -> Tensor:
         if not x.is_cuda:
             raise RuntimeError("conan_fgw_amd has no CPU path: inputs must live on the GPU")
diff --git a/conan-fgw_amd/head.py b/conan-fgw_amd/head.py
--- a/conan-fgw_amd/head.py
+++ b/conan-fgw_amd/head.py
@@ -73,6 +73,7 @@
     def _aggregation_index(self, num_graphs: int, device) -> Tensor:
         return torch.arange(num_graphs // self.num_conformers, device=device).repeat_interleave(self.num_conformers)
 
+    @ops.with_weight_images
     def forward(self, batch, conformers_index: Tensor, node_index: Tensor, num_graphs: int = None, max_nodes: int = None) -> Tensor:
         K = self.num_conformers
         main = torch.cuda.current_stream()
@@ -113,6 +114,7 @@
 
 class EmbeddingsWithGATAggregation(EmbeddingsWithGATAggregationBaryCenter):
 
+    @ops.with_weight_images
     def forward(self, batch, conformers_index: Tensor, node_index: Tensor, num_graphs: int = None, max_nodes: int = None) -> Tensor:
         K = self.num_conformers
         x_3d = self.node_embeddings_model(batch.z, batch.pos, node_index)
@@ -156,6 +158,7 @@
         self.self_attention = _SelfAttentionParams(out_channels)
         self.numItermax, self.epsilon, self.agg_weight = 100, 0.1, agg_weight
 
+    @ops.with_weight_images
     def forward(self, batch, conformers_index: Tensor, node_index: Tensor, num_graphs: int = None, max_nodes: int = None) -> Tensor:
         K = self.num_conformers
         main = torch.cuda.current_stream()
@@ -186,6 +189,7 @@
 
 class EmbeddingsWithGATAggregationClassification(EmbeddingsWithGATAggregationClassificationBaryCenter):
 
+    @ops.with_weight_images
     def forward(self, batch, conformers_index: Tensor, node_index: Tensor, num_graphs: int = None, max_nodes: int = None) -> Tensor:
         K = self.num_conformers
         hint = {"num_graphs": num_graphs} if num_graphs is not None else {}
@@ -226,6 +230,7 @@
     create_aggregation_index = EmbeddingsWithGATAggregationBaryCenter.create_aggregation_index
     _aggregation_index = EmbeddingsWithGATAggregationBaryCenter._aggregation_index
 
+    @ops.with_weight_images
     def forward(self, batch, conformers_index: Tensor = None, node_index: Tensor = None, num_graphs: int = None, max_nodes: int = None) -> Tensor:
         x_cov = self.gat_embeddings_model(batch.x, batch.edge_index, batch.edge_attr, batch.batch,
                                           **({"num_graphs": num_graphs} if num_graphs is not None else {}))
diff --git a/conan-fgw_amd/ops.py b/conan-fgw_amd/ops.py
--- a/conan-fgw_amd/ops.py
+++ b/conan-fgw_amd/ops.py
@@ -1,6 +1,7 @@
 from __future__ import annotations
 
 import ctypes
+import functools
 import math
 from typing import Optional
 
@@ -148,6 +149,91 @@
     return tag[0]
 
 
+WEIGHT_IMAGES = True
+_IMAGES = None
+
+
+class WeightImages:
+
+    def __init__(self):
+        self._jobs = {}
+        self._table, self._built = None, 0
+
+    def __len__(self):
+        return len(self._jobs)
+
+    def lookup(self, w: Tensor, K: int, N: int, form: int) -> Optional[Tensor]:
+        if (K != 64 and K != 128) or (N != 64 and N != 128) or w.dtype != f32 or not w.is_contiguous():
+            return None
+        key = (w.data_ptr(), K, N, form)
+        job = self._jobs.get(key)
+        if job is not None:
+            return job[1] if job[0] < self._built else None
+        if key[0] % 16 == 0 and w.numel() == K * N and not torch.cuda.is_current_stream_capturing():
+            image = torch.zeros(lib().conan_weight_image_bytes(K, N), dtype=torch.uint8, device=w.device)
+            self._jobs[key] = (len(self._jobs), image, w.detach())
+            self._table = None
+        return None
+
+    def build(self):
+        n = len(self._jobs)
+        if n:
+            if self._table is None:
+                from ._lib import WeightImageJob
+                self._table = (WeightImageJob * n)(*[WeightImageJob(key[0], image.data_ptr(), key[1], key[2], key[3], 0)
+                                                     for key, (_i, image, _w) in self._jobs.items()])
+            call("conan_weight_images_build", self._table, n, stream_ptr())
+        self._built = n
+
+
+class weight_images:
+
+    def __init__(self, model):
+        self.model, self.entered = model, False
+
+    def __enter__(self):
+        global _IMAGES
+        if WEIGHT_IMAGES and _IMAGES is None:
+            cache = getattr(self.model, "_conan_weight_images", None)
+            if cache is None:
+                cache = WeightImages()
+                object.__setattr__(self.model, "_conan_weight_images", cache)
+            cache.build()
+            _IMAGES, self.entered = cache, True
+        return self
+
+    def __exit__(self, *exc):
+        global _IMAGES
+        if self.entered:
+            _IMAGES, self.entered = None, False
+        return False
+
+
+def with_weight_images(forward):
+    @functools.wraps(forward)
+    def wrapped(self, *args, **kwargs):
+        with weight_images(self):
+            return forward(self, *args, **kwargs)
+    return wrapped
+
+
+def _img(w: Tensor, K: int, N: int, form: int) -> Optional[Tensor]:
+    return None if _IMAGES is None else _IMAGES.lookup(w, K, N, form)
+
+
+def _call_img(name, args, images, as_array=False):
+    if images is None or any(i is None for i in images):
+        call(name, *args, stream_ptr())
+    elif as_array:
+        call(name + "_img", *args, (ctypes.c_void_p * len(images))(*[i.data_ptr() for i in images]), stream_ptr())
+    else:
+        call(name + "_img", *args, *[ptr(i) for i in images], stream_ptr())
+
+
+def linear_call(x, w, b, residual, M, K, N, w_kn, act, m_dev, y, img=None):
+    _call_img("conan_linear_fwd", (ptr(x, f32), ptr(w, f32), ptr(b), ptr(residual), M, K, N, w_kn, act, ptr(m_dev), ptr(y)), (img,))
+
+
 class _LinearFn(torch.autograd.Function):
     @staticmethod
     def forward(ctx, x, w, b, residual, act, m_dev, grad_tail_unread=False):
@@ -155,8 +241,8 @@
         M, K = x.shape
         N = w.shape[0]
         y = torch.empty(M, N, dtype=f32, device=x.device)
-        call("conan_linear_fwd", ptr(x, f32), ptr(w, f32), ptr(b), ptr(_c(residual)) if residual is not None else None,
-             M, K, N, 0, act, ptr(m_dev), ptr(y), stream_ptr())
+        linear_call(x, w, b, _c(residual) if residual is not None else None, M, K, N, 0, act, m_dev, y, _img(w, K, N, 0))
+        ctx.img_t = _img(w, N, K, 1) if ctx.needs_input_grad[0] else None
         ctx.act, ctx.m_dev, ctx.has_b, ctx.has_res, ctx.grad_tail_unread = act, m_dev, b is not None, residual is not None, grad_tail_unread
         ctx.save_for_backward(x, w, y if act else None)
         return y
@@ -181,7 +267,7 @@
                 dx = unread_rows(x.shape[0], x.shape[1], x.device)
             else:
                 dx = empty_rows(x.shape[0], x.shape[1], x.device, md)
-            call("conan_linear_fwd", ptr(g), ptr(w), None, None, M, N, K, 1, 0, ptr(md), ptr(dx), stream_ptr())
+            linear_call(g, w, None, None, M, N, K, 1, 0, md, dx, ctx.img_t)
         if ctx.needs_input_grad[1] or (ctx.has_b and ctx.needs_input_grad[2]):
             dw, db = wgrad.plain(g, x, M, K, N, md, w, ctx.has_b)
         return dx, dw, db, (dy if ctx.has_res else None), None, None, None
@@ -195,7 +281,8 @@
         M, K = x.shape
         N = w.shape[0]
         y = torch.empty(M, N, dtype=f32, device=x.device)
-        call("conan_linear_fwd", ptr(x, f32), ptr(w, f32), None, None, M, K, N, 0, 0, None, ptr(y), stream_ptr())
+        linear_call(x, w, None, None, M, K, N, 0, 0, None, y, _img(w, K, N, 0))
+        ctx.img_t = _img(w, N, K, 1) if ctx.needs_input_grad[0] else None
         ctx.save_for_backward(x, w)
         return y, x.view_as(x)
 
@@ -210,7 +297,7 @@
         dy = _c(dy)
         if ctx.needs_input_grad[0]:
             dx = torch.empty(M, K, dtype=f32, device=x.device)
-            call("conan_linear_fwd", ptr(dy), ptr(w), None, ptr(_c(dtap)) if dtap is not None else None, M, N, K, 1, 0, None, ptr(dx), stream_ptr())
+            linear_call(dy, w, None, _c(dtap) if dtap is not None else None, M, N, K, 1, 0, None, dx, ctx.img_t)
         elif dtap is not None:
             dx = dtap
         if ctx.needs_input_grad[1]:
@@ -237,8 +324,10 @@
         need = any(ctx.needs_input_grad[:5])
         mid = torch.empty(M, N1, dtype=f32, device=x.device) if need else None
         y = torch.empty(M, N2, dtype=f32, device=x.device)
-        call("conan_mlp2_fwd", ptr(x, f32), ptr(w1, f32), ptr(_c(b1), f32), ptr(w2, f32), ptr(_c(b2), f32),
-             ptr(_c(residual)) if residual is not None else None, M, K, N1, N2, ptr(mid), ptr(y), stream_ptr())
+        _call_img("conan_mlp2_fwd", (ptr(x, f32), ptr(w1, f32), ptr(_c(b1), f32), ptr(w2, f32), ptr(_c(b2), f32),
+                                     ptr(_c(residual)) if residual is not None else None, M, K, N1, N2, ptr(mid), ptr(y)),
+                  (_img(w1, K, N1, 0), _img(w2, N1, N2, 2)))
+        ctx.img_t = (_img(w2, N2, N1, 1), _img(w1, N1, K, 3)) if need else (None, None)
         ctx.has_res = residual is not None
         ctx.save_for_backward(x, w1, w2, mid)
         return y
@@ -251,7 +340,7 @@
         N1, N2 = w1.shape[0], w2.shape[0]
         dmid = torch.empty(M, N1, dtype=f32, device=x.device)
         dx = torch.empty(M, K, dtype=f32, device=x.device)
-        call("conan_mlp2_bwd", ptr(dy), ptr(w2), ptr(w1), ptr(mid), M, K, N1, N2, ptr(dmid), ptr(dx), stream_ptr())
+        _call_img("conan_mlp2_bwd", (ptr(dy), ptr(w2), ptr(w1), ptr(mid), M, K, N1, N2, ptr(dmid), ptr(dx)), ctx.img_t)
         dw2, db2 = wgrad.plain(dy, mid, M, N1, N2, None, w2, True)
         dw1, db1 = wgrad.plain(dmid, x, M, K, N1, None, w1, True)
         return dx, dw1, db1, dw2, db2, (dy if ctx.has_res else None)
@@ -273,8 +362,9 @@
         need = any(ctx.needs_input_grad)
         mid = torch.empty(M, N1, dtype=f32, device=x.device) if need else None
         y = torch.empty(M, N2, dtype=f32, device=x.device)
-        call("conan_mlp2_outact_fwd", ptr(x, f32), ptr(w1, f32), ptr(_c(b1), f32), ptr(w2, f32), ptr(_c(b2), f32), M, K, N1, N2, ptr(mid), ptr(y),
-             stream_ptr())
+        _call_img("conan_mlp2_outact_fwd", (ptr(x, f32), ptr(w1, f32), ptr(_c(b1), f32), ptr(w2, f32), ptr(_c(b2), f32), M, K, N1, N2, ptr(mid), ptr(y)),
+                  (_img(w1, K, N1, 0), _img(w2, N1, N2, 2)))
+        ctx.img_t = (_img(w2, N2, N1, 1), _img(w1, N1, K, 3)) if need else (None, None)
         ctx.save_for_backward(x, w1, w2, mid, y)
         return y
 
@@ -288,7 +378,7 @@
         g = torch.empty(M, N2, dtype=f32, device=dev)
         dmid = torch.empty(M, N1, dtype=f32, device=dev)
         dx = torch.empty(M, K, dtype=f32, device=dev)
-        call("conan_mlp2_outact_bwd", ptr(dy), ptr(y), ptr(w2), ptr(w1), M, K, N1, N2, ptr(g), ptr(dmid), ptr(dx), stream_ptr())
+        _call_img("conan_mlp2_outact_bwd", (ptr(dy), ptr(y), ptr(w2), ptr(w1), M, K, N1, N2, ptr(g), ptr(dmid), ptr(dx)), ctx.img_t)
         dw2, db2 = wgrad.plain(g, mid, M, N1, N2, None, w2, True)
         dw1, db1 = wgrad.plain(dmid, x, M, K, N1, None, w1, True)
         return dx, dw1, db1, dw2, db2
@@ -315,9 +405,11 @@
         need = any(ctx.needs_input_grad)
         mid_a, mid_b = (torch.empty(M, N1, dtype=f32, device=dev) if need else None for _ in range(2))
         y_a, y_b = (torch.empty(M, N2, dtype=f32, device=dev) for _ in range(2))
-        call("conan_mlp2_outact_dual_fwd", ptr(x, f32), ptr(w1a, f32), ptr(_c(b1a), f32), ptr(w2a, f32), ptr(_c(b2a), f32), ptr(w1b, f32),
-             ptr(_c(b1b), f32), ptr(w2b, f32), ptr(_c(b2b), f32), M, K, N1, N2, ptr(m_dev), DUAL_HEAD_FORWARD_FORM, ptr(mid_a), ptr(y_a), ptr(mid_b),
-             ptr(y_b), stream_ptr())
+        _call_img("conan_mlp2_outact_dual_fwd", (ptr(x, f32), ptr(w1a, f32), ptr(_c(b1a), f32), ptr(w2a, f32), ptr(_c(b2a), f32), ptr(w1b, f32),
+                                                 ptr(_c(b1b), f32), ptr(w2b, f32), ptr(_c(b2b), f32), M, K, N1, N2, ptr(m_dev), DUAL_HEAD_FORWARD_FORM,
+                                                 ptr(mid_a), ptr(y_a), ptr(mid_b), ptr(y_b)),
+                  (_img(w1a, K, N1, 0), _img(w2a, N1, N2, 2), _img(w1b, K, N1, 0), _img(w2b, N1, N2, 2)), as_array=True)
+        ctx.img_t = [_img(w2a, N2, N1, 1), _img(w1a, N1, K, 3), _img(w2b, N2, N1, 1), _img(w1b, N1, K, 3)] if need else None
         ctx.m_dev = m_dev
         ctx.save_for_backward(x, w1a, w2a, mid_a, y_a, w1b, w2b, mid_b, y_b)
         return y_a, y_b
@@ -332,8 +424,8 @@
         g_a, g_b = (torch.empty(M, N2, dtype=f32, device=dev) for _ in range(2))
         dmid_a, dmid_b = (torch.empty(M, N1, dtype=f32, device=dev) for _ in range(2))
         dx = empty_rows(M, K, dev, md)
-        call("conan_mlp2_outact_dual_bwd", ptr(dy_a), ptr(y_a), ptr(w2a), ptr(w1a), ptr(dy_b), ptr(y_b), ptr(w2b), ptr(w1b), M, K, N1, N2, ptr(md),
-             ptr(g_a), ptr(dmid_a), ptr(g_b), ptr(dmid_b), ptr(dx), stream_ptr())
+        _call_img("conan_mlp2_outact_dual_bwd", (ptr(dy_a), ptr(y_a), ptr(w2a), ptr(w1a), ptr(dy_b), ptr(y_b), ptr(w2b), ptr(w1b), M, K, N1, N2, ptr(md),
+                                                 ptr(g_a), ptr(dmid_a), ptr(g_b), ptr(dmid_b), ptr(dx)), ctx.img_t, as_array=True)
         dw2b, db2b = wgrad.plain(g_b, mid_b, M, N1, N2, md, w2b, True)
         dw1b, db1b = wgrad.plain(dmid_b, x, M, K, N1, md, w1b, True)
         dw2a, db2a = wgrad.plain(g_a, mid_a, M, N1, N2, md, w2a, True)
diff --git a/conan-fgw_amd/schnet.py b/conan-fgw_amd/schnet.py
--- a/conan-fgw_amd/schnet.py
+++ b/conan-fgw_amd/schnet.py
@@ -188,11 +188,13 @@
     def _head(self, h: Tensor, lin1: Linear, lin2: Linear) -> Tensor:
         return ops.mlp2_outact(h, lin1.weight, lin1.bias, lin2.weight, lin2.bias)
 
+    @ops.with_weight_images
     def forward(self, z: Tensor, pos: Tensor, batch: OptTensor = None, data_batch=None, num_graphs: Optional[int] = None) -> Tensor:
         batch, gptr, graph, G = self._graphs(z, pos, batch, num_graphs)
         h = self._head(self._trunk(z, graph), self.lin1, self.lin2)
         return ops.segment_sum(h, gptr, G) if self.use_readout else h
 
+    @ops.with_weight_images
     def forward_3d_bary(self, z: Tensor, pos: Tensor, batch: OptTensor = None, data_batch=None, num_graphs: Optional[int] = None,
                         _graph=None):
         if _graph is None:
@@ -229,6 +231,7 @@
         node_out = ops.segment_sum(node_feature, graph.graph_ptr, batch_size * num_conformers) if _want_node_out else None
         return node_out, F_bary_batch
 
+    @ops.with_weight_images
     def forward_w_barycenter_parts(self, z: Tensor, pos: Tensor, num_conformers: int, batch: OptTensor = None, num_graphs: Optional[int] = None,
                                    max_nodes: Optional[int] = None):
         batch, gptr, graph, G = self._graphs(z, pos, batch, num_graphs)
@@ -236,6 +239,7 @@
         Y, _ = self._solve_barycenter(h_bary, graph, batch, G // num_conformers, num_conformers, max_nodes=max_nodes)
         return h_3d, gptr, Y
 
+    @ops.with_weight_images
     def forward_w_barycenter(self, z: Tensor, pos: Tensor, num_conformers: int, batch: OptTensor = None, data_batch=None,
                              max_iter: int = 100, epsilon: float = 0.1, num_graphs: Optional[int] = None,
                              max_nodes: Optional[int] = None):
diff --git a/conan-fgw_amd/visnet.py b/conan-fgw_amd/visnet.py
--- a/conan-fgw_amd/visnet.py
+++ b/conan-fgw_amd/visnet.py
@@ -264,11 +264,13 @@
     def _head(self, xs, vs, z, output_model, prior):
         return vo.prior(output_model.pre_reduce(xs, vs), z, prior.atomref.weight, self.std)
 
+    @ops.with_weight_images
     def forward(self, z: Tensor, pos: Tensor, batch: Tensor, num_graphs: Optional[int] = None) -> Tensor:
         batch, gp, G = self._prep(z, batch, num_graphs)
         xs, vs = self.representation_model(z, pos, gp, G)
         return ops.segment_sum(self._head(xs, vs, z, self.output_model, self.prior_model), gp, G)
 
+    @ops.with_weight_images
     def forward_3d_bary(self, z: Tensor, pos: Tensor, batch: Tensor, num_graphs: Optional[int] = None):
         batch, gp, G = self._prep(z, batch, num_graphs)
         xs, vs = self.representation_model(z, pos, gp, G)
@@ -302,6 +304,7 @@
         self.last_fgw = dict(Y=Y, C=C, T=T, info=info, errs=errs)
         return ops.segment_sum(node_feature, graph.graph_ptr, G), ops.fgw_readout(Y, K, self.READOUT_MODE)
 
+    @ops.with_weight_images
     def forward_w_barycenter(self, z: Tensor, pos: Tensor, num_conformers: int, batch: Optional[Tensor] = None, data_batch=None,
                              max_iter: int = 100, epsilon: float = 0.1, num_graphs: Optional[int] = None, max_nodes: Optional[int] = None):
         batch, gp, G = self._prep(z, batch, num_graphs)
diff --git a/conan-fgw_amd/visnet_ops.py b/conan-fgw_amd/visnet_ops.py
--- a/conan-fgw_amd/visnet_ops.py
+++ b/conan-fgw_amd/visnet_ops.py
@@ -45,6 +45,10 @@
 
 def silu(x, m_dev=None):
     return _Silu.apply(x, m_dev)
+
+
+def _linear_act_call(x, w, b, M, K, N, m_dev, y, pre):
+    ops._call_img("conan_linear_act_fwd", (ptr(x, f32), ptr(w, f32), ptr(b), M, K, N, 3, ptr(m_dev), ptr(y), ptr(pre)), (ops._img(w, K, N, 0),))
 
 
 class _LinearSilu(torch.autograd.Function):
@@ -58,10 +62,11 @@
         y = _tail0_shape(M, N, x.device, m_dev)
         if need:
             pre = torch.empty(M, N, dtype=f32, device=x.device)
-            call("conan_linear_act_fwd", ptr(x, f32), ptr(w, f32), ptr(b), M, K, N, 3, ptr(m_dev), ptr(y), ptr(pre), stream_ptr())
+            _linear_act_call(x, w, b, M, K, N, m_dev, y, pre)
             ctx.save_for_backward(x, w, pre)
         else:
-            call("conan_linear_fwd", ptr(x, f32), ptr(w, f32), ptr(b), None, M, K, N, 0, 3, ptr(m_dev), ptr(y), stream_ptr())
+            ops.linear_call(x, w, b, None, M, K, N, 0, 3, m_dev, y, ops._img(w, K, N, 0))
+        ctx.img_t = ops._img(w, N, K, 1) if need and ctx.needs_input_grad[0] else None
         ctx.m_dev, ctx.has_b = m_dev, b is not None
         return y
 
@@ -76,7 +81,7 @@
         dx = dw = db = None
         if ctx.needs_input_grad[0]:
             dx = _tail0_shape(M, K, x.device, md)
-            call("conan_linear_fwd", ptr(g), ptr(w), None, None, M, N, K, 1, 0, ptr(md), ptr(dx), stream_ptr())
+            ops.linear_call(g, w, None, None, M, N, K, 1, 0, md, dx, ctx.img_t)
         if ctx.needs_input_grad[1] or (ctx.has_b and ctx.needs_input_grad[2]):
             dw, db = wgrad.plain(g, x, M, K, N, md, w, ctx.has_b)
         return dx, dw, db, None
@@ -107,11 +112,13 @@
                 y = _tail0_shape(M, N, x.device, m_dev)
                 if act and need:
                     pre = torch.empty(M, N, dtype=f32, device=x.device)
-                    call("conan_linear_act_fwd", ptr(x, f32), ptr(w, f32), ptr(b), M, K, N, 3, ptr(m_dev), ptr(y), ptr(pre), stream_ptr())
+                    _linear_act_call(x, w, b, M, K, N, m_dev, y, pre)
                     pres.append(pre)
                 else:
-                    call("conan_linear_fwd", ptr(x, f32), ptr(w, f32), ptr(b), None, M, K, N, 0, 3 if act else 0, ptr(m_dev), ptr(y), stream_ptr())
+                    ops.linear_call(x, w, b, None, M, K, N, 0, 3 if act else 0, m_dev, y, ops._img(w, K, N, 0))
                 ys.append(y)
+        summed = SUM_INPUT_GRADIENTS and K == 128 and 2 <= n <= 3 and widths == {128}
+        ctx.img_t = [ops._img(w, w.shape[0], K, 1) if need and not summed else None for w in ws]
         ctx.save_for_backward(x, *ws, *pres)
         ctx.n, ctx.act, ctx.m_dev, ctx.has_b, ctx.tap = n, act, m_dev, [b is not None for b in bs], bool(tap)
         return tuple(ys) + ((x.view_as(x),) if tap else ())
@@ -153,10 +160,10 @@
                 else:
                     res = dx
                 if res is None or N <= 128 or (K == 128 and N in (256, 384)):
-                    call("conan_linear_fwd", ptr(g), ptr(w), None, ptr(res), M, N, K, 1, 0, ptr(md), ptr(dx), stream_ptr())
+                    ops.linear_call(g, w, None, res, M, N, K, 1, 0, md, dx, ctx.img_t[i])
                 else:
                     tmp = _tail0_shape(M, K, x.device, md)
-                    call("conan_linear_fwd", ptr(g), ptr(w), None, None, M, N, K, 1, 0, ptr(md), ptr(tmp), stream_ptr())
+                    ops.linear_call(g, w, None, None, M, N, K, 1, 0, md, tmp, ctx.img_t[i])
                     dx = res + tmp
         if len(live) > 1 and len({ws[i].shape[0] for i in live}) == 1:
             for i, (dw, db) in zip(live, wgrad.shared_x([gs[i] for i in live], x, M, K, ws[live[0]].shape[0], md, [ws[i] for i in live],
diff --git a/include/conan_fgw_hip_weight_images.h b/include/conan_fgw_hip_weight_images.h
--- /dev/null
+++ b/include/conan_fgw_hip_weight_images.h
@@ -0,0 +1,42 @@
+#ifndef CONAN_FGW_HIP_WEIGHT_IMAGES_H
+#define CONAN_FGW_HIP_WEIGHT_IMAGES_H
+
+#include "conan_fgw_hip.h"
+
+#ifdef __cplusplus
+extern "C" {
+#endif
+
+typedef struct {
+    const float *w;
+    void *image;
+    int K, N, form, reserved;
+} conan_weight_image_job;
+
+long long conan_weight_image_bytes(int K, int N);
+int conan_weight_images_build(const conan_weight_image_job *jobs, int num_jobs, void *stream);
+
+int conan_linear_fwd_img(const float *x, const float *w, const float *bias, const float *residual, int M, int K, int N,
+                         int w_kn, int act, const int *m_dev, float *y, const void *image, void *stream);
+int conan_linear_act_fwd_img(const float *x, const float *w, const float *bias, int M, int K, int N, int act, const int *m_dev, float *y,
+                             float *pre, const void *image, void *stream);
+
+int conan_mlp2_fwd_img(const float *x, const float *w1, const float *b1, const float *w2, const float *b2, const float *residual, int M, int K, int N1,
+                       int N2, float *mid_out, float *y, const void *img_w1, const void *img_w2, void *stream);
+int conan_mlp2_bwd_img(const float *dy, const float *w2, const float *w1, const float *mid, int M, int K, int N1, int N2, float *dmid_out, float *dx,
+                       const void *img_w2, const void *img_w1, void *stream);
+int conan_mlp2_outact_fwd_img(const float *x, const float *w1, const float *b1, const float *w2, const float *b2, int M, int K, int N1, int N2,
+                              float *mid_out, float *y, const void *img_w1, const void *img_w2, void *stream);
+int conan_mlp2_outact_bwd_img(const float *dy, const float *y, const float *w2, const float *w1, int M, int K, int N1, int N2, float *g_out,
+                              float *dmid_out, float *dx, const void *img_w2, const void *img_w1, void *stream);
+int conan_mlp2_outact_dual_fwd_img(const float *x, const float *w1a, const float *b1a, const float *w2a, const float *b2a, const float *w1b,
+                                   const float *b1b, const float *w2b, const float *b2b, int M, int K, int N1, int N2, const int *m_dev, int form,
+                                   float *mid_a, float *y_a, float *mid_b, float *y_b, const void *const *images, void *stream);
+int conan_mlp2_outact_dual_bwd_img(const float *dy_a, const float *y_a, const float *w2a, const float *w1a, const float *dy_b, const float *y_b,
+                                   const float *w2b, const float *w1b, int M, int K, int N1, int N2, const int *m_dev, float *g_a, float *dmid_a,
+                                   float *g_b, float *dmid_b, float *dx, const void *const *images, void *stream);
+
+#ifdef __cplusplus
+}
+#endif
+#endif
```

Result: no change. 117,000 (median of 6 runs) (+0.7%).
